# yixuan/LBFGSpp

Measured on AMD Instinct MI355X. Metric: L-BFGS iterations/sec at n=10^8, m=10; achieved HBM GB/s vs peak, higher is better.
Workload: dtype f64; 1 GPU; north-star: extended Rosenbrock n=100000000 m=10 f64 LineSearchMoreThuente, x0 from counter hash; n=100000000, m=10, history_full=True, fevals_total=111, apply_Hv_persistent_launches=82

## Files before the change

include/LBFGS.h:

```cpp
#ifndef LBFGSX_DROPIN_LBFGS_H
#define LBFGSX_DROPIN_LBFGS_H

#include <algorithm>
#include <cmath>
#include <cstdlib>
#include <cstring>
#include <exception>
#include <limits>
#include <stdexcept>
#include <string>
#include <thread>
#include <type_traits>
#include <vector>

#include "LBFGSpp/BKLDLT.h"
#include "LBFGSpp/DenseHessian.h"
#include "LBFGSpp/Device.h"
#include "LBFGSpp/Interop.h"
#include "LBFGSpp/GramSpace.h"
#include "LBFGSpp/LineSearchBacktracking.h"
#include "LBFGSpp/LineSearchBracketing.h"
#include "LBFGSpp/LineSearchMoreThuente.h"
#include "LBFGSpp/LineSearchNocedalWright.h"
#include "LBFGSpp/Param.h"
// ... 12 lines not shown
    int m_nfev = 0;
    int m_x_at_throw = LBFGSX_VEC_X;
    int m_recursion = RECURSION_VECTOR;
    std::function<void(int, Scalar, DeviceState<Scalar>&)> m_trace;
    std::function<void(int)> m_iter_hook;
    std::function<void(double*, int)> m_reducer;
    std::vector<int> m_devices;
    mutable bool m_grad_gathered = false;

    template <typename Foo, typename HostVec>
    int run(Foo& f, Scalar& fx)
    {
        using std::abs;
        using std::sqrt;
        detail::Evaluator<Scalar, Foo, HostVec> ev(f, m_dev);
        if (m_trace)
            ev.on_eval = [this](int k, Scalar v) { m_trace(k, v, m_dev); };
        if (m_reducer)
        {
            if (m_recursion == RECURSION_VECTOR)
                throw std::invalid_argument("a row-sharded run (set_reducer) needs the Gram-space recursion: the vector "
                                            "two-loop reduces its dot products on the device, inside one launch");
            ev.reduce = m_reducer;
        }
        if constexpr (detail::is_compiled_objective<Scalar, Foo>::value)
        {
            if (m_recursion != RECURSION_VECTOR || m_reducer)
                throw std::invalid_argument("a TermObjective runs with the vector recursion on one device: the Gram-space and "
                                            "row-sharded modes take the built-in objectives or a device functor");
        }
        lbfgsx_ctx* c = m_dev.ctx();
        detail::check(lbfgsx_bfgs_reset(c));
        if (m_recursion == RECURSION_VECTOR)
            detail::check(lbfgsx_gs_set_history_dtype(c, detail::dtype_of<Scalar>::value));
        ev.prepare();

        const int fpast = m_param.past;
        if (fpast > 0)
            m_fx.assign(size_t(fpast), Scalar(0));

        Scalar gnorm2, xnorm2;
        ev.initial(fx, gnorm2, xnorm2);
        m_gnorm = sqrt(gnorm2);
        if (fpast > 0)
            m_fx[0] = fx;
        m_nfev = ev.nfev();
        if (m_gnorm <= m_param.epsilon || m_gnorm <= m_param.epsilon_rel * sqrt(xnorm2))
            return 1;

        const bool gram = (m_recursion != RECURSION_VECTOR);
        const bool gram_f32h = (m_recursion == RECURSION_GRAM_SPACE_F32H) && std::is_same<Scalar, double>::value;
        GramSpaceHistory gsh;
        std::vector<double> gs_coef, gs_sdots, gs_gdots, gs_ydots;
        double gs_coef_g = 0, gs_scal[7] = {0, 0, 0, 0, 0, 0, 0};
        if (gram)
        {
            gsh.reset(m_param.m);
            gsh.set_gradient_norm2(double(gnorm2));
            gs_sdots.assign(size_t(2 * m_param.m), 0.0);
            gs_gdots.assign(size_t(2 * m_param.m), 0.0);
            gs_ydots.assign(size_t(2 * m_param.m), 0.0);
            detail::check(lbfgsx_gs_set_history_dtype(c, gram_f32h ? LBFGSX_F32 : detail::dtype_of<Scalar>::value));
        }

        double dgd = 0;
        if (gram)
        {
            gsh.direction(-1.0, gs_coef, gs_coef_g);
            detail::check(lbfgsx_gs_direction(c, gs_coef.data(), gs_coef_g, &dgd));
            if (m_reducer)
                m_reducer(&dgd, 1);
        }
        else
            detail::check(lbfgsx_apply_Hv(c, LBFGSX_VEC_G, -1.0, &dgd));
        Scalar dg = Scalar(dgd);
        Scalar step = Scalar(1) / m_gnorm;
        constexpr Scalar eps = std::numeric_limits<Scalar>::epsilon();

        int k = 1;
        for (;;)
        {
            detail::Range range_iteration("lbfgs:iteration");
            detail::check(lbfgsx_ls_begin(c));
            const Scalar step_max = m_param.max_step;
            ev.trial_written = false;
            try
            {
                detail::Range range_ls("lbfgs:line_search");
                detail::run_line_search<Scalar, LineSearch<Scalar>, HostVec>(ev, m_param, step_max, step, fx, dg);
            }
            catch (...)
            {
                m_nfev = ev.nfev();
                if (ev.trial_written)
                    m_x_at_throw = LBFGSX_VEC_XT;
                throw;
            }
            m_nfev = ev.nfev();

            double g2 = 0, x2 = 0, syd = 0, yyd = 0;
            if (gram)
            {
                detail::check(lbfgsx_gs_post_linesearch(c, gs_scal, gs_sdots.data(), gs_gdots.data(), gs_ydots.data()));
                if (m_reducer)
                {
                    const size_t tm = size_t(2 * m_param.m);
                    std::vector<double> bundle(7 + 3 * tm);
                    std::copy(gs_scal, gs_scal + 7, bundle.begin());
                    std::copy(gs_sdots.begin(), gs_sdots.end(), bundle.begin() + 7);
                    std::copy(gs_gdots.begin(), gs_gdots.end(), bundle.begin() + 7 + tm);
                    std::copy(gs_ydots.begin(), gs_ydots.end(), bundle.begin() + 7 + 2 * tm);
                    m_reducer(bundle.data(), int(bundle.size()));
                    std::copy(bundle.begin(), bundle.begin() + 7, gs_scal);
                    std::copy(bundle.begin() + 7, bundle.begin() + 7 + tm, gs_sdots.begin());
                    std::copy(bundle.begin() + 7 + tm, bundle.begin() + 7 + 2 * tm, gs_gdots.begin());
                    std::copy(bundle.begin() + 7 + 2 * tm, bundle.end(), gs_ydots.begin());
                }
                g2 = gs_scal[0];
                x2 = gs_scal[1];
                syd = gs_scal[2];
                yyd = gs_scal[3];
            }
            else
            {
                detail::Range range_post("lbfgs:post+apply_Hv");
                detail::check(lbfgsx_post_linesearch_spec(c, -1.0, &g2, &x2, &syd, &yyd));
            }
            m_gnorm = sqrt(Scalar(g2));
            if (m_gnorm <= m_param.epsilon || m_gnorm <= m_param.epsilon_rel * sqrt(Scalar(x2)))
                return k;
            if (fpast > 0)
            {
                const Scalar old = m_fx[size_t(k % fpast)];
                if (k >= fpast && abs(old - fx) <= m_param.delta * std::max(std::max(abs(fx), abs(old)), Scalar(1)))
                    return k;
                m_fx[size_t(k % fpast)] = fx;
            }
            if (m_param.max_iterations != 0 && k >= m_param.max_iterations)
                return k;

            const bool accept = Scalar(syd) > eps * Scalar(yyd);
            if (accept)
                detail::check(lbfgsx_commit_correction(c));

            if (gram)
            {
                gsh.update(gs_scal, gs_sdots.data(), gs_gdots.data(), accept, gram_f32h ? gs_ydots.data() : nullptr);
                gsh.direction(-1.0, gs_coef, gs_coef_g);
                detail::check(lbfgsx_gs_direction(c, gs_coef.data(), gs_coef_g, &dgd));
                if (m_reducer)
                    m_reducer(&dgd, 1);
            }
            else
                detail::check(lbfgsx_apply_Hv(c, LBFGSX_VEC_G, -1.0, &dgd));
            dg = Scalar(dgd);
            step = Scalar(1);
            if (m_iter_hook)
                m_iter_hook(k);
            k++;
        }
    }

public:
    LBFGSSolver(const LBFGSParam<Scalar>& param) : m_param(param)
    {
        m_param.check_param();
// ... 182 lines not shown
```

include/lbfgsx.h:

```cpp
#ifndef LBFGSX_H
#define LBFGSX_H

#include <stddef.h>
#include <stdint.h>

#ifdef __cplusplus
extern "C" {
#endif

typedef struct lbfgsx_ctx lbfgsx_ctx;

enum { LBFGSX_F64 = 0, LBFGSX_F32 = 1 };
enum { LBFGSX_OBJ_NONE = -1, LBFGSX_OBJ_DIAG_QUAD = 0, LBFGSX_OBJ_EXT_ROSENBROCK = 1,
       LBFGSX_OBJ_BOUND = 64  };
enum
{
    LBFGSX_OK = 0,
    LBFGSX_E_INVALID = -1,
    LBFGSX_E_LOGIC = -2,
    LBFGSX_E_RUNTIME = -3,
    LBFGSX_E_HIP = -4,
    LBFGSX_E_NOGPU = -5,
    LBFGSX_E_USER = -6
};
enum { LBFGSX_FLAG_BOUNDED = 1  };

enum
{
    LBFGSX_VEC_X = 0,
    LBFGSX_VEC_G = 1,
    LBFGSX_VEC_XP = 2,
    LBFGSX_VEC_GP = 3,
    LBFGSX_VEC_D = 4,
    LBFGSX_VEC_XT = 5,
    LBFGSX_VEC_GT = 6,
    LBFGSX_VEC_A = 7,
    LBFGSX_VEC_B = 8,
    LBFGSX_VEC_LB = 9,
    LBFGSX_VEC_UB = 10,
    LBFGSX_VEC_XCP = 11
};

const char* lbfgsx_last_error(void);
const char* lbfgsx_version(void);
int lbfgsx_device_count(void);

int lbfgsx_create(lbfgsx_ctx** out, int dtype, int64_t n, int m, int device, int flags);
void lbfgsx_destroy(lbfgsx_ctx* c);
int lbfgsx_set_stream(lbfgsx_ctx* c, void* hip_stream);
int lbfgsx_sync(lbfgsx_ctx* c);
int64_t lbfgsx_n(const lbfgsx_ctx* c);
void* lbfgsx_vec(lbfgsx_ctx* c, int which);
int lbfgsx_upload(lbfgsx_ctx* c, int which, const void* host);
int lbfgsx_download(lbfgsx_ctx* c, int which, void* host);
int lbfgsx_gather(lbfgsx_ctx* c, int which, int64_t stride, double* host);

int lbfgsx_set_shard(lbfgsx_ctx* c, int64_t offset, int64_t n_global);
int lbfgsx_gen_diag_quad(lbfgsx_ctx* c, double kappa, uint64_t seed);
int lbfgsx_gen_rosen_x0(lbfgsx_ctx* c, uint64_t seed);
int lbfgsx_fill(lbfgsx_ctx* c, int which, double value);

int lbfgsx_bfgs_reset(lbfgsx_ctx* c);
int lbfgsx_bfgs_ncorr(const lbfgsx_ctx* c);
double lbfgsx_bfgs_theta(const lbfgsx_ctx* c);
int lbfgsx_bfgs_add_correction_host(lbfgsx_ctx* c, const void* s, const void* y);
int lbfgsx_bfgs_stage_correction_host(lbfgsx_ctx* c, const void* s, const void* y, double* sy, double* yy);
int lbfgsx_bfgs_download_history(lbfgsx_ctx* c, void* S_out, void* Y_out, int* ncorr, int* ptr, double* theta);
int lbfgsx_apply_Hv(lbfgsx_ctx* c, int v_which, double a, double* dg);

int lbfgsx_eval(lbfgsx_ctx* c, int objective, double* fx, double* gnorm2, double* xnorm2);
int lbfgsx_norms(lbfgsx_ctx* c, double* gnorm2, double* xnorm2);
int lbfgsx_ls_begin(lbfgsx_ctx* c);
int lbfgsx_trial(lbfgsx_ctx* c, int objective, double step, double* fx, double* dg);
int lbfgsx_trial_point(lbfgsx_ctx* c, double step);
int lbfgsx_trial_dg(lbfgsx_ctx* c, double* dg);
int lbfgsx_ls_keep_trial_as_lo(lbfgsx_ctx* c);
int lbfgsx_ls_end(lbfgsx_ctx* c, int use_lo);
int lbfgsx_post_linesearch(lbfgsx_ctx* c, double* gnorm2, double* xnorm2, double* sy, double* yy);
int lbfgsx_commit_correction(lbfgsx_ctx* c);
int lbfgsx_post_linesearch_spec(lbfgsx_ctx* c, double a, double* gnorm2, double* xnorm2, double* sy, double* yy);
int lbfgsx_spec_counts(const lbfgsx_ctx* c, int64_t out[3]);
typedef struct lbfgsx_objective lbfgsx_objective;
int lbfgsx_objective_compile(lbfgsx_objective** out, int dtype, int K, const char* body, char* log, size_t log_len);
void lbfgsx_objective_destroy(lbfgsx_objective* obj);
long long lbfgsx_objective_source(int dtype, int K, const char* body, char* out, size_t len);
int lbfgsx_objective_info(const lbfgsx_objective* obj, long long out[8]);
int lbfgsx_objective_K(const lbfgsx_objective* obj);
int lbfgsx_objective_dtype(const lbfgsx_objective* obj);
int lbfgsx_objective_bind(lbfgsx_ctx* c, const lbfgsx_objective* obj, const void* const p[4], const double cs[8], int* id);
int lbfgsx_objective_upload(lbfgsx_ctx* c, int slot, const void* host, void** dev);
int lbfgsx_objective_bound(const lbfgsx_ctx* c, const void* p[4]);
enum { LBFGSX_FORM_TERM = 0, LBFGSX_FORM_CHAIN = 1, LBFGSX_FORM_GRID = 2, LBFGSX_FORM_GRAPH = 3, LBFGSX_FORM_MESH = 4, LBFGSX_FORM_LINEAR = 5 };
int lbfgsx_objective_compile_chain(lbfgsx_objective** out, int dtype, int K, const char* body, char* log, size_t log_len);
long long lbfgsx_objective_source_chain(int dtype, int K, const char* body, char* out, size_t len);
int lbfgsx_objective_form(const lbfgsx_objective* obj);
int lbfgsx_objective_compile_grid(lbfgsx_objective** out, int dtype, const char* body, char* log, size_t log_len);
long long lbfgsx_objective_source_grid(int dtype, const char* body, char* out, size_t len);
int lbfgsx_objective_bind_grid(lbfgsx_ctx* c, const lbfgsx_objective* obj, int64_t rows, int64_t cols, const void* const p[4],
                               const double cs[8], int* id);
int lbfgsx_objective_shape(const lbfgsx_ctx* c, int64_t* rows, int64_t* cols);
int lbfgsx_objective_compile_graph(lbfgsx_objective** out, int dtype, const char* node_body, const char* edge_body, char* log,
                                   size_t log_len);
long long lbfgsx_objective_source_graph(int dtype, const char* node_body, const char* edge_body, char* out, size_t len);
int lbfgsx_objective_bind_graph(lbfgsx_ctx* c, const lbfgsx_objective* obj, int64_t E, const int32_t* ei, const int32_t* ej,
                                int edges_on_device, const void* const p[4], const double cs[8], int* id);
int lbfgsx_objective_topology(lbfgsx_ctx* c, int64_t* E, uint32_t* off, int32_t* other, uint32_t* edge_side);
int lbfgsx_objective_upload_count(lbfgsx_ctx* c, int slot, const void* host, int64_t count, void** dev);
int lbfgsx_objective_compile_mesh(lbfgsx_objective** out, int dtype, int K, int D, const char* node_body, const char* elem_body,
                                  char* log, size_t log_len);
long long lbfgsx_objective_source_mesh(int dtype, int K, int D, const char* node_body, const char* elem_body, char* out, size_t len);
int lbfgsx_objective_bind_mesh(lbfgsx_ctx* c, const lbfgsx_objective* obj, int64_t E, const int32_t* elems, int elems_on_device,
                               const void* const p[4], const double cs[8], int* id);
int lbfgsx_objective_mesh_topology(lbfgsx_ctx* c, int64_t* E, uint32_t* off, uint32_t* words);
int lbfgsx_objective_dim(const lbfgsx_objective* obj);
int lbfgsx_objective_compile_linear(lbfgsx_objective** out, int dtype, const char* coord_body, const char* row_body, char* log,
                                    size_t log_len);
long long lbfgsx_objective_source_linear(int dtype, const char* coord_body, const char* row_body, char* out, size_t len);
int lbfgsx_objective_bind_linear(lbfgsx_ctx* c, const lbfgsx_objective* obj, int64_t R, int64_t nnz, const int32_t* rowptr,
                                 const int32_t* col, const void* val, int matrix_on_device, int lanes, const void* const p[4],
                                 const double cs[8], int* id);
int lbfgsx_objective_linear_topology(lbfgsx_ctx* c, int64_t info[8], uint32_t* colptr, int32_t* trow, uint32_t* tpos,
                                     int32_t* long_col, uint32_t* long_chunk, uint32_t* chunk);
int lbfgsx_device(const lbfgsx_ctx* c);
int lbfgsx_device_push(const lbfgsx_ctx* c, int* prev);
int lbfgsx_device_pop(int prev);
int lbfgsx_persist_counts(const lbfgsx_ctx* c, int64_t out[4]);
int lbfgsx_debug_persist_fault(lbfgsx_ctx* c);
int lbfgsx_counters(int64_t out[3], int reset);
int lbfgsx_counters_ex(int64_t out[8], int reset);
int lbfgsx_poll_counts(const lbfgsx_ctx* c, int64_t out[2]);
int lbfgsx_poll_counts_ex(const lbfgsx_ctx* c, int64_t out[4]);
void lbfgsx_range_push(const char* name);
void lbfgsx_range_pop(void);

int lbfgsx_gs_post_linesearch(lbfgsx_ctx* c, double scal[7], double* sdots, double* gdots, double* ydots);
int lbfgsx_gs_set_history_dtype(lbfgsx_ctx* c, int dtype);
int lbfgsx_gs_direction(lbfgsx_ctx* c, const double* coef, double coef_g, double* dg);

enum
{
    LBFGSX_ST_FREE = 1, LBFGSX_ST_NEWACT = 2, LBFGSX_ST_L = 4, LBFGSX_ST_U = 8, LBFGSX_ST_P = 16
};
enum
{
    LBFGSX_VS_DRT = 0,
    LBFGSX_VS_NEG_CF = 1,
    LBFGSX_VS_NEG_RHS = 2,
    LBFGSX_VS_LBOUND = 3,
    LBFGSX_VS_UBOUND = 4,
    LBFGSX_VS_Y = 5
};
enum
{
    LBFGSX_CB_LINEAR = 0,
    LBFGSX_CB_SOLVE = 1,
    LBFGSX_CB_RHS_ADD = 2,
    LBFGSX_CB_LAMBDA = 3,
    LBFGSX_CB_MU = 4
};
enum
{
    LBFGSX_SO_SAVE_FALLBACK = 0, LBFGSX_SO_RHS_INIT = 1, LBFGSX_SO_ASSIGN_Y = 2, LBFGSX_SO_CLAMP_Y = 3,
    LBFGSX_SO_CLAMP_FB = 4, LBFGSX_SO_ASSIGN_FB = 5
};
// ... 163 lines not shown
```

lbfgspp_amd/_lib.py:

```python
import ctypes as C
import os

HERE = os.path.dirname(os.path.abspath(__file__))

F64, F32 = 0, 1
OBJ_DIAG_QUAD, OBJ_EXT_ROSENBROCK = 0, 1
OBJ_BOUND = 64
LS_NOCEDAL_WRIGHT, LS_MORE_THUENTE, LS_BACKTRACKING, LS_BRACKETING = 0, 1, 2, 3
ALGO_LBFGS, ALGO_LBFGSB = 0, 1
RECURSION_VECTOR, RECURSION_GRAM_SPACE, RECURSION_GRAM_SPACE_F32H = 0, 1, 2
FLAG_BOUNDED = 1
(VEC_X, VEC_G, VEC_XP, VEC_GP, VEC_D, VEC_XT, VEC_GT, VEC_A, VEC_B, VEC_LB, VEC_UB, VEC_XCP) = range(12)
E_INVALID, E_LOGIC, E_RUNTIME, E_HIP, E_NOGPU, E_USER = -1, -2, -3, -4, -5, -6


class Params(C.Structure):
    _fields_ = [("m", C.c_int), ("epsilon", C.c_double), ("epsilon_rel", C.c_double), ("past", C.c_int),
                ("delta", C.c_double), ("max_iterations", C.c_int), ("linesearch", C.c_int),
                ("max_linesearch", C.c_int), ("min_step", C.c_double), ("max_step", C.c_double),
                ("ftol", C.c_double), ("wolfe", C.c_double), ("max_submin", C.c_int)]


class Result(C.Structure):
    _fields_ = [("niter", C.c_int), ("nfev", C.c_int), ("fx", C.c_double), ("gnorm", C.c_double),
# ... 11 lines not shown

ITER_HOOK = C.CFUNCTYPE(None, C.c_int, C.c_void_p)
ALLREDUCE = C.CFUNCTYPE(None, C.POINTER(C.c_double), C.c_int, C.c_void_p)
OBJECTIVE_FN = C.CFUNCTYPE(C.c_int, C.c_void_p, C.c_void_p, C.c_void_p, C.c_int64, C.POINTER(C.c_double))
BATCH_OBJECTIVE_FN = C.CFUNCTYPE(C.c_int, C.c_void_p, C.c_int, C.POINTER(C.c_int64), C.c_void_p, C.c_void_p, C.c_int64,
                                 C.POINTER(C.c_double))

_core = None
_solver = None


class NativeLibraryMissing(RuntimeError):
    pass


def load():
    global _core, _solver
    if _core is not None:
        return _core, _solver
    try:
        import torch
    except Exception:
        pass
    p_core = os.path.join(HERE, "liblbfgsx.so")
    p_sol = os.path.join(HERE, "liblbfgsx_solver.so")
    for p in (p_core, p_sol):
        if not os.path.exists(p):
            raise NativeLibraryMissing(
                "%s not found: build the HIP extension first (python -c 'import __graft_entry__ as g; g.build()')" % p)
    core = C.CDLL(p_core)
    sol = C.CDLL(p_sol)
    vp, i64, dbl, i32 = C.c_void_p, C.c_int64, C.c_double, C.c_int
    pd = C.POINTER(C.c_double)

    def sig(lib, name, res, *args):
        f = getattr(lib, name)
        f.restype = res
        f.argtypes = list(args)
        return f

    sig(core, "lbfgsx_last_error", C.c_char_p)
    sig(core, "lbfgsx_version", C.c_char_p)
    sig(core, "lbfgsx_device_count", i32)
    sig(core, "lbfgsx_create", i32, C.POINTER(vp), i32, i64, i32, i32, i32)
    sig(core, "lbfgsx_destroy", None, vp)
    sig(core, "lbfgsx_set_stream", i32, vp, vp)
    sig(core, "lbfgsx_sync", i32, vp)
    sig(core, "lbfgsx_n", i64, vp)
    sig(core, "lbfgsx_vec", vp, vp, i32)
    sig(core, "lbfgsx_upload", i32, vp, i32, vp)
    sig(core, "lbfgsx_download", i32, vp, i32, vp)
    sig(core, "lbfgsx_gather", i32, vp, i32, i64, pd)
    sig(core, "lbfgsx_gen_diag_quad", i32, vp, dbl, C.c_uint64)
    sig(core, "lbfgsx_gen_rosen_x0", i32, vp, C.c_uint64)
    sig(core, "lbfgsx_fill", i32, vp, i32, dbl)
    sig(core, "lbfgsx_bfgs_reset", i32, vp)
    sig(core, "lbfgsx_bfgs_ncorr", i32, vp)
    sig(core, "lbfgsx_bfgs_theta", dbl, vp)
    sig(core, "lbfgsx_bfgs_add_correction_host", i32, vp, vp, vp)
    sig(core, "lbfgsx_bfgs_download_history", i32, vp, vp, vp, C.POINTER(i32), C.POINTER(i32), pd)
    sig(core, "lbfgsx_apply_Hv", i32, vp, i32, dbl, pd)
    sig(core, "lbfgsx_eval", i32, vp, i32, pd, pd, pd)
    sig(core, "lbfgsx_norms", i32, vp, pd, pd)
    sig(core, "lbfgsx_ls_begin", i32, vp)
    sig(core, "lbfgsx_trial", i32, vp, i32, dbl, pd, pd)
    sig(core, "lbfgsx_trial_point", i32, vp, dbl)
    sig(core, "lbfgsx_trial_dg", i32, vp, pd)
    sig(core, "lbfgsx_ls_keep_trial_as_lo", i32, vp)
    sig(core, "lbfgsx_ls_end", i32, vp, i32)
    sig(core, "lbfgsx_post_linesearch", i32, vp, pd, pd, pd, pd)
    sig(core, "lbfgsx_commit_correction", i32, vp)
    sig(core, "lbfgsx_gs_post_linesearch", i32, vp, pd, pd, pd, pd)
    sig(core, "lbfgsx_gs_set_history_dtype", i32, vp, i32)
    sig(core, "lbfgsx_gs_direction", i32, vp, pd, dbl, pd)
    sig(core, "lbfgsx_timing_enable", i32, vp, i32)
    sig(core, "lbfgsx_timing_read", i32, vp, pd, C.POINTER(i64), pd, C.POINTER(i64))
    sig(core, "lbfgsx_stream_probe", i32, vp, i32, pd, pd)
    sig(core, "lbfgsx_selftest_reduce", i32, vp, i32, i32, i32, pd)
    sig(core, "lbfgsx_post_linesearch_spec", i32, vp, dbl, pd, pd, pd, pd)
    sig(core, "lbfgsx_rccl_allgather_records", i32, C.POINTER(i32), i32, vp, i64, i64, C.POINTER(vp))
    sig(core, "lbfgsx_device_download", i32, i32, vp, i64, vp)
    sig(core, "lbfgsx_device_free", None, i32, vp)
    sig(core, "lbfgsx_spec_counts", i32, vp, C.POINTER(i64 * 3))
    sig(core, "lbfgsx_counters", i32, C.POINTER(i64 * 3), i32)
    sig(core, "lbfgsx_counters_ex", i32, C.POINTER(i64 * 8), i32)
    sig(core, "lbfgsx_poll_counts", i32, vp, C.POINTER(i64 * 2))
    sig(core, "lbfgsx_poll_counts_ex", i32, vp, C.POINTER(i64 * 4))
    sig(core, "lbfgsx_b_compact_vec_counts", i32, C.POINTER(i64 * 4), i32)
    sig(core, "lbfgsx_b_reserve", i32, vp)
    sig(core, "lbfgsx_device", i32, vp)
    sig(core, "lbfgsx_persist_counts", i32, vp, C.POINTER(i64 * 4))
    sig(core, "lbfgsx_debug_persist_fault", i32, vp)

    sig(sol, "lbfgsx_solver_create", i32, C.POINTER(vp), i32, i32, i32, C.POINTER(Params), i32)
    sig(sol, "lbfgsx_solver_create_error", C.c_char_p)
    sig(sol, "lbfgsx_solver_destroy", None, vp)
    sig(sol, "lbfgsx_solver_prepare", i32, vp, i64)
    sig(sol, "lbfgsx_solver_ctx", vp, vp)
    sig(sol, "lbfgsx_solver_set_recursion", i32, vp, i32)
    sig(sol, "lbfgsx_solver_set_allreduce", i32, vp, ALLREDUCE, vp)
    sig(sol, "lbfgsx_solver_set_devices", i32, vp, C.POINTER(i32), i32)
    sig(core, "lbfgsx_comm_unique_id", i32, C.c_char_p)
    sig(core, "lbfgsx_comm_create_rank", i32, C.POINTER(vp), i32, i32, i32, C.c_char_p)
    sig(core, "lbfgsx_comm_create_local", i32, C.POINTER(vp), C.POINTER(i32), i32)
    sig(core, "lbfgsx_comm_allreduce_sum", i32, vp, i32, pd, i32)
    sig(core, "lbfgsx_comm_abort", i32, vp)
    sig(core, "lbfgsx_comm_abort_from", i32, vp, i32)
    sig(core, "lbfgsx_comm_first_abort", i32, vp)
    sig(core, "lbfgsx_b_gram_pairs_max", i32, vp)
    sig(core, "lbfgsx_b_post_linesearch_build", i32, vp, dbl, pd, pd, pd, pd)
    sig(core, "lbfgsx_b_post_build_counts", i32, C.POINTER(i64 * 2), i32)
    sig(core, "lbfgsx_b_psel_counts", i32, C.POINTER(i64 * 1), i32)
    sig(core, "lbfgsx_b_dg_maxstep_trial", i32, vp, i32, dbl, pd, pd)
    sig(core, "lbfgsx_b_solve_sweep_rhs", i32, vp, i32, i32, pd, dbl, pd, pd, pd, C.POINTER(i64 * 7))
    sig(core, "lbfgsx_b_solve_sweep_rhs_ready", i32, vp)
    sig(core, "lbfgsx_b_gram_last_vrow_dd", i32, vp, pd)
    sig(core, "lbfgsx_b_wtv_lu_c", i32, vp, pd, C.POINTER(i64), pd, C.POINTER(i64), pd)
    sig(core, "lbfgsx_b_trial_ahead_counts", i32, vp, C.POINTER(i64 * 2))
    sig(core, "lbfgsx_comm_info", i32, vp, C.POINTER(i32 * 4))
    sig(core, "lbfgsx_comm_calls", i64, vp, i32)
    sig(core, "lbfgsx_comm_hook_arg", vp, vp, i32)
    sig(core, "lbfgsx_comm_destroy", None, vp)
    sig(core, "lbfgsx_set_shard", i32, vp, i64, i64)
    sig(sol, "lbfgsx_solver_set_iteration_hook", i32, vp, ITER_HOOK, vp)
    sig(sol, "lbfgsx_batch_minimize", i32, i32, i32, i32, C.POINTER(Params), i32, i64, i64, i64, C.c_uint64, i32, i32,
        C.POINTER(BatchItem))
    sig(sol, "lbfgsx_batch_minimize_lockstep", i32, i32, C.POINTER(Params), i64, i64, i32, C.c_uint64, i32,
        C.POINTER(BatchItem), vp, C.c_char_p, i32)
    sig(sol, "lbfgsx_batch_minimize_lockstep_multi", i32, i32, C.POINTER(Params), i64, i64, i32, C.c_uint64,
        C.POINTER(i32), i32, C.POINTER(BatchItem), vp, C.c_char_p, i32)
    sig(sol, "lbfgsx_batch_minimize_lockstep_ex", i32, i32, i32, i32, dbl, C.POINTER(Params), i64, i64, i32, C.c_uint64,
        C.POINTER(i32), i32, C.POINTER(BatchItem), vp, C.c_char_p, i32)
    sig(sol, "lbfgsx_lockstep_create", i32, C.POINTER(vp), i32, i32, C.POINTER(Params), i64, i32, i32, i32, C.c_char_p, i32)
    sig(sol, "lbfgsx_lockstep_minimize", i32, vp, i32, dbl, C.c_uint64, i64, C.POINTER(BatchItem), vp, C.POINTER(dbl * 8),
        C.c_char_p, i32)
    sig(sol, "lbfgsx_lockstep_destroy", None, vp)
    sig(sol, "lbfgsx_lockstep_set_timing", i32, vp, i32)
    sig(sol, "lbfgsx_solver_hessians", i32, vp, vp, vp)
    sig(sol, "lbfgsx_solver_stats", i32, vp, C.POINTER(C.c_longlong * 8))
    sig(sol, "lbfgsx_solver_stats2", i32, vp, C.POINTER(C.c_longlong * 8))
    sig(sol, "lbfgsx_solver_stats3", i32, vp, C.POINTER(C.c_longlong * 8))
    sig(sol, "lbfgsx_solver_minimize", i32, vp, i32, i64, vp, vp, vp, vp, vp, C.POINTER(Trace), C.POINTER(Result))
    sig(sol, "lbfgsx_solver_minimize_fn", i32, vp, i64, OBJECTIVE_FN, vp, vp, vp, vp, C.POINTER(Trace), C.POINTER(Result))
    sig(sol, "lbfgsx_lockstep_minimize_fn", i32, vp, vp, BATCH_OBJECTIVE_FN, vp, C.POINTER(BatchItem), vp, C.POINTER(dbl * 8),
        C.c_char_p, i32)
    sig(core, "lbfgsx_objective_compile", i32, C.POINTER(vp), i32, i32, C.c_char_p, C.c_char_p, C.c_size_t)
    sig(core, "lbfgsx_objective_destroy", None, vp)
    sig(core, "lbfgsx_objective_source", C.c_longlong, i32, i32, C.c_char_p, C.c_char_p, C.c_size_t)
    sig(core, "lbfgsx_objective_info", i32, vp, C.POINTER(C.c_longlong * 8))
    sig(core, "lbfgsx_objective_compile_chain", i32, C.POINTER(vp), i32, i32, C.c_char_p, C.c_char_p, C.c_size_t)
    sig(core, "lbfgsx_objective_source_chain", C.c_longlong, i32, i32, C.c_char_p, C.c_char_p, C.c_size_t)
    sig(core, "lbfgsx_objective_form", i32, vp)
    sig(core, "lbfgsx_objective_K", i32, vp)
    sig(core, "lbfgsx_objective_dtype", i32, vp)
    sig(core, "lbfgsx_objective_bind", i32, vp, vp, C.POINTER(vp * 4), C.POINTER(dbl * 8), C.POINTER(i32))
    sig(core, "lbfgsx_objective_upload", i32, vp, i32, vp, C.POINTER(vp))
    sig(core, "lbfgsx_objective_bound", i32, vp, C.POINTER(vp * 4))
    sig(sol, "lbfgsx_solver_minimize_obj", i32, vp, vp, i64, C.POINTER(vp * 4), i32, C.POINTER(dbl * 8), vp, vp, vp,
        C.POINTER(Trace), C.POINTER(Result))
    sig(core, "lbfgsx_objective_compile_grid", i32, C.POINTER(vp), i32, C.c_char_p, C.c_char_p, C.c_size_t)
    sig(core, "lbfgsx_objective_source_grid", C.c_longlong, i32, C.c_char_p, C.c_char_p, C.c_size_t)
    sig(core, "lbfgsx_objective_bind_grid", i32, vp, vp, i64, i64, C.POINTER(vp * 4), C.POINTER(dbl * 8), C.POINTER(i32))
    sig(core, "lbfgsx_objective_shape", i32, vp, C.POINTER(i64), C.POINTER(i64))
    sig(sol, "lbfgsx_solver_minimize_grid", i32, vp, vp, i64, i64, C.POINTER(vp * 4), i32, C.POINTER(dbl * 8), vp, vp, vp,
        C.POINTER(Trace), C.POINTER(Result))
    i32p, u32p = C.POINTER(C.c_int32), C.POINTER(C.c_uint32)
# ... 64 lines not shown
```

lbfgspp_amd/csrc/ctx.hpp:

```cpp
#pragma once
#include <hip/hip_runtime.h>
#include <stdint.h>

#include <atomic>
#include <chrono>
#include <string>
#include <vector>

#include "../../include/lbfgsx.h"
#include "reduce.cuh"

struct lbfgsx_ctx;
namespace lbfgsx {

void set_error(const std::string& msg);

#define LBFGSX_HIP(expr)                                                                      \
    do                                                                                        \
    {                                                                                         \
        hipError_t e_ = (expr);                                                               \
        if (e_ != hipSuccess)                                                                 \
        {                                                                                     \
            lbfgsx::set_error(std::string(#expr) + ": " + hipGetErrorString(e_) + " [" + __FILE__ + ":" + std::to_string(__LINE__) + "]");            \
            return LBFGSX_E_HIP;                                                              \
// ... 95 lines not shown
int bounded_note_column(lbfgsx_ctx* c, int col);
struct GsState;
void gs_free(lbfgsx_ctx* c);

struct EventPair
{
    hipEvent_t a, b;
};

constexpr int kGridCap = 1024;
constexpr int kGridCapTwoloop = 512;

}

struct lbfgsx_ctx
{
    int dtype = LBFGSX_F64;
    size_t esz = 8;
    int64_t n = 0, ld = 0;
    int64_t shard_off = 0, n_global = 0;
    int m = 0, device = 0, flags = 0;
    hipStream_t stream = nullptr;
    bool own_stream = false;

    void* xb[3] = {nullptr, nullptr, nullptr};
    void* gb[3] = {nullptr, nullptr, nullptr};
    int cur = 0, xp = 0, lo = 0, trial = 1;
    void* d = nullptr;
    void* a = nullptr;
    void* b = nullptr;

    void* S = nullptr;
    void* Y = nullptr;
    std::vector<int> phys;
    unsigned phys_version = 1;
    int spare = 0;
    int ncorr = 0, ptr = 0;
    bool pending = false;
    double theta = 1.0;
    double pend_sy = 0.0, pend_yy = 0.0;
    std::vector<double> ys_host;

    lbfgsx::ScLayout sl;
    void* sc = nullptr;
    void* hout = nullptr;
    void* outmap_host = nullptr;
    void* outmap_dev = nullptr;
    lbfgsx::RedWs ws;
    unsigned long long* done_host = nullptr;
    unsigned long long* done_dev = nullptr;
    unsigned long long done_seq = 0;
    long long poll_waits = 0, poll_timeouts = 0, poll_lost = 0;
    long long poll_late = 0;
    bool poll_pending = false;
    bool poll_off = false;
    unsigned tl_step = 0;
    bool persist = true;
    bool meet_all = true;
    int persist_cooldown = 0;
    int persist_backoff = 8;
    int64_t persist_timeouts = 0;
    int64_t step_products = 0;
    int persist_grid = 0;
    unsigned* gen_dev = nullptr;
    size_t gen_words = 0;
    unsigned gen_count = 0;
    int64_t persist_steps_timed = 0;
    int64_t coarse_steps_timed = 0;
    int64_t fused_timed = 0;
    bool counted = false;
    int64_t persist_launches = 0;
    bool fuse_post = true;
    bool fast_persist_out = true;
    bool st_valid = false;
    int st_obj = -1, st_xp = -1, st_trial = -1;
    double st_step = 0.0, st_f = 0.0, st_dg = 0.0;
    int st_cooldown = 0;
    int64_t st_runs = 0, st_hits = 0;
    bool spec_valid = false;
    unsigned spec_version = 0;
    int spec_cur = 0;
    double spec_a = 0.0, spec_dg = 0.0;
    int64_t spec_launches = 0, spec_used = 0, spec_rejected = 0;

    const struct lbfgsx_objective* term = nullptr;
    void* term_fn[6] = {nullptr, nullptr, nullptr, nullptr, nullptr, nullptr};
    const void* term_p[4] = {nullptr, nullptr, nullptr, nullptr};
    double term_c[8] = {0, 0, 0, 0, 0, 0, 0, 0};
    int term_np = 0;
    int term_form = 0;
    int64_t term_rows = 0, term_cols = 0;
    void* term_own[4] = {nullptr, nullptr, nullptr, nullptr};
    int64_t term_own_count[4] = {0, 0, 0, 0};
    int64_t graph_E = 0;
    void* graph_off = nullptr;
    void* graph_inc = nullptr;
    int mesh_K = 0, mesh_D = 0;
    struct LinearTopo
    {
        int64_t R = 0, nnz = 0, nchunks = 0;
        int L = 0, C = 0, nlong = 0;
        void *rowptr = nullptr, *col = nullptr, *val = nullptr;
        void *colptr = nullptr, *trow = nullptr, *tval = nullptr;
        void* tpos = nullptr;
        void *w = nullptr, *v = nullptr;
        void *part = nullptr, *long_col = nullptr, *long_chunk = nullptr;
        void* chunk = nullptr;
    } lin;

    void* lb = nullptr;
    void* ub = nullptr;
    void* xcp = nullptr;
    struct lbfgsb_state* bstate = nullptr;
    lbfgsx::GsState* gs = nullptr;
    bool gs_f32h = false;

    bool timing = false;
    bool timing_per_launch = true;
    std::vector<lbfgsx::EventPair> ev_twoloop, ev_hv;
    void* gather_tmp = nullptr;
    int64_t gather_cap = 0;

    template <class T>
    T* out_slot() const
    {
        return outmap_dev ? static_cast<T*>(outmap_dev) : static_cast<T*>(sc) + sl.out(0);
    }
    void* col(void* base, int c) const { return static_cast<char*>(base) + size_t(c) * size_t(ld) * esz; }
    int grid_for(int64_t nelem, int unroll_ = 1) const
    {
        const int64_t w = (dtype == LBFGSX_F64) ? 2 : 4;
        const int64_t tile = int64_t(lbfgsx::kBlock) * unroll_;
        int64_t blocks = (nelem / w + tile - 1) / tile;
        if (blocks < 1)
            blocks = 1;
        if (blocks > lbfgsx::kGridCap)
            blocks = lbfgsx::kGridCap;
        return int(blocks);
    }
};

namespace lbfgsx {
inline void poll_arm(lbfgsx_ctx* c)
{
    if (c->done_host && !c->poll_off)
    {
        c->ws.done = c->done_dev;
        c->ws.seq = ++c->done_seq;
        c->poll_pending = true;
    }
}
inline bool poll_armed(const lbfgsx_ctx* c) { return c->done_host && c->poll_pending && c->ws.done && c->ws.seq == c->done_seq; }
inline void poll_disarm(lbfgsx_ctx* c)
{
    c->ws.done = nullptr;
    c->poll_pending = false;
}
inline hipError_t poll_wait(lbfgsx_ctx* c)
{
    if (!poll_armed(c))
    {
        poll_disarm(c);
        return stream_sync(c->stream);
    }
    poll_disarm(c);
    counters().syncs.fetch_add(1, std::memory_order_relaxed);
    const bool tr = host_trace_on();
    if (tr)
        host_trace(">sync");
// ... 39 lines not shown
```

lbfgspp_amd/csrc/jit_objective.hip:

```cpp
#include <dlfcn.h>
#include <hip/hiprtc.h>

#include <chrono>
#include <cstdio>
#include <cstdlib>
#include <cstring>
#include <map>
#include <memory>
#include <mutex>
#include <string>
#include <vector>

#include "launch_args.hpp"

namespace {

const char* const kKernelNames[6][lbfgsx::JIT_NSLOTS] = {
    {"k_eval", "k_trial", "k_b_eval", "k_b_dg_maxstep_trial"},
    {"k_chain_eval", "k_chain_trial", "k_chain_b_eval", "k_chain_b_dg_maxstep_trial"},
    {"k_grid_eval", "k_grid_trial", "k_grid_b_eval", "k_grid_b_dg_maxstep_trial"},
    {"k_graph_eval", "k_graph_trial", "k_graph_b_eval", "k_graph_b_dg_maxstep_trial"},
    {"k_mesh_eval", "k_mesh_trial", "k_mesh_b_eval", "k_mesh_b_dg_maxstep_trial"},
    {"k_lin_eval", "k_lin_trial", "k_lin_b_eval", "k_lin_b_dg_maxstep_trial", "k_lin_rows", "k_lin_rows_trial"}};
const char* const kObjStruct[6] = {"ObjTerm", "ObjChain", "ObjGrid", "ObjGraph", "ObjMesh", "ObjLinear"};
const char* const kFormName[6] = {"term objective", "chain objective", "grid objective", "graph objective", "mesh objective",
                                  "linear-model objective"};
inline int kernels_of(int form) { return form == LBFGSX_FORM_LINEAR ? lbfgsx::JIT_NSLOTS : lbfgsx::JIT_NKERNELS; }

struct Rtc
{
    void* lib = nullptr;
    decltype(&hiprtcCreateProgram) create = nullptr;
    decltype(&hiprtcDestroyProgram) destroy = nullptr;
    decltype(&hiprtcAddNameExpression) add_name = nullptr;
    decltype(&hiprtcCompileProgram) compile = nullptr;
    decltype(&hiprtcGetProgramLogSize) log_size = nullptr;
    decltype(&hiprtcGetProgramLog) log = nullptr;
    decltype(&hiprtcGetLoweredName) lowered = nullptr;
    decltype(&hiprtcGetCodeSize) code_size = nullptr;
    decltype(&hiprtcGetCode) code = nullptr;
    std::string error;
};

const Rtc& rtc()
{
    static Rtc r;
    static std::once_flag once;
    std::call_once(once, []() {
        std::vector<std::string> names = {"libhiprtc.so"};
        if (const char* e = getenv("ROCM_PATH"))
            names.push_back(std::string(e) + "/lib/libhiprtc.so");
        names.push_back("/opt/rocm/lib/libhiprtc.so");
        names.push_back("libhiprtc.so.7");
        for (const std::string& n : names)
            if ((r.lib = dlopen(n.c_str(), RTLD_NOW | RTLD_LOCAL)))
                break;
        if (!r.lib)
        {
            r.error = "libhiprtc.so not found (the run-time compiler of ROCm)";
            return;
        }
#define RTC_SYM(member, name)                                             \
    r.member = reinterpret_cast<decltype(r.member)>(dlsym(r.lib, #name)); \
    if (!r.member)                                                        \
        r.error = "libhiprtc.so lacks " #name;
        RTC_SYM(create, hiprtcCreateProgram)
        RTC_SYM(destroy, hiprtcDestroyProgram)
        RTC_SYM(add_name, hiprtcAddNameExpression)
        RTC_SYM(compile, hiprtcCompileProgram)
        RTC_SYM(log_size, hiprtcGetProgramLogSize)
        RTC_SYM(log, hiprtcGetProgramLog)
        RTC_SYM(lowered, hiprtcGetLoweredName)
        RTC_SYM(code_size, hiprtcGetCodeSize)
        RTC_SYM(code, hiprtcGetCode)
#undef RTC_SYM
    });
    return r;
}

std::string kernel_dir()
{
    if (const char* e = getenv("LBFGSX_KERNEL_DIR"))
        return e;
    Dl_info info;
    if (dladdr(reinterpret_cast<const void*>(&kernel_dir), &info) && info.dli_fname)
    {
        std::string p = info.dli_fname;
        const size_t k = p.rfind('/');
        return (k == std::string::npos ? std::string(".") : p.substr(0, k)) + "/csrc";
    }
    return "csrc";
}

std::string generate_chain(int dtype, int K, const char* body);
std::string generate_grid(int dtype, const char* body);
std::string generate_graph(int dtype, const char* node, const char* body);
std::string generate_mesh(int dtype, int K, int D, const char* node, const char* body);
std::string generate_linear(int dtype, const char* coord, const char* body);

std::string generate(int form, int dtype, int K, const char* body, const char* node, int D)
{
    if (form == LBFGSX_FORM_LINEAR)
        return generate_linear(dtype, node, body);
    if (form == LBFGSX_FORM_MESH)
        return generate_mesh(dtype, K, D, node, body);
    if (form == LBFGSX_FORM_GRAPH)
        return generate_graph(dtype, node, body);
    if (form == LBFGSX_FORM_CHAIN)
        return generate_chain(dtype, K, body);
    if (form == LBFGSX_FORM_GRID)
        return generate_grid(dtype, body);
    std::string s;
    s += "// generated by lbfgsx_objective_compile: one term objective for the fused kernels\n";
    s += "#include \"lbfgs_kernels.cuh\"\n";
    s += "#include \"lbfgsb_kernels.cuh\"\n";
    s += "namespace lbfgsx {\n";
    s += std::string("typedef ") + (dtype == LBFGSX_F64 ? "double" : "float") + " term_scalar_t;\n";
    s += "struct ObjTerm\n{\n";
    s += "    typedef term_scalar_t T;\n";
    s += "    static constexpr int K = " + std::to_string(K) + ";\n";
    s += "    const T* p0;\n    const T* p1;\n    const T* p2;\n    const T* p3;\n    T c[8];\n";
    s += "    // one term: x[0..K) in, g[0..K) out, the term's value returned\n";
    s += "    __device__ __forceinline__ T term(const T (&x)[K], T (&g)[K], int64_t i) const\n    {\n";
    s += "#line 1 \"objective_body\"\n";
    s += body;
    s += "\n#line 1 \"objective_wrapper\"\n";
    s += "    }\n";
    s += "    // the W / K terms of one 16-byte pack (W is a multiple of K: a term never straddles a pack)\n";
    s += "    template <class A>\n";
    s += "    __device__ __forceinline__ void pack(int64_t vi, const Pack<T>& x, Pack<T>& g, A& fx) const\n    {\n";
    s += "        constexpr int W = Vec16<T>::W;\n";
    s += "#pragma unroll\n";
    s += "        for (int k = 0; k < W; k += K)\n        {\n";
    s += "            T tx[K], tg[K];\n";
    s += "#pragma unroll\n";
    s += "            for (int j = 0; j < K; j++)\n                tx[j] = x.e[k + j];\n";
    s += "            const T v = term(tx, tg, vi * W + k);\n";
    s += "#pragma unroll\n";
    s += "            for (int j = 0; j < K; j++)\n                g.e[k + j] = tg[j];\n";
    s += "            fx.add(v);\n";
    s += "        }\n    }\n";
    s += "    __device__ __forceinline__ T finish(T sum) const { return sum; }\n";
    s += "    // the coordinates past the last whole pack, called for every i of them: the term that starts at i, if one does\n";
    s += "    template <class A>\n";
    s += "    __device__ __forceinline__ void tail(int64_t i, int64_t n, const T* x, T* g, A& fx) const\n    {\n";
    s += "        if (i % K == 0 && i + K <= n)\n        {\n";
    s += "            T tx[K], tg[K];\n";
    s += "            for (int j = 0; j < K; j++)\n                tx[j] = x[i + j];\n";
    s += "            const T v = term(tx, tg, i);\n";
    s += "            for (int j = 0; j < K; j++)\n                g[i + j] = tg[j];\n";
    s += "            fx.add(v);\n";
    s += "        }\n    }\n";
    s += "};\n";
    s += "typedef term_scalar_t S;\n";
    s += "template __global__ void k_eval<S, ObjTerm>(const S*, S*, int64_t, ObjTerm, RedWs, S*);\n";
    s += "template __global__ void k_trial<S, ObjTerm>(const S*, const S*, S, S*, S*, int64_t, ObjTerm, RedWs, S*, int);\n";
    s += "template __global__ void k_b_eval<S, ObjTerm>(const S*, S*, const S*, const S*, int64_t, ObjTerm, RedWs, S*);\n";
    s += "template __global__ void k_b_dg_maxstep_trial<S, ObjTerm>(const S*, const S*, const S*, const S*, const S*, S, S*, S*, "
         "int64_t, ObjTerm, RedWs, S*, int);\n";
    s += "}  // namespace lbfgsx\n";
    return s;
}

std::string generate_chain(int dtype, int K, const char* body)
{
    std::string s;
    s += "// generated by lbfgsx_objective_compile_chain: one chain objective for the fused kernels\n";
    s += "#include \"chain_kernels.cuh\"\n";
    s += "namespace lbfgsx {\n";
    s += std::string("typedef ") + (dtype == LBFGSX_F64 ? "double" : "float") + " term_scalar_t;\n";
    s += "struct ObjChain\n{\n";
    s += "    typedef term_scalar_t T;\n";
    s += "    static constexpr int K = " + std::to_string(K) + ";\n";
    s += "    const T* p0;\n    const T* p1;\n    const T* p2;\n    const T* p3;\n    T c[8];\n";
    s += "    // the term that starts at coordinate i: x[0..K) in, its K partial derivatives g[0..K) out, its value returned\n";
    s += "    __device__ __forceinline__ T term(const T (&x)[K], T (&g)[K], int64_t i) const\n    {\n";
    s += "#line 1 \"objective_body\"\n";
    s += body;
    s += "\n#line 1 \"objective_wrapper\"\n";
    s += "    }\n";
    s += "};\n";
    s += "typedef term_scalar_t S;\n";
    s += "template __global__ void k_chain_eval<S, ObjChain>(const S*, S*, int64_t, ObjChain, RedWs, S*);\n";
    s += "template __global__ void k_chain_trial<S, ObjChain>(const S*, const S*, S, S*, S*, int64_t, ObjChain, RedWs, S*, int);\n";
    s += "template __global__ void k_chain_b_eval<S, ObjChain>(const S*, S*, const S*, const S*, int64_t, ObjChain, RedWs, S*);\n";
    s += "template __global__ void k_chain_b_dg_maxstep_trial<S, ObjChain>(const S*, const S*, const S*, const S*, const S*, S, S*, "
         "S*, int64_t, ObjChain, RedWs, S*, int);\n";
    s += "}  // namespace lbfgsx\n";
    return s;
}

std::string generate_grid(int dtype, const char* body)
{
    std::string s;
    s += "// generated by lbfgsx_objective_compile_grid: one grid objective for the fused kernels\n";
    s += "#include \"grid_kernels.cuh\"\n";
    s += "namespace lbfgsx {\n";
    s += std::string("typedef ") + (dtype == LBFGSX_F64 ? "double" : "float") + " term_scalar_t;\n";
    s += "struct ObjGrid\n{\n";
    s += "    typedef term_scalar_t T;\n";
    s += "    static constexpr int K = 4;\n";
    s += "    const T* p0;\n    const T* p1;\n    const T* p2;\n    const T* p3;\n    T c[8];\n";
    s += "    int64_t rows, cols;\n";
    s += "    // the cell whose origin is node (row, col), flat index i = row*cols + col: x = {x[row,col], x[row,col+1], x[row+1,col],\n";
    s += "    // x[row+1,col+1]} in, its four partial derivatives g out, its value returned\n";
    s += "    __device__ __forceinline__ T term(const T (&x)[4], T (&g)[4], int64_t i, int64_t row, int64_t col) const\n    {\n";
    s += "#line 1 \"objective_body\"\n";
    s += body;
    s += "\n#line 1 \"objective_wrapper\"\n";
    s += "    }\n";
    s += "};\n";
    s += "typedef term_scalar_t S;\n";
    s += "template __global__ void k_grid_eval<S, ObjGrid>(const S*, S*, int64_t, ObjGrid, RedWs, S*);\n";
    s += "template __global__ void k_grid_trial<S, ObjGrid>(const S*, const S*, S, S*, S*, int64_t, ObjGrid, RedWs, S*, int);\n";
    s += "template __global__ void k_grid_b_eval<S, ObjGrid>(const S*, S*, const S*, const S*, int64_t, ObjGrid, RedWs, S*);\n";
    s += "template __global__ void k_grid_b_dg_maxstep_trial<S, ObjGrid>(const S*, const S*, const S*, const S*, const S*, S, S*, "
         "S*, int64_t, ObjGrid, RedWs, S*, int);\n";
    s += "}  // namespace lbfgsx\n";
    return s;
}

std::string generate_graph(int dtype, const char* node, const char* body)
{
    const bool has_node = node && *node;
    std::string s;
    s += "// generated by lbfgsx_objective_compile_graph: one graph objective for the fused kernels\n";
    s += "#include \"graph_kernels.cuh\"\n";
    s += "namespace lbfgsx {\n";
    s += std::string("typedef ") + (dtype == LBFGSX_F64 ? "double" : "float") + " term_scalar_t;\n";
    s += "struct ObjGraph\n{\n";
    s += "    typedef term_scalar_t T;\n";
    s += "    static constexpr int K = 2;\n";
    s += std::string("    static constexpr bool kNode = ") + (has_node ? "true" : "false") + ";\n";
    s += "    const T* p0;\n    const T* p1;\n    const T* p2;\n    const T* p3;\n    T c[8];\n";
    s += "    const uint32_t* off;\n    const GraphEntry* inc;\n    int64_t E;\n";
    s += "    // the term of node i: x[0] = x[i] in, its derivative g[0] out, its value returned\n";
    s += "    __device__ __forceinline__ T node(const T (&x)[1], T (&g)[1], int64_t i) const\n    {\n";
    if (has_node)
    {
// ... 233 lines not shown

bool find_symbol(const std::vector<char>& co, const std::string& name, Elf64Sym& out)
{
    if (co.size() < sizeof(Elf64Ehdr) || std::memcmp(co.data(), "\177ELF", 4) != 0)
        return false;
    Elf64Ehdr eh;
    std::memcpy(&eh, co.data(), sizeof(eh));
    if (eh.shentsize != sizeof(Elf64Shdr) || eh.shoff + uint64_t(eh.shnum) * sizeof(Elf64Shdr) > co.size())
        return false;
    std::vector<Elf64Shdr> sh(eh.shnum);
    std::memcpy(sh.data(), co.data() + eh.shoff, sh.size() * sizeof(Elf64Shdr));
    for (const Elf64Shdr& t : sh)
    {
        if ((t.type != 2 && t.type != 11) || t.link >= sh.size() || t.offset + t.size > co.size())
            continue;
        const Elf64Shdr& str = sh[t.link];
        if (str.offset + str.size > co.size())
            continue;
        for (uint64_t k = 0; k + sizeof(Elf64Sym) <= t.size; k += sizeof(Elf64Sym))
        {
            Elf64Sym sy;
            std::memcpy(&sy, co.data() + t.offset + k, sizeof(sy));
            if (sy.name >= str.size)
                continue;
            const char* nm = co.data() + str.offset + sy.name;
            const size_t room = size_t(str.size - sy.name);
            if (name.size() < room && std::memcmp(nm, name.c_str(), name.size() + 1) == 0)
            {
                out = sy;
                return true;
            }
        }
    }
    return false;
}

bool kernel_resources(const std::vector<char>& co, const std::string& kernel, long long& vgprs, long long& scratch)
{
    Elf64Sym kd;
    if (!find_symbol(co, kernel + ".kd", kd))
        return false;
    Elf64Ehdr eh;
    std::memcpy(&eh, co.data(), sizeof(eh));
    uint64_t off = 0;
    bool found = false;
    for (int k = 0; k < eh.shnum && !found; k++)
    {
        Elf64Shdr t;
        std::memcpy(&t, co.data() + eh.shoff + uint64_t(k) * sizeof(Elf64Shdr), sizeof(t));
        if (t.type != 8 && t.addr <= kd.value && kd.value + 64 <= t.addr + t.size)
        {
            off = t.offset + (kd.value - t.addr);
            found = true;
        }
    }
    if (!found || off + 64 > co.size())
        return false;
    uint32_t priv = 0, rsrc1 = 0;
    std::memcpy(&priv, co.data() + off + 4, 4);
    std::memcpy(&rsrc1, co.data() + off + 48, 4);
    scratch = priv;
    Elf64Sym nv, na;
    if (find_symbol(co, kernel + ".num_vgpr", nv))
        vgprs = (long long) nv.value + (find_symbol(co, kernel + ".num_agpr", na) ? (long long) na.value : 0);
    else
        vgprs = ((rsrc1 & 63u) + 1) * 8;
    return true;
}

}

struct lbfgsx_objective
{
    struct lbfgsx_objective_code* code = nullptr;
    bool cache_hit = false;
};

struct lbfgsx_objective_code
{
    lbfgsx_objective self;
    int form = LBFGSX_FORM_TERM, dtype = LBFGSX_F64, K = 1, D = 1;
    std::vector<char> code;
    std::string lowered[lbfgsx::JIT_NSLOTS];
    long long vgprs[lbfgsx::JIT_NSLOTS] = {0, 0, 0, 0, 0, 0}, scratch[lbfgsx::JIT_NSLOTS] = {0, 0, 0, 0, 0, 0};
    double compile_ms = 0.0;
    struct Loaded
    {
        hipModule_t mod = nullptr;
        hipFunction_t fn[lbfgsx::JIT_NSLOTS] = {nullptr, nullptr, nullptr, nullptr, nullptr, nullptr};
    };
    std::mutex mu;
    std::map<int, Loaded> loaded;
};

namespace {

std::mutex g_cache_mu;
std::map<std::string, std::unique_ptr<lbfgsx_objective_code> >& cache()
{
    static std::map<std::string, std::unique_ptr<lbfgsx_objective_code> > m;
    return m;
}

int compile_code(int form, int dtype, int K, int D, const char* body, const char* node,
                 std::unique_ptr<lbfgsx_objective_code>& out, std::string& log)
{
    const Rtc& r = rtc();
    if (!r.error.empty())
    {
        log = r.error;
        return LBFGSX_E_RUNTIME;
    }
    const std::string src = generate(form, dtype, K, body, node, D);
    const char* hsrc[] = {"\n"};
    const char* hname[] = {"hip/hip_runtime.h"};
    hiprtcProgram prog = nullptr;
    if (r.create(&prog, src.c_str(), "objective_wrapper", 1, hsrc, hname) != HIPRTC_SUCCESS)
    {
        log = "hiprtcCreateProgram failed";
        return LBFGSX_E_RUNTIME;
    }
    std::string expr[lbfgsx::JIT_NSLOTS];
    const int nk = kernels_of(form);
    for (int k = 0; k < nk; k++)
    {
        expr[k] = std::string("lbfgsx::") + kKernelNames[form][k] + "<lbfgsx::term_scalar_t, lbfgsx::" + kObjStruct[form] + ">";
        (void) r.add_name(prog, expr[k].c_str());
    }
    const std::string inc = "-I" + kernel_dir();
    const char* opts[] = {"--offload-arch=gfx950", "-O3", "-std=c++17", "-ffp-contract=off", inc.c_str()};
    const auto t0 = std::chrono::steady_clock::now();
    const hiprtcResult res = r.compile(prog, int(sizeof(opts) / sizeof(opts[0])), opts);
    const double ms = std::chrono::duration<double, std::milli>(std::chrono::steady_clock::now() - t0).count();
    size_t ls = 0;
    if (r.log_size(prog, &ls) == HIPRTC_SUCCESS && ls > 1)
    {
        log.assign(ls, '\0');
        (void) r.log(prog, &log[0]);
        while (!log.empty() && log.back() == '\0')
            log.pop_back();
    }
    if (res != HIPRTC_SUCCESS)
    {
        if (log.empty())
            log = "hipRTC could not compile the objective";
        (void) r.destroy(&prog);
        return LBFGSX_E_INVALID;
    }
    std::unique_ptr<lbfgsx_objective_code> code(new lbfgsx_objective_code());
    code->form = form;
    code->dtype = dtype;
    code->K = K;
    code->D = D;
    code->compile_ms = ms;
    size_t cs = 0;
    bool ok = r.code_size(prog, &cs) == HIPRTC_SUCCESS && cs > 0;
    if (ok)
    {
        code->code.resize(cs);
        ok = r.code(prog, code->code.data()) == HIPRTC_SUCCESS;
    }
    for (int k = 0; ok && k < nk; k++)
    {
        const char* low = nullptr;
        ok = r.lowered(prog, expr[k].c_str(), &low) == HIPRTC_SUCCESS && low;
        if (ok)
        {
            code->lowered[k] = low;
            ok = kernel_resources(code->code, code->lowered[k], code->vgprs[k], code->scratch[k]);
        }
    }
    (void) r.destroy(&prog);
    if (!ok)
    {
        log = std::string(kFormName[form]) + ": the compiled code object lacks a kernel or its descriptor";
        return LBFGSX_E_RUNTIME;
    }
    code->self.code = code.get();
    out = std::move(code);
    return LBFGSX_OK;
}

void put_log(char* log, size_t log_len, const std::string& text)
{
    if (log && log_len > 0)
        std::snprintf(log, log_len, "%s", text.c_str());
}

}

namespace lbfgsx {

int jit_launch(lbfgsx_ctx* c, int which, int grid, void** params)
{
    hipFunction_t fn = c->term ? static_cast<hipFunction_t>(c->term_fn[which]) : nullptr;
    if (!fn)
    {
        set_error("term objective: no kernel loaded for this context (lbfgsx_objective_bind)");
        return LBFGSX_E_LOGIC;
    }
    counters().launches.fetch_add(1, std::memory_order_relaxed);
    if (host_trace_on())
        host_trace(kKernelNames[c->term->code->form][which]);
    LBFGSX_HIP(hipModuleLaunchKernel(fn, unsigned(grid), 1, 1, unsigned(kBlock), 1, 1, 0, c->stream, params, nullptr));
    return LBFGSX_OK;
}

}

namespace {

long long objective_source(int form, int dtype, int K, const char* body, char* out, size_t len, const char* node = nullptr,
                           int D = 1)
{
    std::string why;
    if (!valid_request(form, dtype, K, body, node, D, why))
    {
        lbfgsx::set_error(why);
        return LBFGSX_E_INVALID;
    }
    const std::string s = generate(form, dtype, K, body, node, D);
    if (out && len > 0)
        std::snprintf(out, len, "%s", s.c_str());
    return (long long) s.size() + 1;
}

int objective_compile(int form, lbfgsx_objective** out, int dtype, int K, const char* body, char* log, size_t log_len,
                      const char* node = nullptr, int D = 1)
{
    if (log && log_len > 0)
        log[0] = '\0';
    if (!out)
        return LBFGSX_E_INVALID;
    *out = nullptr;
    std::string why;
    if (!valid_request(form, dtype, K, body, node, D, why))
    {
        lbfgsx::set_error(why);
        put_log(log, log_len, why);
        return LBFGSX_E_INVALID;
    }
    std::string key = std::to_string(form) + "/" + std::to_string(dtype) + "/" + std::to_string(K) + "/" + body;
    if (form == LBFGSX_FORM_GRAPH || form == LBFGSX_FORM_MESH || form == LBFGSX_FORM_LINEAR)
        key += std::string("\x1f") + (node ? node : "");
    if (form == LBFGSX_FORM_MESH)
        key += "\x1f" + std::to_string(D);
// ... 6 lines not shown
        std::string text;
        const int rc = compile_code(form, dtype, K, D, body, node, code, text);
        if (rc)
        {
            lbfgsx::set_error(std::string(kFormName[form]) + ": compilation failed\n" + text);
            put_log(log, log_len, text);
            return rc;
        }
        put_log(log, log_len, text);
        it = cache().emplace(key, std::move(code)).first;
    }
    lbfgsx_objective* h = new lbfgsx_objective();
    h->code = it->second.get();
    h->cache_hit = hit;
    *out = h;
    return LBFGSX_OK;
}

}

extern "C" {

long long lbfgsx_objective_source(int dtype, int K, const char* body, char* out, size_t len)
{
    return objective_source(LBFGSX_FORM_TERM, dtype, K, body, out, len);
}
long long lbfgsx_objective_source_chain(int dtype, int K, const char* body, char* out, size_t len)
{
    return objective_source(LBFGSX_FORM_CHAIN, dtype, K, body, out, len);
}
long long lbfgsx_objective_source_grid(int dtype, const char* body, char* out, size_t len)
{
    return objective_source(LBFGSX_FORM_GRID, dtype, 4, body, out, len);
}
long long lbfgsx_objective_source_graph(int dtype, const char* node_body, const char* edge_body, char* out, size_t len)
{
    return objective_source(LBFGSX_FORM_GRAPH, dtype, 2, edge_body, out, len, node_body);
}
long long lbfgsx_objective_source_mesh(int dtype, int K, int D, const char* node_body, const char* elem_body, char* out, size_t len)
{
    return objective_source(LBFGSX_FORM_MESH, dtype, K, elem_body, out, len, node_body, D);
}
long long lbfgsx_objective_source_linear(int dtype, const char* coord_body, const char* row_body, char* out, size_t len)
{
    return objective_source(LBFGSX_FORM_LINEAR, dtype, 1, row_body, out, len, coord_body);
}

int lbfgsx_objective_compile(lbfgsx_objective** out, int dtype, int K, const char* body, char* log, size_t log_len)
{
    return objective_compile(LBFGSX_FORM_TERM, out, dtype, K, body, log, log_len);
}
int lbfgsx_objective_compile_chain(lbfgsx_objective** out, int dtype, int K, const char* body, char* log, size_t log_len)
{
    return objective_compile(LBFGSX_FORM_CHAIN, out, dtype, K, body, log, log_len);
}
int lbfgsx_objective_compile_grid(lbfgsx_objective** out, int dtype, const char* body, char* log, size_t log_len)
{
    return objective_compile(LBFGSX_FORM_GRID, out, dtype, 4, body, log, log_len);
}
int lbfgsx_objective_compile_graph(lbfgsx_objective** out, int dtype, const char* node_body, const char* edge_body, char* log,
                                   size_t log_len)
{
    return objective_compile(LBFGSX_FORM_GRAPH, out, dtype, 2, edge_body, log, log_len, node_body);
}
int lbfgsx_objective_compile_mesh(lbfgsx_objective** out, int dtype, int K, int D, const char* node_body, const char* elem_body,
                                  char* log, size_t log_len)
{
    return objective_compile(LBFGSX_FORM_MESH, out, dtype, K, elem_body, log, log_len, node_body, D);
}
int lbfgsx_objective_compile_linear(lbfgsx_objective** out, int dtype, const char* coord_body, const char* row_body, char* log,
                                    size_t log_len)
{
    return objective_compile(LBFGSX_FORM_LINEAR, out, dtype, 1, row_body, log, log_len, coord_body);
}

void lbfgsx_objective_destroy(lbfgsx_objective* obj) { delete obj; }

int lbfgsx_objective_info(const lbfgsx_objective* obj, long long out[8])
{
    if (!obj || !out)
        return LBFGSX_E_INVALID;
    const lbfgsx_objective_code* k = obj->code;
    out[0] = out[1] = 0;
    for (int j = 0; j < kernels_of(k->form); j++)
    {
        out[0] = k->vgprs[j] > out[0] ? k->vgprs[j] : out[0];
        out[1] = k->scratch[j] > out[1] ? k->scratch[j] : out[1];
        if (j < lbfgsx::JIT_NKERNELS)
            out[4 + j] = k->scratch[j];
    }
    out[2] = obj->cache_hit ? 1 : 0;
    out[3] = (long long) (k->compile_ms + 0.5);
    return LBFGSX_OK;
}

int lbfgsx_objective_K(const lbfgsx_objective* obj) { return obj ? obj->code->K : LBFGSX_E_INVALID; }
int lbfgsx_objective_dim(const lbfgsx_objective* obj) { return obj ? obj->code->D : LBFGSX_E_INVALID; }
int lbfgsx_objective_dtype(const lbfgsx_objective* obj) { return obj ? obj->code->dtype : LBFGSX_E_INVALID; }
int lbfgsx_objective_form(const lbfgsx_objective* obj) { return obj ? obj->code->form : LBFGSX_E_INVALID; }

int lbfgsx_objective_upload_count(lbfgsx_ctx* c, int slot, const void* host, int64_t count, void** dev)
{
    if (!c || slot < 0 || slot >= 4 || !host)
    {
        lbfgsx::set_error("lbfgsx_objective_upload: a term objective has four data arrays, slots 0..3");
        return LBFGSX_E_INVALID;
    }
    if (count < 1)
    {
        lbfgsx::set_error("lbfgsx_objective_upload_count: count = " + std::to_string(count) + ": a data array has at least one element");
        return LBFGSX_E_INVALID;
    }
    lbfgsx::DeviceGuard dev_guard_(c->device);
    if (c->term_own[slot] && c->term_own_count[slot] != count)
    {
        LBFGSX_HIP(lbfgsx::stream_sync(c->stream));
        (void) hipFree(c->term_own[slot]);
        c->term_own[slot] = nullptr;
    }
    if (!c->term_own[slot])
    {
        LBFGSX_HIP(hipMalloc(&c->term_own[slot], size_t(count) * c->esz));
        c->term_own_count[slot] = count;
    }
    LBFGSX_HIP(lbfgsx::copy_async(c->term_own[slot], host, size_t(count) * c->esz, hipMemcpyHostToDevice, c->stream));
    LBFGSX_HIP(lbfgsx::stream_sync(c->stream));
    if (dev)
        *dev = c->term_own[slot];
    return LBFGSX_OK;
}

int lbfgsx_objective_upload(lbfgsx_ctx* c, int slot, const void* host, void** dev)
{
    return lbfgsx_objective_upload_count(c, slot, host, c ? c->n : 0, dev);
}

}

namespace {

int objective_bind(lbfgsx_ctx* c, const lbfgsx_objective* obj, int64_t rows, int64_t cols, const void* const p[4],
                   const double cs[8], int* id)
{
    c->st_valid = false;
    c->spec_valid = false;
    if (!obj)
    {
        c->term = nullptr;
        c->term_np = 0;
        c->term_form = LBFGSX_FORM_TERM;
        c->term_rows = c->term_cols = 0;
        if (c->graph_inc || c->lin.colptr)
        {
            lbfgsx::DeviceGuard dev_guard_(c->device);
            (void) lbfgsx::stream_sync(c->stream);
            lbfgsx::graph_topology_free(c);
        }
        if (id)
            *id = LBFGSX_OBJ_NONE;
        return LBFGSX_OK;
    }
    lbfgsx_objective_code* code = obj->code;
    if (code->dtype != c->dtype)
    {
        lbfgsx::set_error("lbfgsx_objective_bind: the objective was compiled for the other dtype");
        return LBFGSX_E_INVALID;
    }
    if (code->form == LBFGSX_FORM_CHAIN)
    {
        if (c->n < code->K)
        {
            lbfgsx::set_error("chain objective: n = " + std::to_string(c->n) + " is less than K = " + std::to_string(code->K) +
                              ": there is no term");
            return LBFGSX_E_INVALID;
        }
    }
    else if (code->form == LBFGSX_FORM_MESH && c->n % code->D != 0)
    {
        lbfgsx::set_error("mesh objective: n = " + std::to_string(c->n) + " is not a multiple of D = " + std::to_string(code->D) +
                          ": x holds D unknowns per node");
        return LBFGSX_E_INVALID;
    }
    else if (code->form == LBFGSX_FORM_TERM && c->n % code->K != 0)
    {
        lbfgsx::set_error("term objective: n = " + std::to_string(c->n) + " is not a multiple of K = " + std::to_string(code->K));
        return LBFGSX_E_INVALID;
    }
    lbfgsx::DeviceGuard dev_guard_(c->device);
    {
        std::lock_guard<std::mutex> lock(code->mu);
        auto it = code->loaded.find(c->device);
        if (it == code->loaded.end())
        {
            lbfgsx_objective_code::Loaded l;
            LBFGSX_HIP(hipModuleLoadData(&l.mod, code->code.data()));
            for (int k = 0; k < kernels_of(code->form); k++)
                LBFGSX_HIP(hipModuleGetFunction(&l.fn[k], l.mod, code->lowered[k].c_str()));
            it = code->loaded.emplace(c->device, l).first;
        }
        for (int k = 0; k < lbfgsx::JIT_NSLOTS; k++)
            c->term_fn[k] = it->second.fn[k];
    }
    if (code->form != LBFGSX_FORM_GRAPH && code->form != LBFGSX_FORM_MESH && code->form != LBFGSX_FORM_LINEAR &&
        (c->graph_inc || c->lin.colptr))
    {
        (void) lbfgsx::stream_sync(c->stream);
        lbfgsx::graph_topology_free(c);
    }
    c->term = &code->self;
    c->term_form = code->form;
    c->term_rows = rows;
    c->term_cols = cols;
    c->term_np = 0;
    for (int j = 0; j < 4; j++)
    {
        c->term_p[j] = p ? p[j] : nullptr;
        c->term_np += c->term_p[j] ? 1 : 0;
    }
    for (int j = 0; j < 8; j++)
        c->term_c[j] = cs ? cs[j] : 0.0;
    if (id)
        *id = LBFGSX_OBJ_BOUND;
    return LBFGSX_OK;
}

}

extern "C" {

int lbfgsx_objective_bind(lbfgsx_ctx* c, const lbfgsx_objective* obj, const void* const p[4], const double cs[8], int* id)
{
    if (!c)
        return LBFGSX_E_INVALID;
    if (obj && obj->code->form == LBFGSX_FORM_GRID)
    {
        lbfgsx::set_error("a grid objective is bound with its shape: lbfgsx_objective_bind_grid");
        return LBFGSX_E_INVALID;
    }
    if (obj && obj->code->form == LBFGSX_FORM_GRAPH)
    {
        lbfgsx::set_error("a graph objective is bound with its edges: lbfgsx_objective_bind_graph");
        return LBFGSX_E_INVALID;
    }
    if (obj && obj->code->form == LBFGSX_FORM_MESH)
    {
        lbfgsx::set_error("a mesh objective is bound with its elements: lbfgsx_objective_bind_mesh");
        return LBFGSX_E_INVALID;
    }
    if (obj && obj->code->form == LBFGSX_FORM_LINEAR)
    {
        lbfgsx::set_error("a linear-model objective is bound with its matrix: lbfgsx_objective_bind_linear");
        return LBFGSX_E_INVALID;
    }
    return objective_bind(c, obj, 0, 0, p, cs, id);
}

int lbfgsx_objective_bind_grid(lbfgsx_ctx* c, const lbfgsx_objective* obj, int64_t rows, int64_t cols, const void* const p[4],
                               const double cs[8], int* id)
{
    if (!c || !obj)
        return LBFGSX_E_INVALID;
    if (obj->code->form != LBFGSX_FORM_GRID)
    {
        lbfgsx::set_error(std::string("lbfgsx_objective_bind_grid: the handle is a ") + kFormName[obj->code->form] +
                          ", not a grid objective (lbfgsx_objective_compile_grid)");
        return LBFGSX_E_INVALID;
    }
    const std::string shape = "rows = " + std::to_string(rows) + ", cols = " + std::to_string(cols);
    long long prod = 0;
    if (rows < 2 || cols < 2)
    {
        lbfgsx::set_error("grid objective: " + shape + ": a grid has at least 2 rows and 2 columns (rows >= 2, cols >= 2)");
        return LBFGSX_E_INVALID;
    }
    if (__builtin_mul_overflow((long long) rows, (long long) cols, &prod) || prod != (long long) c->n)
    {
        lbfgsx::set_error("grid objective: " + shape + " does not multiply to n = " + std::to_string(c->n));
        return LBFGSX_E_INVALID;
    }
    return objective_bind(c, obj, rows, cols, p, cs, id);
// ... 233 lines not shown
```

lbfgspp_amd/csrc/launch_args.hpp:

```cpp
#pragma once
#include "ctx.hpp"

namespace lbfgsx {

template <class T>
struct EvalLaunch
{
    int grid;
    const T* x;
    T* g;
    int64_t n;
    RedWs ws;
    T* out;
};
template <class T>
inline EvalLaunch<T> eval_launch(lbfgsx_ctx* c)
{
    return {c->grid_for(c->n), static_cast<const T*>(c->xb[c->cur]), static_cast<T*>(c->gb[c->cur]), c->n, c->ws,
            c->out_slot<T>()};
}

template <class T>
struct TrialLaunch
{
    int grid;
    const T *xp, *d;
    T step;
    T *x, *g;
    int64_t n;
    RedWs ws;
    T* out;
    int rev;
};
template <class T>
inline TrialLaunch<T> trial_launch(lbfgsx_ctx* c, T step, int obj_vectors)
{
    const int rev = (c->tl_step++ & 1u) ? 1 : 0;
    poll_arm(c);
    model_add(double(c->n) * sizeof(T) * (4 + obj_vectors));
    return {c->grid_for(c->n), static_cast<const T*>(c->xb[c->xp]), static_cast<const T*>(c->d), step,
            static_cast<T*>(c->xb[c->trial]), static_cast<T*>(c->gb[c->trial]), c->n, c->ws, c->out_slot<T>(), rev};
}

template <class T>
struct BEvalLaunch
{
    int grid;
    const T* x;
    T* g;
    const T *lb, *ub;
    int64_t n;
    RedWs ws;
    T* out;
};
template <class T>
inline BEvalLaunch<T> b_eval_launch(lbfgsx_ctx* c)
{
    return {c->grid_for(c->n), static_cast<const T*>(c->xb[c->cur]), static_cast<T*>(c->gb[c->cur]),
            static_cast<const T*>(c->lb), static_cast<const T*>(c->ub), c->n, c->ws, c->out_slot<T>()};
}

template <class T>
struct DgTrialLaunch
{
    int grid;
    const T *xp, *g0, *d, *lb, *ub;
    T step;
    T *x, *g;
    int64_t n;
    RedWs ws;
    T* out;
    int rev;
};
template <class T>
inline DgTrialLaunch<T> dg_maxstep_trial_launch(lbfgsx_ctx* c, T step, int obj_vectors)
{
    const int rev = (c->tl_step & 1u) ? 1 : 0;
    poll_arm(c);
    model_add(double(c->n) * sizeof(T) * (7 + obj_vectors));
    return {c->grid_for(c->n), static_cast<const T*>(c->xb[c->xp]), static_cast<const T*>(c->gb[c->cur]),
            static_cast<const T*>(c->d), static_cast<const T*>(c->lb), static_cast<const T*>(c->ub), step,
            static_cast<T*>(c->xb[c->trial]), static_cast<T*>(c->gb[c->trial]), c->n, c->ws, c->out_slot<T>(), rev};
}

enum { JIT_K_EVAL = 0, JIT_K_TRIAL = 1, JIT_K_B_EVAL = 2, JIT_K_B_DG_MAXSTEP_TRIAL = 3, JIT_NKERNELS = 4 };
enum { JIT_K_LIN_ROWS = 4, JIT_K_LIN_ROWS_TRIAL = 5, JIT_NSLOTS = 6 };
template <class T>
struct TermArgs
{
    const T* p[4];
    T c[8];
};
template <class T>
inline TermArgs<T> term_args(const lbfgsx_ctx* c)
{
    TermArgs<T> a;
    for (int j = 0; j < 4; j++)
        a.p[j] = static_cast<const T*>(c->term_p[j]);
    for (int j = 0; j < 8; j++)
        a.c[j] = T(c->term_c[j]);
    return a;
}
template <class T>
struct GridArgs
{
    TermArgs<T> t;
    int64_t rows, cols;
};
struct GraphEntry;
template <class T>
struct GraphArgs
{
    TermArgs<T> t;
    const uint32_t* off;
    const GraphEntry* inc;
    int64_t E;
};
template <class T>
struct MeshArgs
{
    TermArgs<T> t;
    const uint32_t* off;
    const uint32_t* inc;
    int64_t E, N;
};
template <class T>
struct LinearArgs
{
    TermArgs<T> t;
    const int32_t* rowptr;
    const int32_t* col;
    const T* val;
    const uint32_t* colptr;
    const int32_t* trow;
    const T* tval;
    T* w;
    T* v;
    const T* part;
    const int32_t* long_col;
    const uint32_t* long_chunk;
    int64_t R, nnz;
    int32_t L, C, nlong, pad_;
};
template <class T>
inline LinearArgs<T> linear_args(const lbfgsx_ctx* c, const TermArgs<T>& t)
{
    const lbfgsx_ctx::LinearTopo& l = c->lin;
    return {t,
            static_cast<const int32_t*>(l.rowptr),
            static_cast<const int32_t*>(l.col),
            static_cast<const T*>(l.val),
            static_cast<const uint32_t*>(l.colptr),
            static_cast<const int32_t*>(l.trow),
            static_cast<const T*>(l.tval),
            static_cast<T*>(l.w),
            static_cast<T*>(l.v),
            static_cast<const T*>(l.part),
            static_cast<const int32_t*>(l.long_col),
            static_cast<const uint32_t*>(l.long_chunk),
            l.R,
            l.nnz,
            l.L,
            l.C,
            l.nlong,
            0};
}
template <class T>
struct BoundArgs
{
// ... 98 lines not shown
```

lbfgspp_amd/csrc/lbfgs_kernels.cuh:

```cuda
#pragma once
#include "reduce.cuh"

namespace lbfgsx {

enum { OBJ_DIAG_QUAD = 0, OBJ_EXT_ROSENBROCK = 1 };

template <class T>
struct ObjQuad
{
    const T* a;
    const T* b;
    template <class A>
    __device__ __forceinline__ void pack(int64_t vi, const Pack<T>& x, Pack<T>& g, A& fx) const
    {
        const Pack<T> pa = ldv(a, vi), pb = ldv(b, vi);
#pragma unroll
        for (int k = 0; k < Vec16<T>::W; k++)
        {
            const T r = pa.e[k] * x.e[k] - pb.e[k];
            g.e[k] = pa.e[k] * r;
            fx.add(r * r);
        }
    }
    __device__ __forceinline__ T finish(T sum) const { return T(0.5) * sum; }
    template <class A>
    __device__ __forceinline__ void tail(int64_t i, int64_t, const T* x, T* g, A& fx) const
    {
        const T r = a[i] * x[i] - b[i];
        g[i] = a[i] * r;
        fx.add(r * r);
    }
};

template <class T>
struct ObjRosen
{
    template <class A>
    __device__ __forceinline__ void pack(int64_t, const Pack<T>& x, Pack<T>& g, A& fx) const
    {
#pragma unroll
        for (int k = 0; k < Vec16<T>::W; k += 2)
        {
            const T t1 = T(1) - x.e[k];
            const T t2 = T(10) * (x.e[k + 1] - x.e[k] * x.e[k]);
            g.e[k + 1] = T(20) * t2;
            g.e[k] = T(-2) * (x.e[k] * g.e[k + 1] + t1);
            fx.add(t1 * t1 + t2 * t2);
        }
    }
    __device__ __forceinline__ T finish(T sum) const { return sum; }
    template <class A>
    __device__ __forceinline__ void tail(int64_t i, int64_t n, const T* x, T* g, A& fx) const
    {
        if ((i & 1) == 0 && i + 1 < n)
        {
            const T t1 = T(1) - x[i];
            const T t2 = T(10) * (x[i + 1] - x[i] * x[i]);
            g[i + 1] = T(20) * t2;
            g[i] = T(-2) * (x[i] * g[i + 1] + t1);
            fx.add(t1 * t1 + t2 * t2);
        }
    }
};

template <class T, class OBJ>
__global__ void __launch_bounds__(kBlock) k_eval(const T* __restrict__ x, T* __restrict__ g, int64_t n, OBJ obj,
                                                 RedWs ws, T* __restrict__ out)
{
    typedef typename AccOf<T>::type A;
    constexpr int W = Vec16<T>::W;
    A acc[3];
    const int64_t nv = n / W;
    const int64_t stride = int64_t(gridDim.x) * kBlock;
    for (int64_t vi = int64_t(blockIdx.x) * kBlock + threadIdx.x; vi < nv; vi += stride)
    {
        const Pack<T> px = ldv(x, vi);
        Pack<T> pg;
        obj.pack(vi, px, pg, acc[0]);
        stv(g, vi, pg);
#pragma unroll
        for (int k = 0; k < W; k++)
        {
            acc[1].add_prod(pg.e[k], pg.e[k]);
            acc[2].add_prod(px.e[k], px.e[k]);
        }
    }
    if (blockIdx.x == 0 && threadIdx.x == 0)
        for (int64_t i = nv * W; i < n; i++)
        {
            obj.tail(i, n, x, g, acc[0]);
            acc[1].add_prod(g[i], g[i]);
            acc[2].add_prod(x[i], x[i]);
        }
    if (grid_reduce<3>(acc, ws) && threadIdx.x == 0)
    {
        out[0] = obj.finish(T(acc[0].value()));
        out[1] = T(acc[1].value());
        out[2] = T(acc[2].value());
    }
}

template <class T, class OBJ>
__global__ void __launch_bounds__(kBlock) k_trial(const T* __restrict__ xp, const T* __restrict__ d, T step,
                                                  T* __restrict__ x, T* __restrict__ g, int64_t n, OBJ obj,
                                                  RedWs ws, T* __restrict__ out, int rev)
{
    typedef typename AccOf<T>::type A;
    constexpr int W = Vec16<T>::W;
    constexpr int U = 4;
    A acc[2];
    const int64_t nv = n / W;
    const int64_t tile = int64_t(kBlock) * U;
    const int64_t top = ((nv + tile - 1) / tile - 1) * tile;
    for (int64_t t0 = int64_t(blockIdx.x) * tile; t0 < nv; t0 += int64_t(gridDim.x) * tile)
    {
        const int64_t base = (rev ? top - t0 : t0) + threadIdx.x;
        Pack<T> pxp[U], pd[U];
#pragma unroll
        for (int u = 0; u < U; u++)
            if (base + u * kBlock < nv)
            {
                pxp[u] = ldv(xp, base + u * kBlock);
                pd[u] = ldv(d, base + u * kBlock);
            }
#pragma unroll
        for (int u = 0; u < U; u++)
        {
            const int64_t vi = base + u * kBlock;
            if (vi < nv)
            {
                Pack<T> px, pg;
#pragma unroll
                for (int k = 0; k < W; k++)
                    px.e[k] = pxp[u].e[k] + step * pd[u].e[k];
                obj.pack(vi, px, pg, acc[0]);
                stv(x, vi, px);
                stv(g, vi, pg);
#pragma unroll
                for (int k = 0; k < W; k++)
                    acc[1].add_prod(pg.e[k], pd[u].e[k]);
            }
        }
    }
    if (blockIdx.x == 0 && threadIdx.x == 0)
    {
        for (int64_t i = nv * W; i < n; i++)
            x[i] = xp[i] + step * d[i];
        for (int64_t i = nv * W; i < n; i++)
        {
            obj.tail(i, n, x, g, acc[0]);
            acc[1].add_prod(g[i], d[i]);
        }
    }
    if (grid_reduce<2>(acc, ws) && threadIdx.x == 0)
    {
        out[0] = obj.finish(T(acc[0].value()));
        out[1] = T(acc[1].value());
        ws_signal(ws);
    }
}

template <class T>
__global__ void __launch_bounds__(kBlock) k_axpy_point(const T* __restrict__ xp, const T* __restrict__ d, T step,
                                                       T* __restrict__ x, int64_t n)
{
    constexpr int W = Vec16<T>::W;
    const int64_t nv = n / W;
    const int64_t stride = int64_t(gridDim.x) * kBlock;
    for (int64_t vi = int64_t(blockIdx.x) * kBlock + threadIdx.x; vi < nv; vi += stride)
    {
        const Pack<T> pxp = ldv(xp, vi), pd = ldv(d, vi);
        Pack<T> px;
#pragma unroll
        for (int k = 0; k < W; k++)
            px.e[k] = pxp.e[k] + step * pd.e[k];
        stv(x, vi, px);
    }
    if (blockIdx.x == 0 && threadIdx.x == 0)
        for (int64_t i = nv * W; i < n; i++)
            x[i] = xp[i] + step * d[i];
}

template <class T>
__global__ void __launch_bounds__(kBlock) k_dot(const T* __restrict__ u, const T* __restrict__ v,
                                                const T* __restrict__ w, int64_t n, RedWs ws,
                                                T* __restrict__ out)
{
    typedef typename AccOf<T>::type A;
    constexpr int W = Vec16<T>::W;
    A acc[2];
    const int64_t nv = n / W;
    const int64_t stride = int64_t(gridDim.x) * kBlock;
    for (int64_t vi = int64_t(blockIdx.x) * kBlock + threadIdx.x; vi < nv; vi += stride)
    {
        const Pack<T> pu = ldv(u, vi), pv = ldv(v, vi);
#pragma unroll
        for (int k = 0; k < W; k++)
            acc[0].add_prod(pu.e[k], pv.e[k]);
        if (w)
        {
            const Pack<T> pw = ldv(w, vi);
#pragma unroll
            for (int k = 0; k < W; k++)
                acc[1].add_prod(pw.e[k], pw.e[k]);
        }
    }
    if (blockIdx.x == 0 && threadIdx.x == 0)
        for (int64_t i = nv * W; i < n; i++)
        {
            acc[0].add_prod(u[i], v[i]);
            if (w)
                acc[1].add_prod(w[i], w[i]);
        }
    if (grid_reduce<2>(acc, ws) && threadIdx.x == 0)
    {
        out[0] = T(acc[0].value());
        out[1] = T(acc[1].value());
    }
}

template <class T, int U = 4>
__global__ void __launch_bounds__(kBlock) k_post(const T* __restrict__ x, const T* __restrict__ xp,
                                                 const T* __restrict__ g, const T* __restrict__ gp,
                                                 T* __restrict__ s, T* __restrict__ y, int64_t n, RedWs ws,
                                                 T* __restrict__ out, T* __restrict__ ys_slot,
                                                 T* __restrict__ theta_slot, int rev)
{
    typedef typename AccOf<T>::type A;
    constexpr int W = Vec16<T>::W;
    A acc[4];
    const int64_t nv = n / W;
    const int64_t tile = int64_t(kBlock) * U;
    const int64_t top = ((nv + tile - 1) / tile - 1) * tile;
    for (int64_t t0 = int64_t(blockIdx.x) * tile; t0 < nv; t0 += int64_t(gridDim.x) * tile)
    {
        const int64_t base = (rev ? top - t0 : t0) + threadIdx.x;
        Pack<T> px[U], pxp[U], pg[U], pgp[U];
#pragma unroll
        for (int u = 0; u < U; u++)
            if (base + u * kBlock < nv)
            {
                px[u] = ldv(x, base + u * kBlock);
// ... 168 lines not shown
#pragma unroll
    for (int k = 0; k < CH; k++)
    {
        const int64_t vi = int64_t(k) * vstride + vbase;
        const int64_t vc = vi < nv ? vi : int64_t(0);
        pu[k] = ldv<T, true>(u, vc);
        pw[k] = ldv<T, true>(w, vc);
    }
}
template <class T, int NR, int NL, class A, bool PRE = false, int CH = kHvChunk>
__device__ __forceinline__ void hv_step(Pack<T> (&rq)[NR], typename Vec16<T>::type* lq, const T* u, const T* w,
                                        bool init, T a, T c, T theta, int64_t nv, int64_t vbase, int64_t vstride,
                                        int ltid, A (&acc)[4], const Pack<T>* pre_u = nullptr, const Pack<T>* pre_w = nullptr)
{
    constexpr int W = Vec16<T>::W;
    constexpr int U = CH;
#pragma unroll
    for (int s0 = 0; s0 < NR + NL; s0 += U)
    {
        Pack<T> pu[U], pw[U];
        bool ok[U];
#pragma unroll
        for (int k = 0; k < U; k++)
            if (s0 + k < NR + NL)
            {
                const int64_t vi = int64_t(s0 + k) * vstride + vbase;
                ok[k] = vi < nv;
                const int64_t vc = ok[k] ? vi : int64_t(0);
                if (PRE && s0 == 0)
                {
                    pu[k] = pre_u[k];
                    pw[k] = pre_w[k];
                }
                else
                {
                    pu[k] = ldv<T, true>(u, vc);
                    pw[k] = ldv<T, true>(w, vc);
                }
            }
#pragma unroll
        for (int k = 0; k < U; k++)
            if (s0 + k < NR + NL)
            {
                constexpr int dummy = 0;
                const int s = s0 + k;
                Pack<T> cur;
                if (s < NR)
                    cur = rq[s < NR ? s : dummy];
                else
                    cur.v = lq[(s < NR ? dummy : s - NR) * kHvThreads + ltid];
#pragma unroll
                for (int e = 0; e < W; e++)
                {
                    const T upd = cur.e[e] + c * pu[k].e[e];
                    const T ini = a * pu[k].e[e];
                    cur.e[e] = init ? ini : upd;
                }
#pragma unroll
                for (int e = 0; e < W; e++)
                    cur.e[e] = cur.e[e] / theta;
#pragma unroll
                for (int e = 0; e < W; e++)
                    acc[(k * W + e) & 3].add_prod(ok[k] ? pw[k].e[e] : T(0), ok[k] ? cur.e[e] : T(0));
                if (s < NR)
                    rq[s < NR ? s : dummy] = cur;
                else
                    lq[(s < NR ? dummy : s - NR) * kHvThreads + ltid] = cur.v;
            }
        asm volatile("" ::: "memory");
        __builtin_amdgcn_sched_barrier(0);
    }
}

constexpr int kPersistMaxM = 128;
struct PersistArgs
{
    int ncorr, m;
    int pcol[kPersistMaxM];
    unsigned gen_base;
    int zigzag;
    unsigned first_rev;
    int64_t ld;
    int pub_first;
};

constexpr int kSc1 = 16;

template <class T>
struct PostFuse
{
    const T* x;
    const T* xp;
    const T* gp;
    T* s;
    T* y;
    T* out;
    T* ys_slot;
    T* theta_slot;
    T eps;
    int* verdict;
};

template <class T, int NR, int NL, class A, int PU = 2>
__device__ __forceinline__ void hv_post_step(Pack<T> (&rq)[NR], typename Vec16<T>::type* lq, const PostFuse<T>& pf,
                                             const T* g, T a, int64_t nv, int64_t bbase, int64_t vstride, int ltid,
                                             A (&acc)[5])
{
    const int64_t vbase = bbase + ltid;
    constexpr int W = Vec16<T>::W;
    constexpr int U = PU;
    const __amdgpu_buffer_rsrc_t rs = __builtin_amdgcn_make_buffer_rsrc(pf.s + W * bbase, 0, 0x40000000, 0x00020000);
    const __amdgpu_buffer_rsrc_t ry = __builtin_amdgcn_make_buffer_rsrc(pf.y + W * bbase, 0, 0x40000000, 0x00020000);
#pragma unroll
    for (int s0 = 0; s0 < NR + NL; s0 += U)
    {
        Pack<T> px[U], pxp[U], pg[U], pgp[U];
        bool ok[U];
#pragma unroll
        for (int k = 0; k < U; k++)
            if (s0 + k < NR + NL)
            {
                const int64_t vi = int64_t(s0 + k) * vstride + vbase;
                ok[k] = vi < nv;
                const int64_t vc = ok[k] ? vi : int64_t(0);
                px[k] = ldv<T, true>(pf.x, vc);
                pxp[k] = ldv<T, true>(pf.xp, vc);
                pg[k] = ldv<T, true>(g, vc);
                pgp[k] = ldv<T, true>(pf.gp, vc);
            }
#pragma unroll
        for (int k = 0; k < U; k++)
            if (s0 + k < NR + NL)
            {
                constexpr int dummy = 0;
                const int s = s0 + k;
                Pack<T> ps, py, cur;
#pragma unroll
                for (int e = 0; e < W; e++)
                {
                    ps.e[e] = px[k].e[e] - pxp[k].e[e];
                    py.e[e] = pg[k].e[e] - pgp[k].e[e];
                    cur.e[e] = a * pg[k].e[e];
                }
                const int soff = int(int64_t(s) * vstride * 16);
                const int voff = ok[k] ? ltid * 16 : 0x7FFFFFF0;
                __builtin_amdgcn_raw_buffer_store_b128(__builtin_bit_cast(i4_t, ps.v), rs, voff, soff, kSc1);
                __builtin_amdgcn_raw_buffer_store_b128(__builtin_bit_cast(i4_t, py.v), ry, voff, soff, kSc1);
#pragma unroll
                for (int e = 0; e < W; e++)
                {
                    const T zg = ok[k] ? pg[k].e[e] : T(0), zx = ok[k] ? px[k].e[e] : T(0);
                    const T zs = ok[k] ? ps.e[e] : T(0), zy = ok[k] ? py.e[e] : T(0);
                    acc[0].add_prod(zg, zg);
                    acc[1].add_prod(zx, zx);
                    acc[2].add_prod(zs, zy);
                    acc[3].add_prod(zy, zy);
                    acc[4].add_prod(zs, cur.e[e]);
                }
                if (s < NR)
                    rq[s < NR ? s : dummy] = cur;
                else
                    lq[(s < NR ? dummy : s - NR) * kHvThreads + ltid] = cur.v;
            }
        asm volatile("" ::: "memory");
        __builtin_amdgcn_sched_barrier(0);
    }
// ... 61 lines not shown
        w.w = int(unsigned(bh >> 32));
        __builtin_amdgcn_raw_buffer_store_b128(w, r, int(((2 * tid + 0) * G + blockIdx.x) * 16), 0, kSc1);
        w.z = int(unsigned(bl & 0xFFFFFFFFull));
        w.w = int(unsigned(bl >> 32));
        __builtin_amdgcn_raw_buffer_store_b128(w, r, int(((2 * tid + 1) * G + blockIdx.x) * 16), 0, kSc1);
    }
    if (blockIdx.x != 0)
        return false;
    if (tid == 0)
        s_bad = 0;
    __syncthreads();
    A t[NRED];
    bool bad = false;
    for (int b = tid; b < G && !bad; b += kHvThreads)
    {
        i4_t w[2 * NRED];
        unsigned spins = 0;
        const unsigned long long t_begin = wall_clock64();
        for (;;)
        {
            asm volatile("" ::: "memory");
            bool all = true;
#pragma unroll
            for (int j = 0; j < 2 * NRED; j++)
                w[j] = __builtin_amdgcn_raw_buffer_load_b128(r, int((j * G + b) * 16), 0, kSc1);
#pragma unroll
            for (int j = 0; j < 2 * NRED; j++)
                all = all && (unsigned(w[j].x) == tag);
            if (all)
                break;
            __builtin_amdgcn_s_sleep(1);
            if ((++spins & 1023u) == 0u &&
                (wall_clock64() - t_begin > 10000000ull || __hip_atomic_load(err, __ATOMIC_RELAXED, __HIP_MEMORY_SCOPE_AGENT) != 0))
            {
                __hip_atomic_store(err, 1, __ATOMIC_RELAXED, __HIP_MEMORY_SCOPE_AGENT);
                bad = true;
                break;
            }
        }
        auto dbl = [](const i4_t& v) {
            return __longlong_as_double((long long) ((unsigned long long) unsigned(v.z) | ((unsigned long long) unsigned(v.w) << 32)));
        };
        if (!bad)
#pragma unroll
            for (int j = 0; j < NRED; j++)
                t[j].merge(dbl(w[2 * j]), dbl(w[2 * j + 1]));
    }
    if (bad)
        s_bad = 1;
    mine = block_reduce_all<NRED, A>(t, sh);
    if (tid < NRED)
    {
        sfin[tid][0] = mine.hi;
        sfin[tid][1] = acc_lo(mine);
    }
    __syncthreads();
    if (tid == 0)
#pragma unroll
        for (int k = 0; k < NRED; k++)
        {
            A z;
            z.hi = sfin[k][0];
            z.lo = sfin[k][1];
            acc[k] = z;
        }
    return s_bad == 0;
}

template <class T, bool FUSE = false, bool MEET = false>
__global__ void __launch_bounds__(kHvThreads, 2)
    k_twoloop_persist(T* __restrict__ q, const T* __restrict__ vin, T a, const T* __restrict__ S, const T* __restrict__ Y,
                      int64_t n, T* __restrict__ sc, PersistArgs pa, RedWs ws, unsigned* __restrict__ gen,
                      int* __restrict__ err, PostFuse<T> pf)
{
    typedef typename AccOf<T>::type A;
    constexpr int W = Vec16<T>::W;
    constexpr int NR = kPersistNR, NL = kPersistNL, U = 4;
    __shared__ typename Vec16<T>::type lq[NL * kHvThreads];
    __shared__ int s_pcol[kPersistMaxM];
    __shared__ int s_verdict;
    __shared__ T s_dotv[MEET ? kPersistMaxM + 1 : 1];
    __shared__ T s_ys[MEET ? kPersistMaxM : 1];
    __shared__ T s_theta0;
    const int tid = threadIdx.x;
    if (tid < kPersistMaxM)
        s_pcol[tid] = pa.pcol[tid];
    if (tid == 0)
        s_verdict = __hip_atomic_load(err, __ATOMIC_RELAXED, __HIP_MEMORY_SCOPE_AGENT);
    __syncthreads();
    if (s_verdict != 0)
        return;
    __syncthreads();
    const int cn = pa.ncorr, m = pa.m;
    const int64_t nv = n / W;
    const int64_t gthreads = int64_t(gridDim.x) * kHvThreads;
    const int64_t gtid = int64_t(blockIdx.x) * kHvThreads + tid;
    int64_t nres = (nv + gthreads - 1) / gthreads;
    if (nres > NR + NL)
        nres = NR + NL;
    const int64_t res_end = nres * gthreads < nv ? nres * gthreads : nv;
    const int DOT0 = 2 * (m + 1) + 1;
    auto sload = [&](int idx) { return T(__hip_atomic_load(sc + idx, __ATOMIC_RELAXED, __HIP_MEMORY_SCOPE_AGENT)); };
    if (MEET)
    {
        if (tid < cn)
            s_ys[tid] = sload(s_pcol[tid]);
        if (tid == 0)
            s_theta0 = cn > 0 ? sload(m + 1 + s_pcol[0]) : T(1);
        __syncthreads();
    }
    auto dslot = [&](int k) { return MEET ? (k < cn ? k : cn) : 0; };
    auto dotv = [&](int k) { return MEET ? s_dotv[dslot(k)] : sload(DOT0 + k); };
    auto ysv = [&](int i) { return MEET ? s_ys[MEET ? i : 0] : sload(s_pcol[i]); };
    auto col = [&](const T* base, int c) { return base + int64_t(c) * pa.ld; };

    Pack<T> rq[NR];
    const int64_t tile = int64_t(kHvThreads) * U;
    if (FUSE)
    {
        A accp[5];
        hv_post_step<T, NR, NL>(rq, lq, pf, vin, a, res_end, int64_t(blockIdx.x) * kHvThreads, gthreads, tid, accp);
        {
            const bool rev = pa.zigzag && ((pa.first_rev & 1u) != 0u);
            const int64_t span = nv - res_end;
            const int64_t ntile = (span + tile - 1) / tile;
            for (int64_t t0 = blockIdx.x; t0 < ntile; t0 += gridDim.x)
            {
                const int64_t tt = rev ? ntile - 1 - t0 : t0;
                const int64_t base = res_end + tt * tile + tid;
                const int64_t eoff = W * (res_end + tt * tile);
                const __amdgpu_buffer_rsrc_t rq_ = __builtin_amdgcn_make_buffer_rsrc(const_cast<T*>(q) + eoff, 0, int(tile * 16), 0x00020000);
                const __amdgpu_buffer_rsrc_t rs_ = __builtin_amdgcn_make_buffer_rsrc(pf.s + eoff, 0, int(tile * 16), 0x00020000);
                const __amdgpu_buffer_rsrc_t ry_ = __builtin_amdgcn_make_buffer_rsrc(pf.y + eoff, 0, int(tile * 16), 0x00020000);
                Pack<T> px[U], pxp[U], pg[U], pgp[U];
#pragma unroll
                for (int k = 0; k < U; k++)
                {
                    const int64_t vi = base + int64_t(k) * kHvThreads;
                    if (vi < nv)
                    {
                        px[k] = ldv<T, true>(pf.x, vi);
                        pxp[k] = ldv<T, true>(pf.xp, vi);
                        pg[k] = ldv<T, true>(vin, vi);
                        pgp[k] = ldv<T, true>(pf.gp, vi);
                    }
                }
#pragma unroll
                for (int k = 0; k < U; k++)
                {
                    const int64_t vi = base + int64_t(k) * kHvThreads;
                    if (vi < nv)
                    {
                        Pack<T> ps, py, cur;
#pragma unroll
                        for (int e = 0; e < W; e++)
                        {
                            ps.e[e] = px[k].e[e] - pxp[k].e[e];
                            py.e[e] = pg[k].e[e] - pgp[k].e[e];
                            cur.e[e] = a * pg[k].e[e];
                            accp[0].add_prod(pg[k].e[e], pg[k].e[e]);
                            accp[1].add_prod(px[k].e[e], px[k].e[e]);
                            accp[2].add_prod(ps.e[e], py.e[e]);
                            accp[3].add_prod(py.e[e], py.e[e]);
                            accp[4].add_prod(ps.e[e], cur.e[e]);
                        }
                        const int boff = int((tid + k * kHvThreads) * 16);
                        __builtin_amdgcn_raw_buffer_store_b128(__builtin_bit_cast(i4_t, ps.v), rs_, boff, 0, kSc1);
                        __builtin_amdgcn_raw_buffer_store_b128(__builtin_bit_cast(i4_t, py.v), ry_, boff, 0, kSc1);
                        __builtin_amdgcn_raw_buffer_store_b128(__builtin_bit_cast(i4_t, cur.v), rq_, boff, 0, kSc1);
                    }
                }
            }
            if (blockIdx.x == 0 && tid == 0)
                for (int64_t i = nv * W; i < n; i++)
                {
                    const T si = pf.x[i] - pf.xp[i], yi = vin[i] - pf.gp[i], qi = a * vin[i];
                    __hip_atomic_store(pf.s + i, si, __ATOMIC_RELAXED, __HIP_MEMORY_SCOPE_AGENT);
                    __hip_atomic_store(pf.y + i, yi, __ATOMIC_RELAXED, __HIP_MEMORY_SCOPE_AGENT);
                    q[i] = qi;
                    accp[0].add_prod(vin[i], vin[i]);
                    accp[1].add_prod(pf.x[i], pf.x[i]);
                    accp[2].add_prod(si, yi);
                    accp[3].add_prod(yi, yi);
                    accp[4].add_prod(si, qi);
                }
            asm volatile("s_waitcnt vmcnt(0)" ::: "memory");
        }
        const unsigned want0 = pa.gen_base + 1u;
        if (MEET)
        {
            const bool lastb = persist_gather<5, A>(accp, gen, want0, err);
            if (tid == 0)
            {
// ... 12 lines not shown
                    __hip_atomic_store(pf.theta_slot, yy / sy, __ATOMIC_RELAXED, __HIP_MEMORY_SCOPE_AGENT);
                    __hip_atomic_store(sc + DOT0, d0, __ATOMIC_RELAXED, __HIP_MEMORY_SCOPE_AGENT);
                    __hip_atomic_store(pf.verdict, (sy > pf.eps * yy) ? 1 : 2, __ATOMIC_RELAXED, __HIP_MEMORY_SCOPE_AGENT);
                    if (!(sy > pf.eps * yy))
                    {
                        __hip_atomic_store(pf.out + 5, T(2), __ATOMIC_RELAXED, __HIP_MEMORY_SCOPE_SYSTEM);
                        ws_signal(ws);
                    }
                    persist_publish(gen + 8, want0, double(sy));
                    persist_publish(gen + 12, want0, double(yy));
                    asm volatile("s_waitcnt vmcnt(0)" ::: "memory");
                    persist_publish(gen + 4, want0, double(d0));
                }
                else
                {
                    double v0 = 0.0, v1 = 0.0, v2 = 0.0;
                    ok = persist_await(gen + 4, want0, err, v0);
                    if (ok)
                        ok = persist_await(gen + 8, want0, err, v1) && persist_await(gen + 12, want0, err, v2);
                    d0 = T(v0);
                    sy = T(v1);
                    yy = T(v2);
                }
                s_ys[0] = sy;
                s_theta0 = yy / sy;
                s_dotv[0] = d0;
                s_verdict = !ok ? 2 : ((sy > pf.eps * yy) ? 1 : 2);
            }
            __syncthreads();
            if (s_verdict != 1)
                return;
        }
        else
        {
        if (grid_reduce<5>(accp, ws))
        {
            if (tid == 0)
            {
                const T sy = T(accp[2].value()), yy = T(accp[3].value());
                pf.out[0] = T(accp[0].value());
                pf.out[1] = T(accp[1].value());
                pf.out[2] = sy;
                pf.out[3] = yy;
                __hip_atomic_store(pf.ys_slot, sy, __ATOMIC_RELAXED, __HIP_MEMORY_SCOPE_AGENT);
                __hip_atomic_store(pf.theta_slot, yy / sy, __ATOMIC_RELAXED, __HIP_MEMORY_SCOPE_AGENT);
                __hip_atomic_store(sc + DOT0, T(accp[4].value()), __ATOMIC_RELAXED, __HIP_MEMORY_SCOPE_AGENT);
                __hip_atomic_store(pf.verdict, (sy > pf.eps * yy) ? 1 : 2, __ATOMIC_RELAXED, __HIP_MEMORY_SCOPE_AGENT);
                asm volatile("s_waitcnt vmcnt(0)" ::: "memory");
                __hip_atomic_store(gen, want0, __ATOMIC_RELEASE, __HIP_MEMORY_SCOPE_AGENT);
            }
        }
        if (tid == 0)
        {
            unsigned spins = 0;
            bool gave_up = false;
            const unsigned long long t_begin = wall_clock64();
            while (int(__hip_atomic_load(gen, __ATOMIC_RELAXED, __HIP_MEMORY_SCOPE_AGENT) - want0) < 0)
            {
                __builtin_amdgcn_s_sleep(8);
                if ((++spins & 255u) == 0u &&
                    (wall_clock64() - t_begin > 10000000ull ||
                     __hip_atomic_load(err, __ATOMIC_RELAXED, __HIP_MEMORY_SCOPE_AGENT) != 0))
                {
                    __hip_atomic_store(err, 1, __ATOMIC_RELAXED, __HIP_MEMORY_SCOPE_AGENT);
                    gave_up = true;
                    break;
                }
            }
            s_verdict = gave_up ? 2 : __hip_atomic_load(pf.verdict, __ATOMIC_RELAXED, __HIP_MEMORY_SCOPE_AGENT);
        }
        __syncthreads();
        if (s_verdict != 1)
            return;
        }
    }
    bool was_last = false;
    for (int L = FUSE ? 1 : 0; L <= 2 * cn; L++)
    {
        const T* u;
        const T* w;
        if (L == 0)
        {
            u = vin;
            w = cn > 0 ? col(S, s_pcol[0]) : vin;
        }
        else if (L < cn)
        {
            u = col(Y, s_pcol[L - 1]);
            w = col(S, s_pcol[L]);
        }
        else if (L == cn)
        {
            u = col(Y, s_pcol[cn - 1]);
            w = u;
        }
        else
        {
            const int t = L - cn - 1, i = cn - 1 - t;
            u = col(S, s_pcol[i]);
            w = (t < cn - 1) ? col(Y, s_pcol[i - 1]) : vin;
        }
        int64_t gt = gtid;
        asm volatile("" : "+v"(gt));
        Pack<T> pu0[kHvChunk], pw0[kHvChunk];
        if (MEET)
        {
            hv_prefetch<T>(u, w, res_end, gt, gthreads, pu0, pw0);
            if (L > (FUSE ? 1 : 0))
            {
                if (tid == 0 && !was_last)
                {
                    double dv = 0.0;
                    (void) persist_await(gen + 4, pa.gen_base + unsigned(L), err, dv);
                    s_dotv[dslot(L - 1)] = T(dv);
                }
                __syncthreads();
            }
        }
        T c = T(0), theta = T(1);
        bool div = false;
        if (L == 0)
            ;
        else if (L < cn)
            c = -(dotv(L - 1) / ysv(L - 1));
        else if (L == cn)
        {
            c = -(dotv(cn - 1) / ysv(cn - 1));
            theta = MEET ? s_theta0 : sload(m + 1 + s_pcol[0]);
            div = true;
        }
        else
        {
            const int i = cn - 1 - (L - cn - 1);
            c = dotv(i) / ysv(i) - dotv(L - 1) / ysv(i);
        }
        A acc4[4];
        hv_step<T, NR, NL, A, MEET>(rq, lq, u, w, L == 0, a, c, theta, res_end, gt, gthreads, tid, acc4, pu0, pw0);
        {
            const bool rev = pa.zigzag && (((pa.first_rev + unsigned(L)) & 1u) != 0u);
            const int64_t span = nv - res_end;
            const int64_t ntile = (span + tile - 1) / tile;
            for (int64_t t0 = blockIdx.x; t0 < ntile; t0 += gridDim.x)
            {
                const int64_t tt = rev ? ntile - 1 - t0 : t0;
                const int64_t base = res_end + tt * tile + tid;
                const __amdgpu_buffer_rsrc_t rq = __builtin_amdgcn_make_buffer_rsrc(
                    const_cast<T*>(q) + W * (res_end + tt * tile), 0, int(tile * 16), 0x00020000);
                Pack<T> pq[U], pu[U], pw[U];
#pragma unroll
                for (int k = 0; k < U; k++)
                {
                    const int64_t vi = base + int64_t(k) * kHvThreads;
                    if (vi < nv)
                    {
                        pu[k] = ldv<T, true>(u, vi);
                        pw[k] = ldv<T, true>(w, vi);
                        if (L != 0)
                            pq[k].v = __builtin_bit_cast(typename Vec16<T>::type,
                                                         __builtin_amdgcn_raw_buffer_load_b128(rq, int((tid + k * kHvThreads) * 16), 0, kSc1));
                    }
                }
#pragma unroll
                for (int k = 0; k < U; k++)
                {
                    const int64_t vi = base + int64_t(k) * kHvThreads;
                    if (vi < nv)
                    {
#pragma unroll
                        for (int e = 0; e < W; e++)
                        {
                            T qv = (L == 0) ? a * pu[k].e[e] : pq[k].e[e] + c * pu[k].e[e];
                            if (div)
                                qv = qv / theta;
                            pq[k].e[e] = qv;
                            acc4[(k * W + e) & 3].add_prod(pw[k].e[e], qv);
                        }
                        __builtin_amdgcn_raw_buffer_store_b128(__builtin_bit_cast(i4_t, pq[k].v), rq,
                                                               int((tid + k * kHvThreads) * 16), 0, kSc1);
                    }
                }
            }
            asm volatile("s_waitcnt vmcnt(0)" ::: "memory");
            if (blockIdx.x == 0 && tid == 0)
                for (int64_t i = nv * W; i < n; i++)
                {
                    T qv = (L == 0) ? a * u[i] : q[i] + c * u[i];
                    if (div)
                        qv = qv / theta;
                    q[i] = qv;
                    acc4[0].add_prod(w[i], qv);
                }
        }
        A acc[1];
        acc[0] = acc4[0];
        for (int k = 1; k < 4; k++)
            acc[0].merge(acc4[k].hi, acc_lo(acc4[k]));
        const unsigned want = pa.gen_base + unsigned(L) + 1u;
        if (MEET)
        {
            was_last = persist_gather<1, A>(acc, gen, want, err);
            if (was_last && tid == 0)
            {
                const T dv = T(acc[0].value());
                s_dotv[dslot(L)] = dv;
                if (pa.pub_first && L < 2 * cn)
                    persist_publish<false>(gen + 4, want, double(dv));
                __hip_atomic_store(sc + DOT0 + L, dv, __ATOMIC_RELAXED, __HIP_MEMORY_SCOPE_AGENT);
                if (!pa.pub_first && L < 2 * cn)
                    persist_publish(gen + 4, want, double(dv));
                if (FUSE && L == 2 * cn)
                {
                    __hip_atomic_store(pf.out + 4, dv, __ATOMIC_RELAXED, __HIP_MEMORY_SCOPE_SYSTEM);
                    __hip_atomic_store(pf.out + 5, T(1), __ATOMIC_RELAXED, __HIP_MEMORY_SCOPE_SYSTEM);
                    ws_signal(ws);
                }
            }
            continue;
        }
        if (grid_reduce<1>(acc, ws))
        {
            if (tid == 0)
            {
                __hip_atomic_store(sc + DOT0 + L, T(acc[0].value()), __ATOMIC_RELAXED, __HIP_MEMORY_SCOPE_AGENT);
                asm volatile("s_waitcnt vmcnt(0)" ::: "memory");
                __hip_atomic_store(gen, want, __ATOMIC_RELEASE, __HIP_MEMORY_SCOPE_AGENT);
            }
        }
        if (L < 2 * cn)
        {
            if (tid == 0)
            {
                unsigned spins = 0;
                const unsigned long long t_begin = wall_clock64();
                while (int(__hip_atomic_load(gen, __ATOMIC_RELAXED, __HIP_MEMORY_SCOPE_AGENT) - want) < 0)
                {
                    __builtin_amdgcn_s_sleep(8);
                    if ((++spins & 255u) == 0u &&
                        (wall_clock64() - t_begin > 10000000ull ||
                         __hip_atomic_load(err, __ATOMIC_RELAXED, __HIP_MEMORY_SCOPE_AGENT) != 0))
                    {
                        __hip_atomic_store(err, 1, __ATOMIC_RELAXED, __HIP_MEMORY_SCOPE_AGENT);
                        break;
                    }
                }
            }
            __syncthreads();
        }
    }
#pragma unroll
    for (int s = 0; s < NR + NL; s++)
    {
        const int64_t vi = int64_t(s) * gthreads + gtid;
        if (vi < res_end)
        {
            Pack<T> cur;
            if (s < NR)
                cur = rq[s < NR ? s : 0];
            else
                cur.v = lq[(s < NR ? 0 : s - NR) * kHvThreads + tid];
            stv<T, false>(q, vi, cur);
        }
    }
}

}
```

lbfgspp_amd/csrc/lbfgsx.hip:

```cpp
#include <dlfcn.h>

#include <algorithm>
#include <atomic>
#include <cmath>
#include <chrono>
#include <string>
#include <vector>
#include <utility>
#include <cstdio>
#include <cstdlib>
#include <cstring>
#include <limits>
#include <mutex>

#include "ctx.hpp"
#include "lbfgs_kernels.cuh"
#include "launch_args.hpp"

namespace lbfgsx {

static std::atomic<int> g_live[64];
Counters& counters()
{
    static Counters g;
// ... 235 lines not shown

}

using namespace lbfgsx;

static int create_fill(lbfgsx_ctx* c, int dtype, int64_t n, int m, int device, int flags);

extern "C" {

const char* lbfgsx_last_error(void) { return g_err.c_str(); }
const char* lbfgsx_version(void) { return "lbfgsx 0.1 (gfx950)"; }

int lbfgsx_device_count(void)
{
    int n = 0;
    if (hipGetDeviceCount(&n) != hipSuccess)
        return 0;
    return n;
}

int lbfgsx_create(lbfgsx_ctx** out, int dtype, int64_t n, int m, int device, int flags)
{
    if (!out || n <= 0 || m <= 0 || (dtype != LBFGSX_F64 && dtype != LBFGSX_F32))
    {
        set_error("lbfgsx_create: invalid argument");
        return LBFGSX_E_INVALID;
    }
    int ndev = 0;
    if (hipGetDeviceCount(&ndev) != hipSuccess || ndev <= 0)
    {
        set_error("lbfgsx_create: no HIP device available (this library has no CPU fallback)");
        return LBFGSX_E_NOGPU;
    }
    if (device < 0 || device >= ndev)
    {
        set_error("lbfgsx_create: device index out of range");
        return LBFGSX_E_INVALID;
    }
    lbfgsx::DeviceGuard dev_guard_(device);
    lbfgsx_ctx* c = new lbfgsx_ctx();
    *out = nullptr;
    const int rc = create_fill(c, dtype, n, m, device, flags);
    if (rc != LBFGSX_OK)
    {
        const std::string msg = lbfgsx_last_error();
        lbfgsx_destroy(c);
        (void) hipGetLastError();
        set_error(msg);
        return rc;
    }
    *out = c;
    return LBFGSX_OK;
}

}
static int create_fill(lbfgsx_ctx* c, int dtype, int64_t n, int m, int device, int flags)
{
    c->dtype = dtype;
    c->esz = (dtype == LBFGSX_F64) ? 8 : 4;
    c->n = n;
    c->n_global = n;
    c->ld = (n + 63) / 64 * 64;
    c->m = m;
    c->device = device;
    c->flags = flags;
    c->sl.m = m;
    LBFGSX_HIP(hipStreamCreateWithFlags(&c->stream, hipStreamNonBlocking));
    c->own_stream = true;
    {
        int64_t min_n = 4096;
        if (const char* e = getenv("LBFGSX_PERSIST_MIN_N"))
            min_n = atoll(e);
        if (n < min_n)
            c->persist = false;
    }
    if (const char* e = getenv("LBFGSX_PERSIST"))
        c->persist = atoi(e) != 0 && c->persist;
    if (const char* e = getenv("LBFGSX_MEET"))
        c->meet_all = std::strcmp(e, "last") != 0;
    if (const char* e = getenv("LBFGSX_PERSIST_POLL"))
        c->fast_persist_out = atoi(e) != 0;
    if (const char* e = getenv("LBFGSX_FUSE_POST"))
        c->fuse_post = atoi(e) != 0;
    {
        int occ = 0;
        hipDeviceProp_t prop;
        LBFGSX_HIP(hipGetDeviceProperties(&prop, device));
        if (dtype == LBFGSX_F64)
            (void) hipOccupancyMaxActiveBlocksPerMultiprocessor(&occ, k_twoloop_persist<double, true, true>, kHvThreads, 0);
        else
            (void) hipOccupancyMaxActiveBlocksPerMultiprocessor(&occ, k_twoloop_persist<float, true, true>, kHvThreads, 0);
        c->persist_grid = occ * prop.multiProcessorCount;
        c->gen_words = 16 + size_t(10) * size_t(c->persist_grid) * 4;
        LBFGSX_HIP(hipMalloc(reinterpret_cast<void**>(&c->gen_dev), c->gen_words * sizeof(unsigned)));
        LBFGSX_HIP(hipMemset(c->gen_dev, 0, c->gen_words * sizeof(unsigned)));
    }
    const size_t vbytes = size_t(c->ld) * c->esz;
    for (int k = 0; k < 3; k++)
    {
        LBFGSX_HIP(hipMalloc(&c->xb[k], vbytes));
        LBFGSX_HIP(hipMalloc(&c->gb[k], vbytes));
    }
    LBFGSX_HIP(hipMalloc(&c->d, vbytes));
    LBFGSX_HIP(hipMalloc(&c->a, vbytes));
    LBFGSX_HIP(hipMalloc(&c->b, vbytes));
    LBFGSX_HIP(hipMalloc(&c->S, vbytes * size_t(m + 1)));
    LBFGSX_HIP(hipMalloc(&c->Y, vbytes * size_t(m + 1)));
    LBFGSX_HIP(hipMalloc(&c->sc, sizeof(double) * size_t(c->sl.total())));
    LBFGSX_HIP(hipMemset(c->sc, 0, sizeof(double) * size_t(c->sl.total())));
    LBFGSX_HIP(hipHostMalloc(&c->hout, sizeof(double) * 64, hipHostMallocDefault));
    {
        const char* e = getenv("LBFGSX_MAPPED_OUT");
        if (e ? atoi(e) != 0 : true)
        {
            LBFGSX_HIP(hipHostMalloc(&c->outmap_host, sizeof(double) * 16, hipHostMallocMapped | hipHostMallocCoherent));
            std::memset(c->outmap_host, 0, sizeof(double) * 16);
            LBFGSX_HIP(hipHostGetDevicePointer(&c->outmap_dev, c->outmap_host, 0));
            const char* pe = getenv("LBFGSX_POLL");
            if (!(pe && atoi(pe) == 0))
            {
                LBFGSX_HIP(hipHostMalloc(reinterpret_cast<void**>(&c->done_host), 64, hipHostMallocMapped | hipHostMallocCoherent));
                std::memset(c->done_host, 0, 64);
                LBFGSX_HIP(hipHostGetDevicePointer(reinterpret_cast<void**>(&c->done_dev), c->done_host, 0));
            }
        }
    }
    c->ws.maxGrid = 8192;
    LBFGSX_HIP(hipMalloc(reinterpret_cast<void**>(&c->ws.partials), sizeof(double) * size_t(kMaxRed) * 2 * size_t(c->ws.maxGrid)));
    LBFGSX_HIP(hipMalloc(reinterpret_cast<void**>(&c->ws.ticket), sizeof(unsigned) * 4));
    LBFGSX_HIP(hipMemset(c->ws.ticket, 0, sizeof(unsigned) * 4));
    c->phys.assign(size_t(m), 0);
    c->ys_host.assign(size_t(m), 0.0);
    int rc = lbfgsx_bfgs_reset(c);
    if (rc != LBFGSX_OK)
        return rc;
    if (flags & LBFGSX_FLAG_BOUNDED)
    {
        if (m > LBFGSX_MAX_M_BOUNDED)
        {
            set_error("lbfgsx_create: an L-BFGS-B context supports m <= 40 history pairs");
            return LBFGSX_E_INVALID;
        }
        if (n > int64_t(2147483647))
        {
            set_error("lbfgsx_create: an L-BFGS-B context supports n < 2^31 coordinates");
            return LBFGSX_E_INVALID;
        }
        LBFGSX_HIP(hipMalloc(&c->lb, vbytes));
        LBFGSX_HIP(hipMalloc(&c->ub, vbytes));
        LBFGSX_HIP(hipMalloc(&c->xcp, vbytes));
        rc = bounded_alloc(c);
        if (rc != LBFGSX_OK)
            return rc;
    }
    LBFGSX_HIP(lbfgsx::stream_sync(c->stream));
    live_add(c->device, +1);
    c->counted = true;
    return LBFGSX_OK;
}
extern "C" {

void lbfgsx_destroy(lbfgsx_ctx* c)
{
    if (!c)
        return;
    lbfgsx::DeviceGuard dev_guard_(c->device);
// ... 95 lines not shown
    return LBFGSX_OK;
}

int lbfgsx_gather(lbfgsx_ctx* c, int which, int64_t stride, double* host)
{
    lbfgsx::DeviceGuard dev_guard_(c->device);
    void* p = vec_ptr(c, which);
    if (!p || !host || stride < 1)
    {
        set_error("lbfgsx_gather: invalid argument");
        return LBFGSX_E_INVALID;
    }
    const int64_t nsamp = (c->n + stride - 1) / stride;
    if (nsamp > c->gather_cap)
    {
        if (c->gather_tmp)
            LBFGSX_HIP(hipFree(c->gather_tmp));
        LBFGSX_HIP(hipMalloc(&c->gather_tmp, sizeof(double) * size_t(nsamp)));
        c->gather_cap = nsamp;
    }
    const int grid = int(std::min<int64_t>((nsamp + 255) / 256, 1024));
    DISPATCH_T(c, { LBFGSX_LAUNCH(k_gather<T>, dim3(grid), dim3(256), 0, c->stream, P<T>(p), nsamp, stride,
                                       static_cast<double*>(c->gather_tmp)); });
    LBFGSX_HIP(lbfgsx::copy_async(host, c->gather_tmp, sizeof(double) * size_t(nsamp), hipMemcpyDeviceToHost, c->stream));
    LBFGSX_HIP(lbfgsx::stream_sync(c->stream));
    return LBFGSX_OK;
}

int lbfgsx_set_shard(lbfgsx_ctx* c, int64_t offset, int64_t n_global)
{
    if (!c || offset < 0 || n_global < offset + c->n)
    {
        set_error("lbfgsx_set_shard: need 0 <= offset and offset + n <= n_global");
        return LBFGSX_E_INVALID;
    }
    c->shard_off = offset;
    c->n_global = n_global;
    return LBFGSX_OK;
}

int lbfgsx_gen_diag_quad(lbfgsx_ctx* c, double kappa, uint64_t seed)
{
    lbfgsx::DeviceGuard dev_guard_(c->device);
    c->spec_valid = false;
    DISPATCH_T(c, { LBFGSX_LAUNCH(k_gen_quad<T>, dim3(2048), dim3(256), 0, c->stream, P<T>(c->a), P<T>(c->b),
                                       c->n, kappa, seed, c->shard_off, c->n_global); });
    LBFGSX_HIP(hipGetLastError());
    return LBFGSX_OK;
}

int lbfgsx_gen_rosen_x0(lbfgsx_ctx* c, uint64_t seed)
{
    lbfgsx::DeviceGuard dev_guard_(c->device);
    c->spec_valid = false;
    DISPATCH_T(c, { LBFGSX_LAUNCH(k_gen_rosen<T>, dim3(2048), dim3(256), 0, c->stream, P<T>(c->xb[c->cur]),
                                       c->n, seed, c->shard_off); });
    LBFGSX_HIP(hipGetLastError());
    return LBFGSX_OK;
}

int lbfgsx_fill(lbfgsx_ctx* c, int which, double value)
{
    lbfgsx::DeviceGuard dev_guard_(c->device);
    c->spec_valid = false;
    void* p = vec_ptr(c, which);
    if (!p)
    {
        set_error("lbfgsx_fill: unknown vector");
        return LBFGSX_E_INVALID;
    }
    DISPATCH_T(c, { LBFGSX_LAUNCH(k_fill<T>, dim3(2048), dim3(256), 0, c->stream, P<T>(p), c->n, T(value)); });
    LBFGSX_HIP(hipGetLastError());
    return LBFGSX_OK;
}

int lbfgsx_bfgs_reset(lbfgsx_ctx* c)
{
    lbfgsx::DeviceGuard dev_guard_(c->device);
    c->theta = 1.0;
    c->ncorr = 0;
    c->ptr = c->m;
    c->pending = false;
    c->spec_valid = false;
    c->tl_step = 0;
    for (int j = 0; j < c->m; j++)
        c->phys[size_t(j)] = j;
    c->phys_version++;
    c->spare = c->m;
    DISPATCH_T(c, {
        T one = T(1);
        LBFGSX_HIP(lbfgsx::copy_async(P<T>(c->sc) + c->sl.one(), &one, sizeof(T), hipMemcpyHostToDevice, c->stream));
        LBFGSX_HIP(lbfgsx::stream_sync(c->stream));
    });
    return LBFGSX_OK;
}

int lbfgsx_bfgs_ncorr(const lbfgsx_ctx* c) { return c->ncorr; }
double lbfgsx_bfgs_theta(const lbfgsx_ctx* c) { return c->theta; }

int lbfgsx_bfgs_download_history(lbfgsx_ctx* c, void* S_out, void* Y_out, int* ncorr, int* ptr, double* theta)
{
    lbfgsx::DeviceGuard dev_guard_(c->device);
    if (c->gs_f32h)
    {
        set_error("lbfgsx_bfgs_download_history: this context keeps its history in f32 for the Gram-space recursion (lbfgsx_gs_set_history_dtype)");
        return LBFGSX_E_LOGIC;
    }
    for (int j = 0; j < c->ncorr; j++)
    {
        const size_t bytes = size_t(c->n) * c->esz;
        LBFGSX_HIP(lbfgsx::copy_async(static_cast<char*>(S_out) + size_t(j) * bytes, c->col(c->S, c->phys[size_t(j)]), bytes,
                                  hipMemcpyDeviceToHost, c->stream));
        LBFGSX_HIP(lbfgsx::copy_async(static_cast<char*>(Y_out) + size_t(j) * bytes, c->col(c->Y, c->phys[size_t(j)]), bytes,
                                  hipMemcpyDeviceToHost, c->stream));
    }
    LBFGSX_HIP(lbfgsx::stream_sync(c->stream));
    if (ncorr) *ncorr = c->ncorr;
    if (ptr) *ptr = c->ptr;
    if (theta) *theta = c->theta;
    return LBFGSX_OK;
}

int lbfgsx_commit_correction(lbfgsx_ctx* c)
{
    lbfgsx::DeviceGuard dev_guard_(c->device);
    if (!c->pending)
    {
        set_error("lbfgsx_commit_correction: no pending (s, y) pair");
        return LBFGSX_E_LOGIC;
    }
    const int loc = c->ptr % c->m;
    const int old = c->phys[size_t(loc)];
    c->phys[size_t(loc)] = c->spare;
    c->phys_version++;
    c->spare = old;
    c->ys_host[size_t(loc)] = c->pend_sy;
    DISPATCH_T(c, { c->theta = double(T(T(c->pend_yy) / T(c->pend_sy))); });
    if (c->ncorr < c->m)
        c->ncorr++;
    c->ptr = loc + 1;
    c->pending = false;
    return LBFGSX_OK;
}

int lbfgsx_bfgs_stage_correction_host(lbfgsx_ctx* c, const void* s, const void* y, double* sy, double* yy)
{
    lbfgsx::DeviceGuard dev_guard_(c->device);
    c->spec_valid = false;
    if (c->gs_f32h)
    {
        set_error("lbfgsx_bfgs_stage_correction_host: this context keeps its history in f32 for the Gram-space recursion (lbfgsx_gs_set_history_dtype)");
        return LBFGSX_E_LOGIC;
    }
    void* sp = c->col(c->S, c->spare);
    void* yp = c->col(c->Y, c->spare);
    LBFGSX_HIP(lbfgsx::copy_async(sp, s, size_t(c->n) * c->esz, hipMemcpyHostToDevice, c->stream));
    LBFGSX_HIP(lbfgsx::copy_async(yp, y, size_t(c->n) * c->esz, hipMemcpyHostToDevice, c->stream));
    if (c->bstate)
    {
        const int rcn = bounded_note_column(c, c->spare);
        if (rcn)
            return rcn;
    }
    const int grid = c->grid_for(c->n);
    double r[2];
    DISPATCH_T(c, {
        LBFGSX_LAUNCH((k_dot<T>), dim3(grid), dim3(kBlock), 0, c->stream, P<T>(sp), P<T>(yp), P<T>(yp), c->n,
                           c->ws, c->out_slot<T>());
        int rc = fetch_scalars<T>(c, c->sl.out(0), 2, r);
        if (rc)
            return rc;
        T vals[2] = {T(r[0]), T(T(r[1]) / T(r[0]))};
        LBFGSX_HIP(lbfgsx::copy_async(P<T>(c->sc) + c->sl.ys(c->spare), &vals[0], sizeof(T), hipMemcpyHostToDevice, c->stream));
        LBFGSX_HIP(lbfgsx::copy_async(P<T>(c->sc) + c->sl.theta(c->spare), &vals[1], sizeof(T), hipMemcpyHostToDevice, c->stream));
        LBFGSX_HIP(lbfgsx::stream_sync(c->stream));
    });
    c->pend_sy = r[0];
    c->pend_yy = r[1];
    c->pending = true;
    if (sy) *sy = r[0];
    if (yy) *yy = r[1];
    return LBFGSX_OK;
}

int lbfgsx_bfgs_add_correction_host(lbfgsx_ctx* c, const void* s, const void* y)
{
    lbfgsx::DeviceGuard dev_guard_(c->device);
    int rc = lbfgsx_bfgs_stage_correction_host(c, s, y, nullptr, nullptr);
    if (rc)
        return rc;
    return lbfgsx_commit_correction(c);
}

}
template <class T>
static int apply_Hv_t(lbfgsx_ctx* c, const T* v, T a, double* dg)
{
    const int cn = c->ncorr, m = c->m;
    const int grid = std::min(c->grid_for(c->n, 4), kGridCapTwoloop);
    T* q = P<T>(c->d);
    T* sc = P<T>(c->sc);
    const T* gcur = P<T>(c->gb[c->cur]);
    const ScLayout& sl = c->sl;
    std::vector<int> pcol(size_t(cn > 0 ? cn : 1));
    {
        int j = c->ptr % m;
        for (int i = 0; i < cn; i++)
        {
            j = (j + m - 1) % m;
            pcol[i] = c->phys[size_t(j)];
        }
    }
    EventPair hv;
    if (c->timing)
    {
        LBFGSX_HIP(hipEventCreate(&hv.a));
        LBFGSX_HIP(hipEventCreate(&hv.b));
        LBFGSX_HIP(hipEventRecord(hv.a, c->stream));
    }
    std::unique_lock<std::mutex> persist_lock;
    if (c->persist && c->persist_cooldown == 0 && c->persist_grid > 0 && m <= kPersistMaxM && c->device >= 0 && c->device < 64)
        persist_lock = std::unique_lock<std::mutex>(g_persist_mu[c->device], std::try_to_lock);
    if (persist_lock.owns_lock())
    {
        PersistArgs pa;
        pa.ncorr = cn;
        pa.m = m;
        for (int i = 0; i < kPersistMaxM; i++)
            pa.pcol[i] = i < cn ? pcol[i] : 0;
        pa.gen_base = c->gen_count;
        pa.zigzag = 1;
        pa.first_rev = c->tl_step;
        pa.pub_first = 1;
        pa.ld = c->ld;
        c->gen_count += unsigned(2 * cn + 1);
        c->tl_step += unsigned(2 * cn + 1);
        if (c->meet_all)
            LBFGSX_LAUNCH((k_twoloop_persist<T, false, true>), dim3(c->persist_grid), dim3(kHvThreads), 0, c->stream, q, v, a,
                               P<T>(c->S), P<T>(c->Y), c->n, sc, pa, c->ws, c->gen_dev, reinterpret_cast<int*>(c->gen_dev + 1),
                               PostFuse<T>());
        else
            LBFGSX_LAUNCH((k_twoloop_persist<T, false, false>), dim3(c->persist_grid), dim3(kHvThreads), 0, c->stream, q, v, a,
                               P<T>(c->S), P<T>(c->Y), c->n, sc, pa, c->ws, c->gen_dev, reinterpret_cast<int*>(c->gen_dev + 1),
                               PostFuse<T>());
        LBFGSX_HIP(hipGetLastError());
        int* err = reinterpret_cast<int*>(c->gen_dev + 1);
        c->persist_launches++;
        if (c->timing)
        {
            LBFGSX_HIP(hipEventRecord(hv.b, c->stream));
            c->ev_hv.push_back(hv);
            c->persist_steps_timed += 2 * cn + 1;
        }
        int herr = 0;
        LBFGSX_HIP(lbfgsx::copy_async(&herr, err, sizeof(int), hipMemcpyDeviceToHost, c->stream));
        int rc2 = dg ? fetch_scalars<T>(c, sl.dot(2 * cn), 1, dg) : LBFGSX_OK;
        if (!dg)
            LBFGSX_HIP(lbfgsx::stream_sync(c->stream));
        if (herr)
        {
            LBFGSX_HIP(hipMemsetAsync(c->gen_dev, 0, c->gen_words * sizeof(unsigned), c->stream));
            LBFGSX_HIP(hipMemsetAsync(c->ws.ticket, 0, sizeof(unsigned), c->stream));
            c->gen_count = 0;
            persist_timed_out(c);
            persist_lock.unlock();
            if (c->timing && !c->ev_hv.empty())
            {
                (void) hipEventDestroy(c->ev_hv.back().a);
                (void) hipEventDestroy(c->ev_hv.back().b);
                c->ev_hv.pop_back();
                c->persist_steps_timed -= 2 * cn + 1;
            }
            return apply_Hv_t<T>(c, v, a, dg);
        }
        c->persist_backoff = 8;
        return rc2;
    }
    c->step_products++;
    if (c->persist_cooldown > 0)
        c->persist_cooldown--;
    auto launch = [&](int mode, const T* u, const T* w, TwoLoopArgs args) -> int {
        EventPair ev;
        args.rev = (c->tl_step++ & 1u) ? 1 : 0;
        if (c->timing && c->timing_per_launch)
        {
            LBFGSX_HIP(hipEventCreate(&ev.a));
            LBFGSX_HIP(hipEventCreate(&ev.b));
            LBFGSX_HIP(hipEventRecord(ev.a, c->stream));
        }
#define TL_LAUNCH(MODE) \
    LBFGSX_LAUNCH((k_twoloop<T, MODE>), dim3(grid), dim3(kBlock), 0, c->stream, q, v, a, u, w, c->n, sc, args, c->ws)
        switch (mode)
        {
        case TL_INIT: TL_LAUNCH(TL_INIT); break;
        case TL_SUB: TL_LAUNCH(TL_SUB); break;
        case TL_SUBDIV: TL_LAUNCH(TL_SUBDIV); break;
        default: TL_LAUNCH(TL_ADD); break;
        }
#undef TL_LAUNCH
        if (c->timing && c->timing_per_launch)
        {
            LBFGSX_HIP(hipEventRecord(ev.b, c->stream));
            c->ev_twoloop.push_back(ev);
        }
        return LBFGSX_OK;
    };
    auto Scol = [&](int i) { return static_cast<const T*>(c->col(c->S, pcol[i])); };
    auto Ycol = [&](int i) { return static_cast<const T*>(c->col(c->Y, pcol[i])); };
    int rc;
    TwoLoopArgs args = {0, 0, 0, 0, 0, 0};
    if (cn == 0)
    {
        args.i_out = sl.dot(0);
        if ((rc = launch(TL_INIT, nullptr, gcur, args)))
            return rc;
    }
    else
// ... 19 lines not shown
        {
            const int i = cn - 1 - t, L = cn + 1 + t;
            args.i_num = sl.dot(i);
            args.i_num2 = sl.dot(L - 1);
            args.i_den = sl.ys(pcol[i]);
            args.i_out = sl.dot(L);
            if ((rc = launch(TL_ADD, Scol(i), (t < cn - 1) ? Ycol(i - 1) : gcur, args)))
                return rc;
        }
    }
    LBFGSX_HIP(hipGetLastError());
    if (c->timing)
    {
        LBFGSX_HIP(hipEventRecord(hv.b, c->stream));
        c->ev_hv.push_back(hv);
        if (!c->timing_per_launch)
            c->coarse_steps_timed += 2 * cn + 1;
    }
    if (dg)
        return fetch_scalars<T>(c, sl.dot(2 * cn), 1, dg);
    return LBFGSX_OK;
}
extern "C" {

int lbfgsx_apply_Hv(lbfgsx_ctx* c, int v_which, double a, double* dg)
{
    lbfgsx::DeviceGuard dev_guard_(c->device);
    void* v = vec_ptr(c, v_which);
    if (!v || v == c->d)
    {
        set_error("lbfgsx_apply_Hv: invalid source vector");
        return LBFGSX_E_INVALID;
    }
    if (c->gs_f32h && c->ncorr > 0)
    {
        set_error("lbfgsx_apply_Hv: this context keeps its history in f32 for the Gram-space recursion (lbfgsx_gs_set_history_dtype)");
        return LBFGSX_E_LOGIC;
    }
    if (c->spec_valid)
    {
        const bool hit = c->spec_version == c->phys_version && !c->pending && v == c->gb[c->spec_cur] &&
                         c->spec_cur == c->cur && a == c->spec_a;
        c->spec_valid = false;
        if (hit)
        {
            c->spec_used++;
            if (dg) *dg = c->spec_dg;
            return LBFGSX_OK;
        }
    }
    DISPATCH_T(c, { return apply_Hv_t<T>(c, P<T>(v), T(a), dg); });
    return LBFGSX_OK;
}

}
template <class T, class OBJ>
static int eval_t(lbfgsx_ctx* c, OBJ obj, double* out3)
{
    const lbfgsx::EvalLaunch<T> a = lbfgsx::eval_launch<T>(c);
    LBFGSX_LAUNCH((k_eval<T, OBJ>), dim3(a.grid), dim3(kBlock), 0, c->stream, a.x, a.g, a.n, obj, a.ws, a.out);
    LBFGSX_HIP(hipGetLastError());
    return fetch_scalars<T>(c, c->sl.out(0), 3, out3);
}
template <class T>
static int eval_term_t(lbfgsx_ctx* c, double* out3)
{
    lbfgsx::EvalLaunch<T> a = lbfgsx::eval_launch<T>(c);
    lbfgsx::BoundArgs<T> obj(c);
    void* params[] = {&a.x, &a.g, &a.n, obj.ptr, &a.ws, &a.out};
    int rc = lbfgsx::linear_pre_eval<T>(c, obj, a.x);
    if (rc)
        return rc;
    rc = lbfgsx::jit_launch(c, lbfgsx::JIT_K_EVAL, lbfgsx::linear_col_grid(c, a.grid), params);
    if (rc)
        return rc;
    return fetch_scalars<T>(c, c->sl.out(0), 3, out3);
}
extern "C" {

int lbfgsx_eval(lbfgsx_ctx* c, int objective, double* fx, double* gnorm2, double* xnorm2)
{
    lbfgsx::DeviceGuard dev_guard_(c->device);
    c->spec_valid = false;
    double r[3];
    int rc = LBFGSX_E_INVALID;
    if (objective == LBFGSX_OBJ_EXT_ROSENBROCK && (c->n & 1))
    {
        set_error("extended Rosenbrock needs an even dimension");
        return LBFGSX_E_INVALID;
    }
    DISPATCH_T(c, {
        if (objective == LBFGSX_OBJ_DIAG_QUAD)
            rc = eval_t<T>(c, ObjQuad<T>{P<T>(c->a), P<T>(c->b)}, r);
        else if (objective == LBFGSX_OBJ_EXT_ROSENBROCK)
            rc = eval_t<T>(c, ObjRosen<T>{}, r);
        else if (lbfgsx::term_bound(c, objective))
            rc = eval_term_t<T>(c, r);
        else
            set_error("lbfgsx_eval: unknown objective");
    });
    if (rc)
        return rc;
    if (fx) *fx = r[0];
    if (gnorm2) *gnorm2 = r[1];
    if (xnorm2) *xnorm2 = r[2];
    return LBFGSX_OK;
}

int lbfgsx_norms(lbfgsx_ctx* c, double* gnorm2, double* xnorm2)
{
    lbfgsx::DeviceGuard dev_guard_(c->device);
    const int grid = c->grid_for(c->n);
    double r[2];
    DISPATCH_T(c, {
        const T* g = P<T>(c->gb[c->cur]);
        LBFGSX_LAUNCH((k_dot<T>), dim3(grid), dim3(kBlock), 0, c->stream, g, g, P<T>(c->xb[c->cur]), c->n, c->ws,
                           c->out_slot<T>());
        int rc = fetch_scalars<T>(c, c->sl.out(0), 2, r);
        if (rc)
            return rc;
    });
    if (gnorm2) *gnorm2 = r[0];
    if (xnorm2) *xnorm2 = r[1];
    return LBFGSX_OK;
}

int lbfgsx_ls_begin(lbfgsx_ctx* c)
{
    c->st_valid = false;
    c->xp = c->cur;
    c->lo = c->xp;
    c->trial = (c->xp + 1) % 3;
    return LBFGSX_OK;
}

}
template <class T, class OBJ>
static int trial_t(lbfgsx_ctx* c, OBJ obj, T step, double* out2)
{
    const lbfgsx::TrialLaunch<T> a = lbfgsx::trial_launch<T>(c, step, sizeof(OBJ) >= 2 * sizeof(void*) ? 2 : 0);
    LBFGSX_LAUNCH((k_trial<T, OBJ>), dim3(a.grid), dim3(kBlock), 0, c->stream, a.xp, a.d, a.step, a.x, a.g, a.n, obj, a.ws,
                       a.out, a.rev);
    LBFGSX_HIP(hipGetLastError());
    return fetch_scalars<T>(c, c->sl.out(0), 2, out2);
}
template <class T>
static int trial_term_t(lbfgsx_ctx* c, T step, double* out2)
{
    lbfgsx::TrialLaunch<T> a = lbfgsx::trial_launch<T>(c, step, c->term_np);
    lbfgsx::BoundArgs<T> obj(c);
    lbfgsx::graph_model_add<T>(c, 2);
    lbfgsx::mesh_model_add<T>(c, 2);
    void* params[] = {&a.xp, &a.d, &a.step, &a.x, &a.g, &a.n, obj.ptr, &a.ws, &a.out, &a.rev};
    int rc = lbfgsx::linear_pre_trial<T>(c, obj, a.xp, a.d, a.step);
    if (rc)
        return rc;
    rc = lbfgsx::jit_launch(c, lbfgsx::JIT_K_TRIAL, lbfgsx::linear_col_grid(c, a.grid), params);
    if (rc)
        return rc;
    return fetch_scalars<T>(c, c->sl.out(0), 2, out2);
}
extern "C" {

int lbfgsx_trial(lbfgsx_ctx* c, int objective, double step, double* fx, double* dg)
{
    lbfgsx::DeviceGuard dev_guard_(c->device);
    c->spec_valid = false;
    double r[2];
    int rc = LBFGSX_E_INVALID;
    if (c->st_valid)
    {
        c->st_valid = false;
        bool same = objective == c->st_obj && c->xp == c->st_xp && c->trial == c->st_trial;
        DISPATCH_T(c, { same = same && T(step) == T(c->st_step); });
        if (same)
        {
            c->st_hits++;
            c->tl_step++;
            if (fx) *fx = c->st_f;
            if (dg) *dg = c->st_dg;
            return LBFGSX_OK;
        }
        c->st_cooldown = 4;
    }
    DISPATCH_T(c, {
        if (objective == LBFGSX_OBJ_DIAG_QUAD)
            rc = trial_t<T>(c, ObjQuad<T>{P<T>(c->a), P<T>(c->b)}, T(step), r);
        else if (objective == LBFGSX_OBJ_EXT_ROSENBROCK)
            rc = trial_t<T>(c, ObjRosen<T>{}, T(step), r);
        else if (lbfgsx::term_bound(c, objective))
            rc = trial_term_t<T>(c, T(step), r);
        else
            set_error("lbfgsx_trial: unknown objective");
    });
    if (rc)
        return rc;
    if (fx) *fx = r[0];
    if (dg) *dg = r[1];
    return LBFGSX_OK;
}

int lbfgsx_trial_point(lbfgsx_ctx* c, double step)
{
    lbfgsx::DeviceGuard dev_guard_(c->device);
    c->spec_valid = false;
    const int grid = c->grid_for(c->n);
    DISPATCH_T(c, {
        LBFGSX_LAUNCH((k_axpy_point<T>), dim3(grid), dim3(kBlock), 0, c->stream, P<T>(c->xb[c->xp]), P<T>(c->d),
                           T(step), P<T>(c->xb[c->trial]), c->n);
    });
    LBFGSX_HIP(hipGetLastError());
    return LBFGSX_OK;
}

int lbfgsx_trial_dg(lbfgsx_ctx* c, double* dg)
{
    lbfgsx::DeviceGuard dev_guard_(c->device);
    const int grid = c->grid_for(c->n);
    DISPATCH_T(c, {
        LBFGSX_LAUNCH((k_dot<T>), dim3(grid), dim3(kBlock), 0, c->stream, P<T>(c->gb[c->trial]), P<T>(c->d),
                           static_cast<const T*>(nullptr), c->n, c->ws, c->out_slot<T>());
        LBFGSX_HIP(hipGetLastError());
        return fetch_scalars<T>(c, c->sl.out(0), 1, dg);
    });
    return LBFGSX_OK;
}

int lbfgsx_ls_keep_trial_as_lo(lbfgsx_ctx* c)
{
    if (c->lo == c->xp)
    {
        c->lo = c->trial;
        c->trial = third_point(c->xp, c->lo);
    }
    else
        std::swap(c->lo, c->trial);
    return LBFGSX_OK;
}

int lbfgsx_ls_end(lbfgsx_ctx* c, int use_lo)
{
    c->cur = use_lo ? c->lo : c->trial;
    return LBFGSX_OK;
}

int lbfgsx_post_linesearch(lbfgsx_ctx* c, double* gnorm2, double* xnorm2, double* sy, double* yy)
{
    lbfgsx::DeviceGuard dev_guard_(c->device);
    c->spec_valid = false;
    if (c->gs_f32h)
    {
        set_error("lbfgsx_post_linesearch: this context keeps its history in f32 for the Gram-space recursion (lbfgsx_gs_set_history_dtype)");
        return LBFGSX_E_LOGIC;
    }
    const int grid = c->grid_for(c->n);
    double r[4];
    DISPATCH_T(c, {
        const int rev = (c->tl_step++ & 1u) ? 1 : 0;
        LBFGSX_LAUNCH((k_post<T, 4>), dim3(grid), dim3(kBlock), 0, c->stream, P<T>(c->xb[c->cur]), P<T>(c->xb[c->xp]),
                           P<T>(c->gb[c->cur]), P<T>(c->gb[c->xp]), P<T>(c->col(c->S, c->spare)),
                           P<T>(c->col(c->Y, c->spare)), c->n, c->ws, c->out_slot<T>(), P<T>(c->sc) + c->sl.ys(c->spare),
                           P<T>(c->sc) + c->sl.theta(c->spare), rev);
        LBFGSX_HIP(hipGetLastError());
        int rc = fetch_scalars<T>(c, c->sl.out(0), 4, r);
        if (rc)
            return rc;
    });
    c->pend_sy = r[2];
    c->pend_yy = r[3];
    c->pending = true;
    if (gnorm2) *gnorm2 = r[0];
    if (xnorm2) *xnorm2 = r[1];
    if (sy) *sy = r[2];
    if (yy) *yy = r[3];
    return LBFGSX_OK;
}

}
template <class T>
static int post_spec_t(lbfgsx_ctx* c, T a, double* r4)
{
    const int m = c->m;
    if (!(c->fuse_post && c->persist && c->persist_cooldown == 0 && c->persist_grid > 0 && m <= kPersistMaxM && !c->gs_f32h && c->device >= 0 &&
          c->device < 64))
        return 1;
    std::unique_lock<std::mutex> lock(g_persist_mu[c->device], std::try_to_lock);
    if (!lock.owns_lock())
        return 1;
    const int loc = c->ptr % m;
    const int cn = std::min(c->ncorr + 1, m);
    PersistArgs pa;
    pa.ncorr = cn;
    pa.m = m;
    for (int i = 0; i < kPersistMaxM; i++)
        pa.pcol[i] = 0;
    {
        int j = loc;
        for (int i = 0; i < cn; i++)
        {
            pa.pcol[i] = (j == loc) ? c->spare : c->phys[size_t(j)];
            j = (j + m - 1) % m;
        }
    }
    pa.gen_base = c->gen_count;
    pa.zigzag = 1;
    pa.first_rev = c->tl_step;
    pa.pub_first = 1;
    pa.ld = c->ld;
    c->gen_count += unsigned(2 * cn + 1);
    c->tl_step += unsigned(2 * cn + 1);
    T* sc = P<T>(c->sc);
    PostFuse<T> pf;
    pf.x = P<T>(c->xb[c->cur]);
    pf.xp = P<T>(c->xb[c->xp]);
    pf.gp = P<T>(c->gb[c->xp]);
    pf.s = P<T>(c->col(c->S, c->spare));
    pf.y = P<T>(c->col(c->Y, c->spare));
    pf.out = c->out_slot<T>();
    pf.ys_slot = sc + c->sl.ys(c->spare);
    pf.theta_slot = sc + c->sl.theta(c->spare);
    pf.eps = std::numeric_limits<T>::epsilon();
    pf.verdict = reinterpret_cast<int*>(c->gen_dev + 2);
    EventPair hv;
    if (c->timing)
    {
        LBFGSX_HIP(hipEventCreate(&hv.a));
        LBFGSX_HIP(hipEventCreate(&hv.b));
        LBFGSX_HIP(hipEventRecord(hv.a, c->stream));
    }
    const bool fast_out = c->meet_all && c->outmap_dev && c->done_host && !c->poll_off && c->fast_persist_out;
    if (fast_out)
    {
        static_cast<volatile T*>(c->outmap_host)[5] = T(0);
        lbfgsx::poll_arm(c);
    }
    if (c->meet_all)
        LBFGSX_LAUNCH((k_twoloop_persist<T, true, true>), dim3(c->persist_grid), dim3(kHvThreads), 0, c->stream, P<T>(c->d),
                           P<T>(c->gb[c->cur]), a, P<T>(c->S), P<T>(c->Y), c->n, sc, pa, c->ws, c->gen_dev,
                           reinterpret_cast<int*>(c->gen_dev + 1), pf);
    else
        LBFGSX_LAUNCH((k_twoloop_persist<T, true, false>), dim3(c->persist_grid), dim3(kHvThreads), 0, c->stream, P<T>(c->d),
                           P<T>(c->gb[c->cur]), a, P<T>(c->S), P<T>(c->Y), c->n, sc, pa, c->ws, c->gen_dev,
                           reinterpret_cast<int*>(c->gen_dev + 1), pf);
    LBFGSX_HIP(hipGetLastError());
    if (c->timing)
    {
        LBFGSX_HIP(hipEventRecord(hv.b, c->stream));
        c->ev_hv.push_back(hv);
        c->persist_steps_timed += 2 * cn + 1;
        c->fused_timed++;
    }
    int hflags[2] = {0, 0};
    double dgv = 0.0;
    bool have = false;
    if (fast_out)
    {
        const unsigned long long want = c->done_seq;
        LBFGSX_HIP(lbfgsx::poll_wait(c));
        const volatile T* o = static_cast<const volatile T*>(c->outmap_host);
        if (*static_cast<volatile unsigned long long*>(c->done_host) >= want && (o[5] == T(1) || o[5] == T(2)))
        {
            hflags[1] = int(o[5]);
            dgv = double(o[4]);
            for (int i = 0; i < 4; i++)
                r4[i] = double(o[i]);
            have = true;
        }
    }
    if (!have)
    {
        LBFGSX_HIP(lbfgsx::copy_async(hflags, c->gen_dev + 1, 2 * sizeof(int), hipMemcpyDeviceToHost, c->stream));
        T* h = static_cast<T*>(c->hout);
        LBFGSX_HIP(lbfgsx::copy_async(h, sc + c->sl.dot(2 * cn), sizeof(T), hipMemcpyDeviceToHost, c->stream));
        if (!c->outmap_dev)
            LBFGSX_HIP(lbfgsx::copy_async(h + 8, sc + c->sl.out(0), 4 * sizeof(T), hipMemcpyDeviceToHost, c->stream));
        LBFGSX_HIP(lbfgsx::stream_sync(c->stream));
        dgv = double(h[0]);
        for (int i = 0; i < 4; i++)
            r4[i] = c->outmap_dev ? double(static_cast<const volatile T*>(c->outmap_host)[i]) : double(h[8 + i]);
    }
    if (hflags[0])
    {
        LBFGSX_HIP(hipMemsetAsync(c->gen_dev, 0, c->gen_words * sizeof(unsigned), c->stream));
        LBFGSX_HIP(hipMemsetAsync(c->ws.ticket, 0, sizeof(unsigned), c->stream));
        c->gen_count = 0;
        persist_timed_out(c);
        if (c->timing && !c->ev_hv.empty())
        {
            (void) hipEventDestroy(c->ev_hv.back().a);
            (void) hipEventDestroy(c->ev_hv.back().b);
            c->ev_hv.pop_back();
            c->persist_steps_timed -= 2 * cn + 1;
            c->fused_timed--;
        }
        return 1;
    }
    c->persist_launches++;
    c->spec_launches++;
    c->persist_backoff = 8;
    if (hflags[1] == 1)
    {
        c->spec_valid = true;
        c->spec_version = c->phys_version + 1;
        c->spec_cur = c->cur;
        c->spec_a = double(a);
        c->spec_dg = dgv;
    }
    else
    {
        c->spec_rejected++;
        if (c->timing && !c->ev_hv.empty())
        {
            (void) hipEventDestroy(c->ev_hv.back().a);
            (void) hipEventDestroy(c->ev_hv.back().b);
            c->ev_hv.pop_back();
            c->persist_steps_timed -= 2 * cn + 1;
            c->fused_timed--;
        }
    }
    return LBFGSX_OK;
}
extern "C" {

int lbfgsx_post_linesearch_spec(lbfgsx_ctx* c, double a, double* gnorm2, double* xnorm2, double* sy, double* yy)
{
    lbfgsx::DeviceGuard dev_guard_(c->device);
    if (c->gs_f32h)
        return lbfgsx_post_linesearch(c, gnorm2, xnorm2, sy, yy);
    double r[4];
    int rc = 1;
    c->spec_valid = false;
    DISPATCH_T(c, { rc = post_spec_t<T>(c, T(a), r); });
    if (rc == 1)
        return lbfgsx_post_linesearch(c, gnorm2, xnorm2, sy, yy);
    if (rc)
        return rc;
    c->pend_sy = r[2];
    c->pend_yy = r[3];
    c->pending = true;
    if (gnorm2) *gnorm2 = r[0];
    if (xnorm2) *xnorm2 = r[1];
    if (sy) *sy = r[2];
    if (yy) *yy = r[3];
    return LBFGSX_OK;
}

int lbfgsx_spec_counts(const lbfgsx_ctx* c, int64_t out[3])
{
    out[0] = c->spec_launches;
    out[1] = c->spec_used;
    out[2] = c->spec_rejected;
    return LBFGSX_OK;
}

int lbfgsx_device(const lbfgsx_ctx* c) { return c ? c->device : -1; }

int lbfgsx_device_push(const lbfgsx_ctx* c, int* prev)
{
    int cur = -1;
    if (!c || !prev)
    {
        set_error("lbfgsx_device_push: null argument");
        return LBFGSX_E_INVALID;
    }
    LBFGSX_HIP(hipGetDevice(&cur));
    *prev = cur;
    if (cur != c->device)
        LBFGSX_HIP(hipSetDevice(c->device));
    return LBFGSX_OK;
}

int lbfgsx_device_pop(int prev)
{
    int cur = -1;
    if (prev < 0)
        return LBFGSX_OK;
    LBFGSX_HIP(hipGetDevice(&cur));
    if (cur != prev)
        LBFGSX_HIP(hipSetDevice(prev));
    return LBFGSX_OK;
}

int lbfgsx_persist_counts(const lbfgsx_ctx* c, int64_t out[4])
{
    out[0] = c->persist_launches;
    out[1] = c->persist_timeouts;
    out[2] = c->persist_cooldown;
    out[3] = c->step_products;
    return LBFGSX_OK;
}

int lbfgsx_debug_persist_fault(lbfgsx_ctx* c)
{
    lbfgsx::DeviceGuard dev_guard_(c->device);
    if (!c->gen_dev)
    {
        set_error("lbfgsx_debug_persist_fault: this context has no persistent launch");
        return LBFGSX_E_INVALID;
    }
    LBFGSX_HIP(hipMemsetAsync(c->gen_dev + 1, 1, 1, c->stream));
    return LBFGSX_OK;
}

int lbfgsx_poll_counts(const lbfgsx_ctx* c, int64_t out[2])
{
    if (!c || !out)
        return LBFGSX_E_INVALID;
    out[0] = c->poll_waits;
    out[1] = c->poll_timeouts;
    return LBFGSX_OK;
}

void lbfgsx_range_push(const char* name)
{
    Roctx& r = roctx_state();
    if (r.on && name)
        (void) r.push(name);
    if (lbfgsx::host_trace_on() && name)
        lbfgsx::host_trace(name);
}
void lbfgsx_range_pop(void)
{
    Roctx& r = roctx_state();
    if (r.on)
        (void) r.pop();
}
// ... 227 lines not shown
```

Before: 89.15 iterations/s.

## Fuse post-linesearch s/y update and reductions into first line-search trial kernel

When the previous line search accepted its first trial, the first trial of the next line search now runs a fused kernel. That kernel also computes s=x-xp and y=g-gp, writes them into history, and reduces gnorm, xnorm, s'y, y'y and the first two-loop dot product in the same pass. The persistent two-loop kernel gains a from_g mode that skips the first sweep and reads a*g directly, so the separate post-linesearch pass over x, g, xp and gp is removed when the trial is accepted. The cost is more registers and loads in the trial kernel, plus extra state tracking that must fall back correctly when the trial is rejected or the buffers differ.

```diff
diff --git a/include/LBFGS.h b/include/LBFGS.h
--- a/include/LBFGS.h
+++ b/include/LBFGS.h
@@ -118,6 +118,8 @@
         {
             detail::Range range_iteration("lbfgs:iteration");
             detail::check(lbfgsx_ls_begin(c));
+            if (!gram)
+                detail::check(lbfgsx_ls_post_in_trial(c, -1.0));
             const Scalar step_max = m_param.max_step;
             ev.trial_written = false;
             try
diff --git a/include/lbfgsx.h b/include/lbfgsx.h
--- a/include/lbfgsx.h
+++ b/include/lbfgsx.h
@@ -80,6 +80,8 @@
 int lbfgsx_commit_correction(lbfgsx_ctx* c);
 int lbfgsx_post_linesearch_spec(lbfgsx_ctx* c, double a, double* gnorm2, double* xnorm2, double* sy, double* yy);
 int lbfgsx_spec_counts(const lbfgsx_ctx* c, int64_t out[3]);
+int lbfgsx_ls_post_in_trial(lbfgsx_ctx* c, double a);
+int lbfgsx_post_in_trial_counts(const lbfgsx_ctx* c, int64_t out[4]);
 typedef struct lbfgsx_objective lbfgsx_objective;
 int lbfgsx_objective_compile(lbfgsx_objective** out, int dtype, int K, const char* body, char* log, size_t log_len);
 void lbfgsx_objective_destroy(lbfgsx_objective* obj);
diff --git a/lbfgspp_amd/_lib.py b/lbfgspp_amd/_lib.py
--- a/lbfgspp_amd/_lib.py
+++ b/lbfgspp_amd/_lib.py
@@ -117,6 +117,8 @@
     sig(core, "lbfgsx_device_download", i32, i32, vp, i64, vp)
     sig(core, "lbfgsx_device_free", None, i32, vp)
     sig(core, "lbfgsx_spec_counts", i32, vp, C.POINTER(i64 * 3))
+    sig(core, "lbfgsx_ls_post_in_trial", i32, vp, dbl)
+    sig(core, "lbfgsx_post_in_trial_counts", i32, vp, C.POINTER(i64 * 4))
     sig(core, "lbfgsx_counters", i32, C.POINTER(i64 * 3), i32)
     sig(core, "lbfgsx_counters_ex", i32, C.POINTER(i64 * 8), i32)
     sig(core, "lbfgsx_poll_counts", i32, vp, C.POINTER(i64 * 2))
diff --git a/lbfgspp_amd/csrc/ctx.hpp b/lbfgspp_amd/csrc/ctx.hpp
--- a/lbfgspp_amd/csrc/ctx.hpp
+++ b/lbfgspp_amd/csrc/ctx.hpp
@@ -201,9 +201,19 @@
     int spec_cur = 0;
     double spec_a = 0.0, spec_dg = 0.0;
     int64_t spec_launches = 0, spec_used = 0, spec_rejected = 0;
+    bool post_in_trial = true;
+    bool pt_armed = false;
+    double pt_a = 0.0;
+    int ls_trials = 0;
+    bool ls_first_ok = false;
+    bool pt_valid = false;
+    int pt_buf = -1, pt_xp = -1;
+    double pt_r[4] = {0, 0, 0, 0};
+    int64_t pt_issued = 0, pt_accepted = 0;
+    int64_t from_g_launches = 0;
 
     const struct lbfgsx_objective* term = nullptr;
-    void* term_fn[6] = {nullptr, nullptr, nullptr, nullptr, nullptr, nullptr};
+    void* term_fn[7] = {nullptr, nullptr, nullptr, nullptr, nullptr, nullptr, nullptr};
     const void* term_p[4] = {nullptr, nullptr, nullptr, nullptr};
     double term_c[8] = {0, 0, 0, 0, 0, 0, 0, 0};
     int term_np = 0;
diff --git a/lbfgspp_amd/csrc/jit_objective.hip b/lbfgspp_amd/csrc/jit_objective.hip
--- a/lbfgspp_amd/csrc/jit_objective.hip
+++ b/lbfgspp_amd/csrc/jit_objective.hip
@@ -16,7 +16,7 @@
 namespace {
 
 const char* const kKernelNames[6][lbfgsx::JIT_NSLOTS] = {
-    {"k_eval", "k_trial", "k_b_eval", "k_b_dg_maxstep_trial"},
+    {"k_eval", "k_trial", "k_b_eval", "k_b_dg_maxstep_trial", nullptr, nullptr, "k_trial_post"},
     {"k_chain_eval", "k_chain_trial", "k_chain_b_eval", "k_chain_b_dg_maxstep_trial"},
     {"k_grid_eval", "k_grid_trial", "k_grid_b_eval", "k_grid_b_dg_maxstep_trial"},
     {"k_graph_eval", "k_graph_trial", "k_graph_b_eval", "k_graph_b_dg_maxstep_trial"},
@@ -25,7 +25,7 @@
 const char* const kObjStruct[6] = {"ObjTerm", "ObjChain", "ObjGrid", "ObjGraph", "ObjMesh", "ObjLinear"};
 const char* const kFormName[6] = {"term objective", "chain objective", "grid objective", "graph objective", "mesh objective",
                                   "linear-model objective"};
-inline int kernels_of(int form) { return form == LBFGSX_FORM_LINEAR ? lbfgsx::JIT_NSLOTS : lbfgsx::JIT_NKERNELS; }
+inline bool has_kernel(int form, int k) { return k >= 0 && k < lbfgsx::JIT_NSLOTS && kKernelNames[form][k] != nullptr; }
 
 struct Rtc
 {
@@ -155,6 +155,8 @@
     s += "typedef term_scalar_t S;\n";
     s += "template __global__ void k_eval<S, ObjTerm>(const S*, S*, int64_t, ObjTerm, RedWs, S*);\n";
     s += "template __global__ void k_trial<S, ObjTerm>(const S*, const S*, S, S*, S*, int64_t, ObjTerm, RedWs, S*, int);\n";
+    s += "template __global__ void k_trial_post<S, ObjTerm>(const S*, const S*, S, S*, S*, int64_t, ObjTerm, RedWs, S*, int, "
+         "TrialPost<S>);\n";
     s += "template __global__ void k_b_eval<S, ObjTerm>(const S*, S*, const S*, const S*, int64_t, ObjTerm, RedWs, S*);\n";
     s += "template __global__ void k_b_dg_maxstep_trial<S, ObjTerm>(const S*, const S*, const S*, const S*, const S*, S, S*, S*, "
          "int64_t, ObjTerm, RedWs, S*, int);\n";
@@ -554,12 +556,12 @@
     int form = LBFGSX_FORM_TERM, dtype = LBFGSX_F64, K = 1, D = 1;
     std::vector<char> code;
     std::string lowered[lbfgsx::JIT_NSLOTS];
-    long long vgprs[lbfgsx::JIT_NSLOTS] = {0, 0, 0, 0, 0, 0}, scratch[lbfgsx::JIT_NSLOTS] = {0, 0, 0, 0, 0, 0};
+    long long vgprs[lbfgsx::JIT_NSLOTS] = {0, 0, 0, 0, 0, 0, 0}, scratch[lbfgsx::JIT_NSLOTS] = {0, 0, 0, 0, 0, 0, 0};
     double compile_ms = 0.0;
     struct Loaded
     {
         hipModule_t mod = nullptr;
-        hipFunction_t fn[lbfgsx::JIT_NSLOTS] = {nullptr, nullptr, nullptr, nullptr, nullptr, nullptr};
+        hipFunction_t fn[lbfgsx::JIT_NSLOTS] = {nullptr, nullptr, nullptr, nullptr, nullptr, nullptr, nullptr};
     };
     std::mutex mu;
     std::map<int, Loaded> loaded;
@@ -593,9 +595,11 @@
         return LBFGSX_E_RUNTIME;
     }
     std::string expr[lbfgsx::JIT_NSLOTS];
-    const int nk = kernels_of(form);
+    const int nk = lbfgsx::JIT_NSLOTS;
     for (int k = 0; k < nk; k++)
     {
+        if (!has_kernel(form, k))
+            continue;
         expr[k] = std::string("lbfgsx::") + kKernelNames[form][k] + "<lbfgsx::term_scalar_t, lbfgsx::" + kObjStruct[form] + ">";
         (void) r.add_name(prog, expr[k].c_str());
     }
@@ -634,6 +638,8 @@
     }
     for (int k = 0; ok && k < nk; k++)
     {
+        if (!has_kernel(form, k))
+            continue;
         const char* low = nullptr;
         ok = r.lowered(prog, expr[k].c_str(), &low) == HIPRTC_SUCCESS && low;
         if (ok)
@@ -806,8 +812,10 @@
         return LBFGSX_E_INVALID;
     const lbfgsx_objective_code* k = obj->code;
     out[0] = out[1] = 0;
-    for (int j = 0; j < kernels_of(k->form); j++)
-    {
+    for (int j = 0; j < lbfgsx::JIT_NSLOTS; j++)
+    {
+        if (!has_kernel(k->form, j))
+            continue;
         out[0] = k->vgprs[j] > out[0] ? k->vgprs[j] : out[0];
         out[1] = k->scratch[j] > out[1] ? k->scratch[j] : out[1];
         if (j < lbfgsx::JIT_NKERNELS)
@@ -918,8 +926,9 @@
         {
             lbfgsx_objective_code::Loaded l;
             LBFGSX_HIP(hipModuleLoadData(&l.mod, code->code.data()));
-            for (int k = 0; k < kernels_of(code->form); k++)
-                LBFGSX_HIP(hipModuleGetFunction(&l.fn[k], l.mod, code->lowered[k].c_str()));
+            for (int k = 0; k < lbfgsx::JIT_NSLOTS; k++)
+                if (has_kernel(code->form, k))
+                    LBFGSX_HIP(hipModuleGetFunction(&l.fn[k], l.mod, code->lowered[k].c_str()));
             it = code->loaded.emplace(c->device, l).first;
         }
         for (int k = 0; k < lbfgsx::JIT_NSLOTS; k++)
diff --git a/lbfgspp_amd/csrc/launch_args.hpp b/lbfgspp_amd/csrc/launch_args.hpp
--- a/lbfgspp_amd/csrc/launch_args.hpp
+++ b/lbfgspp_amd/csrc/launch_args.hpp
@@ -84,7 +84,8 @@
 }
 
 enum { JIT_K_EVAL = 0, JIT_K_TRIAL = 1, JIT_K_B_EVAL = 2, JIT_K_B_DG_MAXSTEP_TRIAL = 3, JIT_NKERNELS = 4 };
-enum { JIT_K_LIN_ROWS = 4, JIT_K_LIN_ROWS_TRIAL = 5, JIT_NSLOTS = 6 };
+enum { JIT_K_LIN_ROWS = 4, JIT_K_LIN_ROWS_TRIAL = 5 };
+enum { JIT_K_TRIAL_POST = 6, JIT_NSLOTS = 7 };
 template <class T>
 struct TermArgs
 {
diff --git a/lbfgspp_amd/csrc/lbfgs_kernels.cuh b/lbfgspp_amd/csrc/lbfgs_kernels.cuh
--- a/lbfgspp_amd/csrc/lbfgs_kernels.cuh
+++ b/lbfgspp_amd/csrc/lbfgs_kernels.cuh
@@ -100,28 +100,43 @@
     }
 }
 
-template <class T, class OBJ>
-__global__ void __launch_bounds__(kBlock) k_trial(const T* __restrict__ xp, const T* __restrict__ d, T step,
-                                                  T* __restrict__ x, T* __restrict__ g, int64_t n, OBJ obj,
-                                                  RedWs ws, T* __restrict__ out, int rev)
+template <class T>
+struct TrialPost
+{
+    const T* gp;
+    T* s;
+    T* y;
+    T a;
+    T* ys_slot;
+    T* theta_slot;
+    T* dot0;
+};
+
+template <class T, class OBJ, bool POST>
+__device__ __forceinline__ void trial_pass(const T* __restrict__ xp, const T* __restrict__ d, T step, T* __restrict__ x,
+                                           T* __restrict__ g, int64_t n, const OBJ& obj, const RedWs& ws,
+                                           T* __restrict__ out, int rev, const TrialPost<T>& tp)
 {
     typedef typename AccOf<T>::type A;
     constexpr int W = Vec16<T>::W;
     constexpr int U = 4;
-    A acc[2];
+    constexpr int NRED = POST ? 7 : 2;
+    A acc[NRED];
     const int64_t nv = n / W;
     const int64_t tile = int64_t(kBlock) * U;
     const int64_t top = ((nv + tile - 1) / tile - 1) * tile;
     for (int64_t t0 = int64_t(blockIdx.x) * tile; t0 < nv; t0 += int64_t(gridDim.x) * tile)
     {
         const int64_t base = (rev ? top - t0 : t0) + threadIdx.x;
-        Pack<T> pxp[U], pd[U];
+        Pack<T> pxp[U], pd[U], pgp[POST ? U : 1];
 #pragma unroll
         for (int u = 0; u < U; u++)
             if (base + u * kBlock < nv)
             {
                 pxp[u] = ldv(xp, base + u * kBlock);
                 pd[u] = ldv(d, base + u * kBlock);
+                if (POST)
+                    pgp[POST ? u : 0] = ldv(tp.gp, base + u * kBlock);
             }
 #pragma unroll
         for (int u = 0; u < U; u++)
@@ -139,6 +154,24 @@
 #pragma unroll
                 for (int k = 0; k < W; k++)
                     acc[1].add_prod(pg.e[k], pd[u].e[k]);
+                if (POST)
+                {
+                    Pack<T> ps, py;
+#pragma unroll
+                    for (int k = 0; k < W; k++)
+                    {
+                        ps.e[k] = px.e[k] - pxp[u].e[k];
+                        py.e[k] = pg.e[k] - pgp[POST ? u : 0].e[k];
+                        const T q0 = tp.a * pg.e[k];
+                        acc[POST ? 2 : 0].add_prod(pg.e[k], pg.e[k]);
+                        acc[POST ? 3 : 0].add_prod(px.e[k], px.e[k]);
+                        acc[POST ? 4 : 0].add_prod(ps.e[k], py.e[k]);
+                        acc[POST ? 5 : 0].add_prod(py.e[k], py.e[k]);
+                        acc[POST ? 6 : 0].add_prod(ps.e[k], q0);
+                    }
+                    stv(tp.s, vi, ps);
+                    stv(tp.y, vi, py);
+                }
             }
         }
     }
@@ -151,13 +184,51 @@
             obj.tail(i, n, x, g, acc[0]);
             acc[1].add_prod(g[i], d[i]);
         }
-    }
-    if (grid_reduce<2>(acc, ws) && threadIdx.x == 0)
+        if (POST)
+            for (int64_t i = nv * W; i < n; i++)
+            {
+                const T si = x[i] - xp[i], yi = g[i] - tp.gp[i], q0 = tp.a * g[i];
+                tp.s[i] = si;
+                tp.y[i] = yi;
+                acc[POST ? 2 : 0].add_prod(g[i], g[i]);
+                acc[POST ? 3 : 0].add_prod(x[i], x[i]);
+                acc[POST ? 4 : 0].add_prod(si, yi);
+                acc[POST ? 5 : 0].add_prod(yi, yi);
+                acc[POST ? 6 : 0].add_prod(si, q0);
+            }
+    }
+    if (grid_reduce<NRED>(acc, ws) && threadIdx.x == 0)
     {
         out[0] = obj.finish(T(acc[0].value()));
         out[1] = T(acc[1].value());
+        if (POST)
+        {
+            const T sy = T(acc[POST ? 4 : 0].value()), yy = T(acc[POST ? 5 : 0].value());
+            out[2] = T(acc[POST ? 2 : 0].value());
+            out[3] = T(acc[POST ? 3 : 0].value());
+            out[4] = sy;
+            out[5] = yy;
+            *tp.ys_slot = sy;
+            *tp.theta_slot = yy / sy;
+            *tp.dot0 = T(acc[POST ? 6 : 0].value());
+        }
         ws_signal(ws);
     }
+}
+
+template <class T, class OBJ>
+__global__ void __launch_bounds__(kBlock) k_trial(const T* __restrict__ xp, const T* __restrict__ d, T step,
+                                                  T* __restrict__ x, T* __restrict__ g, int64_t n, OBJ obj,
+                                                  RedWs ws, T* __restrict__ out, int rev)
+{
+    trial_pass<T, OBJ, false>(xp, d, step, x, g, n, obj, ws, out, rev, TrialPost<T>());
+}
+template <class T, class OBJ>
+__global__ void __launch_bounds__(kBlock) k_trial_post(const T* __restrict__ xp, const T* __restrict__ d, T step,
+                                                       T* __restrict__ x, T* __restrict__ g, int64_t n, OBJ obj,
+                                                       RedWs ws, T* __restrict__ out, int rev, TrialPost<T> tp)
+{
+    trial_pass<T, OBJ, true>(xp, d, step, x, g, n, obj, ws, out, rev, tp);
 }
 
 template <class T>
@@ -492,6 +563,7 @@
     unsigned first_rev;
     int64_t ld;
     int pub_first;
+    int from_g;
 };
 
 constexpr int kSc1 = 16;
@@ -719,9 +791,16 @@
     __shared__ T s_dotv[MEET ? kPersistMaxM + 1 : 1];
     __shared__ T s_ys[MEET ? kPersistMaxM : 1];
     __shared__ T s_theta0;
+    __shared__ unsigned long long s_sig[FUSE ? 1 : 3];
     const int tid = threadIdx.x;
     if (tid < kPersistMaxM)
         s_pcol[tid] = pa.pcol[tid];
+    if (!FUSE && tid == 0)
+    {
+        s_sig[0] = (unsigned long long) ws.done;
+        s_sig[FUSE ? 0 : 1] = ws.seq;
+        s_sig[FUSE ? 0 : 2] = (unsigned long long) pf.out;
+    }
     if (tid == 0)
         s_verdict = __hip_atomic_load(err, __ATOMIC_RELAXED, __HIP_MEMORY_SCOPE_AGENT);
     __syncthreads();
@@ -744,8 +823,11 @@
             s_ys[tid] = sload(s_pcol[tid]);
         if (tid == 0)
             s_theta0 = cn > 0 ? sload(m + 1 + s_pcol[0]) : T(1);
+        if (!FUSE && tid == 0 && pa.from_g)
+            s_dotv[0] = sload(DOT0);
         __syncthreads();
     }
+    const bool fromg = !FUSE && pa.from_g != 0;
     auto dslot = [&](int k) { return MEET ? (k < cn ? k : cn) : 0; };
     auto dotv = [&](int k) { return MEET ? s_dotv[dslot(k)] : sload(DOT0 + k); };
     auto ysv = [&](int i) { return MEET ? s_ys[MEET ? i : 0] : sload(s_pcol[i]); };
@@ -924,7 +1006,7 @@
         if (L == 0)
         {
             u = vin;
-            w = cn > 0 ? col(S, s_pcol[0]) : vin;
+            w = (cn > 0 && !fromg) ? col(S, s_pcol[0]) : vin;
         }
         else if (L < cn)
         {
@@ -948,7 +1030,7 @@
         if (MEET)
         {
             hv_prefetch<T>(u, w, res_end, gt, gthreads, pu0, pw0);
-            if (L > (FUSE ? 1 : 0))
+            if (L > ((FUSE || fromg) ? 1 : 0))
             {
                 if (tid == 0 && !was_last)
                 {
@@ -981,13 +1063,16 @@
         {
             const bool rev = pa.zigzag && (((pa.first_rev + unsigned(L)) & 1u) != 0u);
             const int64_t span = nv - res_end;
-            const int64_t ntile = (span + tile - 1) / tile;
+            const bool g1 = fromg && L == 1;
+            const int64_t ntile = (fromg && L == 0) ? 0 : (span + tile - 1) / tile;
             for (int64_t t0 = blockIdx.x; t0 < ntile; t0 += gridDim.x)
             {
                 const int64_t tt = rev ? ntile - 1 - t0 : t0;
                 const int64_t base = res_end + tt * tile + tid;
                 const __amdgpu_buffer_rsrc_t rq = __builtin_amdgcn_make_buffer_rsrc(
                     const_cast<T*>(q) + W * (res_end + tt * tile), 0, int(tile * 16), 0x00020000);
+                const __amdgpu_buffer_rsrc_t rl = __builtin_amdgcn_make_buffer_rsrc(
+                    const_cast<T*>(g1 ? vin : q) + W * (res_end + tt * tile), 0, int(tile * 16), 0x00020000);
                 Pack<T> pq[U], pu[U], pw[U];
 #pragma unroll
                 for (int k = 0; k < U; k++)
@@ -999,9 +1084,15 @@
                         pw[k] = ldv<T, true>(w, vi);
                         if (L != 0)
                             pq[k].v = __builtin_bit_cast(typename Vec16<T>::type,
-                                                         __builtin_amdgcn_raw_buffer_load_b128(rq, int((tid + k * kHvThreads) * 16), 0, kSc1));
+                                                         __builtin_amdgcn_raw_buffer_load_b128(rl, int((tid + k * kHvThreads) * 16), 0, kSc1));
                     }
                 }
+                if (g1)
+#pragma unroll
+                    for (int k = 0; k < U; k++)
+#pragma unroll
+                        for (int e = 0; e < W; e++)
+                            pq[k].e[e] = a * pq[k].e[e];
 #pragma unroll
                 for (int k = 0; k < U; k++)
                 {
@@ -1023,16 +1114,18 @@
                 }
             }
             asm volatile("s_waitcnt vmcnt(0)" ::: "memory");
-            if (blockIdx.x == 0 && tid == 0)
+            if (blockIdx.x == 0 && tid == 0 && !(fromg && L == 0))
                 for (int64_t i = nv * W; i < n; i++)
                 {
-                    T qv = (L == 0) ? a * u[i] : q[i] + c * u[i];
+                    T qv = (L == 0) ? a * u[i] : (g1 ? a * vin[i] : q[i]) + c * u[i];
                     if (div)
                         qv = qv / theta;
                     q[i] = qv;
                     acc4[0].add_prod(w[i], qv);
                 }
         }
+        if (fromg && L == 0)
+            continue;
         A acc[1];
         acc[0] = acc4[0];
         for (int k = 1; k < 4; k++)
@@ -1050,6 +1143,16 @@
                 __hip_atomic_store(sc + DOT0 + L, dv, __ATOMIC_RELAXED, __HIP_MEMORY_SCOPE_AGENT);
                 if (!pa.pub_first && L < 2 * cn)
                     persist_publish(gen + 4, want, double(dv));
+                if (!FUSE && fromg && L == 2 * cn)
+                {
+                    T* o = reinterpret_cast<T*>(s_sig[FUSE ? 0 : 2]);
+                    RedWs wsig;
+                    wsig.done = reinterpret_cast<unsigned long long*>(s_sig[0]);
+                    wsig.seq = s_sig[FUSE ? 0 : 1];
+                    __hip_atomic_store(o + 4, dv, __ATOMIC_RELAXED, __HIP_MEMORY_SCOPE_SYSTEM);
+                    __hip_atomic_store(o + 5, T(1), __ATOMIC_RELAXED, __HIP_MEMORY_SCOPE_SYSTEM);
+                    ws_signal(wsig);
+                }
                 if (FUSE && L == 2 * cn)
                 {
                     __hip_atomic_store(pf.out + 4, dv, __ATOMIC_RELAXED, __HIP_MEMORY_SCOPE_SYSTEM);
diff --git a/lbfgspp_amd/csrc/lbfgsx.hip b/lbfgspp_amd/csrc/lbfgsx.hip
--- a/lbfgspp_amd/csrc/lbfgsx.hip
+++ b/lbfgspp_amd/csrc/lbfgsx.hip
@@ -341,6 +341,8 @@
         c->fast_persist_out = atoi(e) != 0;
     if (const char* e = getenv("LBFGSX_FUSE_POST"))
         c->fuse_post = atoi(e) != 0;
+    if (const char* e = getenv("LBFGSX_POST_IN_TRIAL"))
+        c->post_in_trial = atoi(e) != 0;
     {
         int occ = 0;
         hipDeviceProp_t prop;
@@ -602,6 +604,8 @@
     c->ptr = c->m;
     c->pending = false;
     c->spec_valid = false;
+    c->pt_valid = c->pt_armed = c->ls_first_ok = false;
+    c->ls_trials = 0;
     c->tl_step = 0;
     for (int j = 0; j < c->m; j++)
         c->phys[size_t(j)] = j;
@@ -667,6 +671,7 @@
 {
     lbfgsx::DeviceGuard dev_guard_(c->device);
     c->spec_valid = false;
+    c->pt_valid = false;
     if (c->gs_f32h)
     {
         set_error("lbfgsx_bfgs_stage_correction_host: this context keeps its history in f32 for the Gram-space recursion (lbfgsx_gs_set_history_dtype)");
@@ -753,6 +758,7 @@
         pa.first_rev = c->tl_step;
         pa.pub_first = 1;
         pa.ld = c->ld;
+        pa.from_g = 0;
         c->gen_count += unsigned(2 * cn + 1);
         c->tl_step += unsigned(2 * cn + 1);
         if (c->meet_all)
@@ -938,6 +944,7 @@
 {
     lbfgsx::DeviceGuard dev_guard_(c->device);
     c->spec_valid = false;
+    c->pt_valid = false;
     double r[3];
     int rc = LBFGSX_E_INVALID;
     if (objective == LBFGSX_OBJ_EXT_ROSENBROCK && (c->n & 1))
@@ -984,6 +991,8 @@
 int lbfgsx_ls_begin(lbfgsx_ctx* c)
 {
     c->st_valid = false;
+    c->pt_valid = c->pt_armed = false;
+    c->ls_trials = 0;
     c->xp = c->cur;
     c->lo = c->xp;
     c->trial = (c->xp + 1) % 3;
@@ -999,6 +1008,59 @@
                        a.out, a.rev);
     LBFGSX_HIP(hipGetLastError());
     return fetch_scalars<T>(c, c->sl.out(0), 2, out2);
+}
+template <class T>
+static lbfgsx::TrialPost<T> trial_post_args(lbfgsx_ctx* c)
+{
+    T* sc = P<T>(c->sc);
+    return {P<T>(c->gb[c->xp]), P<T>(c->col(c->S, c->spare)), P<T>(c->col(c->Y, c->spare)), T(c->pt_a),
+            sc + c->sl.ys(c->spare), sc + c->sl.theta(c->spare), sc + c->sl.dot(0)};
+}
+static void trial_post_done(lbfgsx_ctx* c, const double* out6)
+{
+    c->pending = false;
+    c->pt_valid = true;
+    c->pt_buf = c->trial;
+    c->pt_xp = c->xp;
+    for (int i = 0; i < 4; i++)
+        c->pt_r[i] = out6[2 + i];
+    c->pt_issued++;
+}
+template <class T, class OBJ>
+static int trial_post_t(lbfgsx_ctx* c, OBJ obj, T step, double* out2)
+{
+    const lbfgsx::TrialLaunch<T> a = lbfgsx::trial_launch<T>(c, step, sizeof(OBJ) >= 2 * sizeof(void*) ? 2 : 0);
+    const lbfgsx::TrialPost<T> tp = trial_post_args<T>(c);
+    LBFGSX_LAUNCH((k_trial_post<T, OBJ>), dim3(a.grid), dim3(kBlock), 0, c->stream, a.xp, a.d, a.step, a.x, a.g, a.n, obj,
+                       a.ws, a.out, a.rev, tp);
+    LBFGSX_HIP(hipGetLastError());
+    double r[6];
+    const int rc = fetch_scalars<T>(c, c->sl.out(0), 6, r);
+    if (rc)
+        return rc;
+    out2[0] = r[0];
+    out2[1] = r[1];
+    trial_post_done(c, r);
+    return LBFGSX_OK;
+}
+template <class T>
+static int trial_post_term_t(lbfgsx_ctx* c, T step, double* out2)
+{
+    lbfgsx::TrialLaunch<T> a = lbfgsx::trial_launch<T>(c, step, c->term_np);
+    lbfgsx::BoundArgs<T> obj(c);
+    lbfgsx::TrialPost<T> tp = trial_post_args<T>(c);
+    void* params[] = {&a.xp, &a.d, &a.step, &a.x, &a.g, &a.n, obj.ptr, &a.ws, &a.out, &a.rev, &tp};
+    int rc = lbfgsx::jit_launch(c, lbfgsx::JIT_K_TRIAL_POST, a.grid, params);
+    if (rc)
+        return rc;
+    double r[6];
+    rc = fetch_scalars<T>(c, c->sl.out(0), 6, r);
+    if (rc)
+        return rc;
+    out2[0] = r[0];
+    out2[1] = r[1];
+    trial_post_done(c, r);
+    return LBFGSX_OK;
 }
 template <class T>
 static int trial_term_t(lbfgsx_ctx* c, T step, double* out2)
@@ -1032,6 +1094,7 @@
         if (same)
         {
             c->st_hits++;
+            c->ls_trials++;
             c->tl_step++;
             if (fx) *fx = c->st_f;
             if (dg) *dg = c->st_dg;
@@ -1039,13 +1102,19 @@
         }
         c->st_cooldown = 4;
     }
+    const bool post = c->pt_armed && c->ls_trials == 0 &&
+                      (objective == LBFGSX_OBJ_DIAG_QUAD || objective == LBFGSX_OBJ_EXT_ROSENBROCK ||
+                       (lbfgsx::term_bound(c, objective) && c->term_fn[lbfgsx::JIT_K_TRIAL_POST] != nullptr));
+    c->ls_trials++;
+    c->pt_valid = false;
     DISPATCH_T(c, {
         if (objective == LBFGSX_OBJ_DIAG_QUAD)
-            rc = trial_t<T>(c, ObjQuad<T>{P<T>(c->a), P<T>(c->b)}, T(step), r);
+            rc = post ? trial_post_t<T>(c, ObjQuad<T>{P<T>(c->a), P<T>(c->b)}, T(step), r)
+                      : trial_t<T>(c, ObjQuad<T>{P<T>(c->a), P<T>(c->b)}, T(step), r);
         else if (objective == LBFGSX_OBJ_EXT_ROSENBROCK)
-            rc = trial_t<T>(c, ObjRosen<T>{}, T(step), r);
+            rc = post ? trial_post_t<T>(c, ObjRosen<T>{}, T(step), r) : trial_t<T>(c, ObjRosen<T>{}, T(step), r);
         else if (lbfgsx::term_bound(c, objective))
-            rc = trial_term_t<T>(c, T(step), r);
+            rc = post ? trial_post_term_t<T>(c, T(step), r) : trial_term_t<T>(c, T(step), r);
         else
             set_error("lbfgsx_trial: unknown objective");
     });
@@ -1060,6 +1129,8 @@
 {
     lbfgsx::DeviceGuard dev_guard_(c->device);
     c->spec_valid = false;
+    c->pt_valid = false;
+    c->ls_trials++;
     const int grid = c->grid_for(c->n);
     DISPATCH_T(c, {
         LBFGSX_LAUNCH((k_axpy_point<T>), dim3(grid), dim3(kBlock), 0, c->stream, P<T>(c->xb[c->xp]), P<T>(c->d),
@@ -1097,6 +1168,7 @@
 int lbfgsx_ls_end(lbfgsx_ctx* c, int use_lo)
 {
     c->cur = use_lo ? c->lo : c->trial;
+    c->ls_first_ok = !use_lo && c->ls_trials == 1;
     return LBFGSX_OK;
 }
 
@@ -1104,6 +1176,7 @@
 {
     lbfgsx::DeviceGuard dev_guard_(c->device);
     c->spec_valid = false;
+    c->pt_valid = false;
     if (c->gs_f32h)
     {
         set_error("lbfgsx_post_linesearch: this context keeps its history in f32 for the Gram-space recursion (lbfgsx_gs_set_history_dtype)");
@@ -1134,7 +1207,7 @@
 
 }
 template <class T>
-static int post_spec_t(lbfgsx_ctx* c, T a, double* r4)
+static int post_spec_t(lbfgsx_ctx* c, T a, double* r4, bool from_g = false)
 {
     const int m = c->m;
     if (!(c->fuse_post && c->persist && c->persist_cooldown == 0 && c->persist_grid > 0 && m <= kPersistMaxM && !c->gs_f32h && c->device >= 0 &&
@@ -1163,6 +1236,7 @@
     pa.first_rev = c->tl_step;
     pa.pub_first = 1;
     pa.ld = c->ld;
+    pa.from_g = from_g ? 1 : 0;
     c->gen_count += unsigned(2 * cn + 1);
     c->tl_step += unsigned(2 * cn + 1);
     T* sc = P<T>(c->sc);
@@ -1190,21 +1264,30 @@
         static_cast<volatile T*>(c->outmap_host)[5] = T(0);
         lbfgsx::poll_arm(c);
     }
-    if (c->meet_all)
-        LBFGSX_LAUNCH((k_twoloop_persist<T, true, true>), dim3(c->persist_grid), dim3(kHvThreads), 0, c->stream, P<T>(c->d),
-                           P<T>(c->gb[c->cur]), a, P<T>(c->S), P<T>(c->Y), c->n, sc, pa, c->ws, c->gen_dev,
-                           reinterpret_cast<int*>(c->gen_dev + 1), pf);
+#define PERSIST_LAUNCH(FUSE, MEET)                                                                                          \
+    LBFGSX_LAUNCH((k_twoloop_persist<T, FUSE, MEET>), dim3(c->persist_grid), dim3(kHvThreads), 0, c->stream, P<T>(c->d),   \
+                  P<T>(c->gb[c->cur]), a, P<T>(c->S), P<T>(c->Y), c->n, sc, pa, c->ws, c->gen_dev,                        \
+                  reinterpret_cast<int*>(c->gen_dev + 1), pf)
+    if (from_g)
+    {
+        if (c->meet_all)
+            PERSIST_LAUNCH(false, true);
+        else
+            PERSIST_LAUNCH(false, false);
+    }
+    else if (c->meet_all)
+        PERSIST_LAUNCH(true, true);
     else
-        LBFGSX_LAUNCH((k_twoloop_persist<T, true, false>), dim3(c->persist_grid), dim3(kHvThreads), 0, c->stream, P<T>(c->d),
-                           P<T>(c->gb[c->cur]), a, P<T>(c->S), P<T>(c->Y), c->n, sc, pa, c->ws, c->gen_dev,
-                           reinterpret_cast<int*>(c->gen_dev + 1), pf);
+        PERSIST_LAUNCH(true, false);
+#undef PERSIST_LAUNCH
     LBFGSX_HIP(hipGetLastError());
+    const int fused = from_g ? 0 : 1;
     if (c->timing)
     {
         LBFGSX_HIP(hipEventRecord(hv.b, c->stream));
         c->ev_hv.push_back(hv);
         c->persist_steps_timed += 2 * cn + 1;
-        c->fused_timed++;
+        c->fused_timed += fused;
     }
     int hflags[2] = {0, 0};
     double dgv = 0.0;
@@ -1218,7 +1301,7 @@
         {
             hflags[1] = int(o[5]);
             dgv = double(o[4]);
-            for (int i = 0; i < 4; i++)
+            for (int i = 0; i < 4 && !from_g; i++)
                 r4[i] = double(o[i]);
             have = true;
         }
@@ -1228,12 +1311,14 @@
         LBFGSX_HIP(lbfgsx::copy_async(hflags, c->gen_dev + 1, 2 * sizeof(int), hipMemcpyDeviceToHost, c->stream));
         T* h = static_cast<T*>(c->hout);
         LBFGSX_HIP(lbfgsx::copy_async(h, sc + c->sl.dot(2 * cn), sizeof(T), hipMemcpyDeviceToHost, c->stream));
-        if (!c->outmap_dev)
+        if (!c->outmap_dev && !from_g)
             LBFGSX_HIP(lbfgsx::copy_async(h + 8, sc + c->sl.out(0), 4 * sizeof(T), hipMemcpyDeviceToHost, c->stream));
         LBFGSX_HIP(lbfgsx::stream_sync(c->stream));
         dgv = double(h[0]);
-        for (int i = 0; i < 4; i++)
+        for (int i = 0; i < 4 && !from_g; i++)
             r4[i] = c->outmap_dev ? double(static_cast<const volatile T*>(c->outmap_host)[i]) : double(h[8 + i]);
+        if (from_g)
+            hflags[1] = 1;
     }
     if (hflags[0])
     {
@@ -1247,12 +1332,13 @@
             (void) hipEventDestroy(c->ev_hv.back().b);
             c->ev_hv.pop_back();
             c->persist_steps_timed -= 2 * cn + 1;
-            c->fused_timed--;
+            c->fused_timed -= fused;
         }
         return 1;
     }
     c->persist_launches++;
     c->spec_launches++;
+    c->from_g_launches += from_g ? 1 : 0;
     c->persist_backoff = 8;
     if (hflags[1] == 1)
     {
@@ -1271,7 +1357,7 @@
             (void) hipEventDestroy(c->ev_hv.back().b);
             c->ev_hv.pop_back();
             c->persist_steps_timed -= 2 * cn + 1;
-            c->fused_timed--;
+            c->fused_timed -= fused;
         }
     }
     return LBFGSX_OK;
@@ -1286,6 +1372,30 @@
     double r[4];
     int rc = 1;
     c->spec_valid = false;
+    if (c->pt_valid && c->cur == c->pt_buf && c->xp == c->pt_xp)
+    {
+        c->pt_valid = false;
+        c->pt_accepted++;
+        for (int i = 0; i < 4; i++)
+            r[i] = c->pt_r[i];
+        c->pend_sy = r[2];
+        c->pend_yy = r[3];
+        c->pending = true;
+        bool usable = false;
+        DISPATCH_T(c, { usable = a == c->pt_a && T(r[2]) > std::numeric_limits<T>::epsilon() * T(r[3]); });
+        if (usable)
+        {
+            DISPATCH_T(c, { rc = post_spec_t<T>(c, T(a), r, true); });
+            if (rc != LBFGSX_OK && rc != 1)
+                return rc;
+        }
+        if (gnorm2) *gnorm2 = r[0];
+        if (xnorm2) *xnorm2 = r[1];
+        if (sy) *sy = r[2];
+        if (yy) *yy = r[3];
+        return LBFGSX_OK;
+    }
+    c->pt_valid = false;
     DISPATCH_T(c, { rc = post_spec_t<T>(c, T(a), r); });
     if (rc == 1)
         return lbfgsx_post_linesearch(c, gnorm2, xnorm2, sy, yy);
@@ -1298,6 +1408,27 @@
     if (xnorm2) *xnorm2 = r[1];
     if (sy) *sy = r[2];
     if (yy) *yy = r[3];
+    return LBFGSX_OK;
+}
+
+int lbfgsx_ls_post_in_trial(lbfgsx_ctx* c, double a)
+{
+    if (!c)
+        return LBFGSX_E_INVALID;
+    c->pt_a = a;
+    c->pt_armed = c->post_in_trial && c->ls_first_ok && c->ncorr > 0 && !c->gs_f32h && c->ls_trials == 0 &&
+                  c->shard_off == 0 && c->n_global == c->n;
+    return LBFGSX_OK;
+}
+
+int lbfgsx_post_in_trial_counts(const lbfgsx_ctx* c, int64_t out[4])
+{
+    if (!c || !out)
+        return LBFGSX_E_INVALID;
+    out[0] = c->pt_issued;
+    out[1] = c->pt_accepted;
+    out[2] = c->from_g_launches;
+    out[3] = c->post_in_trial ? 1 : 0;
     return LBFGSX_OK;
 }
 
```

Result: faster. 91.38 iterations/s (median of 6 runs) (+2.5%).
